# etri/bwa-mem-scale

Hardware: AMD Instinct MI355X
Metric: Mreads/sec through the GPU hot path (seed -> chain -> extend -> dedup, reads and index resident), 150bp SE vs a synthetic genome of GRCh38 size, at 1 MI355X; % HBM roofline in roofline.frac (higher is better)
Workload: dtype int64 intervals / int16 DP (two columns per register; int32 for queries beyond 191 bases or scores beyond 2^14)

## Files before the change

bwa-mem-scale_amd/bwams/capi.py:

```python
from __future__ import annotations

import ctypes as C
import os
import subprocess

import numpy as np

PKG = os.path.dirname(os.path.dirname(os.path.abspath(__file__)))
LIB_PATH = os.environ.get("BWAMS_LIB") or os.path.join(PKG, "_build", "libbwams.so")

SMEM_DTYPE = np.dtype([("rid", "<u4"), ("m", "<u4"), ("n", "<u4"), ("pad_", "<u4"),
                       ("k", "<i8"), ("l", "<i8"), ("s", "<i8")])
SEQPAIR_DTYPE = np.dtype([(n, "<i4") for n in
                          ("idr", "idq", "id", "len1", "len2", "h0", "seqid", "regid",
                           "score", "tle", "gtle", "qle", "gscore", "max_off")])

SYMBOLS = [
    "bwams_strerror", "bwams_last_error", "bwams_device_count", "bwams_debug_reload",
    "bwams_index_open", "bwams_index_from_host", "bwams_index_from_device", "bwams_index_close",
    "bwams_index_bytes", "bwams_index_build", "bwams_index_fetch", "bwams_index_save", "bwams_reg2aln_run", "bwams_reg2aln_run_sam", "bwams_reg2aln_fetch",
    "bwams_index_set_contig_names", "bwams_index_set_contig_annos", "bwams_sam_upload", "bwams_sam_run", "bwams_sam_run_pe", "bwams_sam_run_emf", "bwams_sam_fetch",
    "bwams_process_chunk", "bwams_process_chunk_smart", "bwams_process_chunk2", "bwams_emf_regs_merge", "bwams_fastq_decode", "bwams_fastq_info", "bwams_fastq_has_qual", "bwams_fastq_fetch", "bwams_fastq_to_batch", "bwams_fastq_to_batch_opt", "bwams_fastq_close", "bwams_batch_create", "bwams_batch_destroy", "bwams_seed_fmi",
    "bwams_seed_upload", "bwams_seed_run", "bwams_seed_counts", "bwams_seed_fetch",
    "bwams_ert_from_host", "bwams_ert_open", "bwams_ert_close", "bwams_ert_bytes", "bwams_ert_set_fat", "bwams_seed_run_ert",
# ... 67 lines not shown
class SwOpt(C.Structure):
    _fields_ = [("o_del", C.c_int32), ("e_del", C.c_int32), ("o_ins", C.c_int32),
                ("e_ins", C.c_int32), ("zdrop", C.c_int32), ("end_bonus", C.c_int32),
                ("mat", C.c_int8 * 25), ("pad_", C.c_int8 * 3)]


class MemOpt(C.Structure):
    _fields_ = [("a", C.c_int32), ("o_del", C.c_int32), ("e_del", C.c_int32), ("o_ins", C.c_int32), ("e_ins", C.c_int32),
                ("pen_clip5", C.c_int32), ("pen_clip3", C.c_int32), ("w", C.c_int32), ("zdrop", C.c_int32),
                ("min_seed_len", C.c_int32), ("min_chain_weight", C.c_int32), ("max_chain_extend", C.c_int32),
                ("max_occ", C.c_int32), ("max_chain_gap", C.c_int32), ("mask_level", C.c_float),
                ("drop_ratio", C.c_float), ("mat", C.c_int8 * 25), ("pad_", C.c_int8 * 3), ("extend_all", C.c_int32), ("mask_level_redun", C.c_float), ("max_ins", C.c_int32),
                ("b", C.c_int32), ("pen_unpaired", C.c_int32), ("max_matesw", C.c_int32), ("mapq_coef_len", C.c_int32)]


class FmiDesc(C.Structure):
    _fields_ = [("ref_seq_len", C.c_int64), ("count", C.c_int64 * 5),
                ("cp_occ", C.c_void_p), ("sa_ms_byte", C.c_void_p), ("sa_ls_word", C.c_void_p),
                ("sentinel_index", C.c_int64), ("ref_0123", C.c_void_p)]


class Fastq:

    def __init__(self, text, device: int = 0, n_bytes: int | None = None):
        self.h = C.c_void_p()
        n, nb = C.c_int64(0), C.c_int64(0)
        if isinstance(text, int):
            rc = lib().bwams_fastq_decode(device, C.c_void_p(text), C.c_int64(n_bytes), C.byref(self.h), C.byref(n), C.byref(nb))
        else:
            rc = lib().bwams_fastq_decode(device, text, C.c_int64(len(text)), C.byref(self.h), C.byref(n), C.byref(nb))
        _chk(rc, "bwams_fastq_decode")
        self.n_reads, self.n_bases = n.value, nb.value

    def info(self):
        n, nb, nn, nc, ms = C.c_int64(0), C.c_int64(0), C.c_int64(0), C.c_int64(0), C.c_float(0)
        _chk(lib().bwams_fastq_info(self.h, C.byref(n), C.byref(nb), C.byref(nn), C.byref(nc), C.byref(ms)), "bwams_fastq_info")
        return dict(n_reads=n.value, n_bases=nb.value, name_bytes=nn.value, comment_bytes=nc.value, ms=ms.value)

    def fetch(self):
        i = self.info()
        n1 = i["n_reads"] + 1
        enc = np.zeros(max(i["n_bases"], 1), np.uint8); qual = np.zeros(max(i["n_bases"], 1), np.uint8)
        names = np.zeros(max(i["name_bytes"], 1), np.uint8); comm = np.zeros(max(i["comment_bytes"], 1), np.uint8)
        cum = np.zeros(n1, np.int64); noff = np.zeros(n1, np.int64); coff = np.zeros(n1, np.int64)
        _chk(lib().bwams_fastq_fetch(self.h, _p(enc), _p(cum), _p(names), _p(noff), _p(qual), _p(comm), _p(coff)), "bwams_fastq_fetch")
        nb_, cb_ = bytes(names[:i["name_bytes"]]), bytes(comm[:i["comment_bytes"]])
        return dict(n=i["n_reads"], enc=enc[:i["n_bases"]], cum=cum, quals=qual[:i["n_bases"]] if lib().bwams_fastq_has_qual(self.h) else None,
                    names=[nb_[noff[k]:noff[k + 1]] for k in range(i["n_reads"])],
                    comments=[cb_[coff[k]:coff[k + 1]] or None for k in range(i["n_reads"])])

    def to_batch(self, batch: "Batch"):
        _chk(lib().bwams_fastq_to_batch(self.h, batch.h), "bwams_fastq_to_batch")
        batch._nseq = self.n_reads

    def close(self):
        if self.h:
            lib().bwams_fastq_close(self.h)
            self.h = C.c_void_p()


class SamOpt(C.Structure):
    _fields_ = [("T", C.c_int32), ("flag", C.c_int32), ("XA_drop_ratio", C.c_float), ("max_XA_hits", C.c_int32),
                ("max_XA_hits_alt", C.c_int32), ("rg_id", C.c_char * 256)]


def default_sam_opt(flag: int = 0, rg_id: bytes = b"") -> SamOpt:
    return SamOpt(30, flag, 0.80, 5, 200, rg_id)


class Stats(C.Structure):
    _fields_ = [("n_ext", C.c_int64), ("n_ext_blocks", C.c_int64), ("n_sa_lookups", C.c_int64),
                ("n_lf_steps", C.c_int64), ("n_smem", C.c_int64 * 3), ("bsw_cells", C.c_int64),
                ("n_ext_round", C.c_int64 * 3), ("n_blk_round", C.c_int64 * 3),
                ("ms_smem_r1", C.c_float), ("ms_smem_r2", C.c_float), ("ms_smem_r3", C.c_float),
                ("ms_sort", C.c_float), ("ms_sal", C.c_float), ("ms_seed_total", C.c_float),
                ("ms_bsw", C.c_float), ("ms_ksw", C.c_float), ("ms_tasks", C.c_float), ("ms_emf", C.c_float),
                ("emf_nodes", C.c_int64), ("emf_cmp_bytes", C.c_int64),
                ("n_chains", C.c_int64), ("n_chain_seeds", C.c_int64), ("n_left", C.c_int64), ("n_right", C.c_int64),
                ("n_retry_left", C.c_int64), ("n_retry_right", C.c_int64),
                ("ms_chain", C.c_float), ("ms_ext_plan", C.c_float), ("ms_ext_left", C.c_float),
                ("ms_ext_right", C.c_float), ("ms_ext_purge", C.c_float), ("ms_ext_total", C.c_float),
                ("n_ext_rounds", C.c_int64), ("n_final_regs", C.c_int64), ("ms_dedup", C.c_float), ("ms_pair", C.c_float),
                ("n_pair_tasks", C.c_int64), ("n_pair_redone", C.c_int64), ("n_pair_regs", C.c_int64), ("n_chain_redo", C.c_int64),
                ("ert_kmer_lookups", C.c_int64), ("ert_node_reads", C.c_int64), ("ert_ref_bytes", C.c_int64)]


class BuildStats(C.Structure):
    _fields_ = [("rows", C.c_int64), ("chunks", C.c_int32), ("rounds", C.c_int32), ("unresolved_after_first", C.c_int64),
                ("ms_first_pass", C.c_float), ("ms_outputs", C.c_float)]


class FastaStats(C.Structure):
    _fields_ = [("l_pac", C.c_int64), ("n_seqs", C.c_int32), ("n_holes", C.c_int32), ("n_ambig_bases", C.c_int64),
                ("ms_host_read", C.c_float), ("ms_upload", C.c_float), ("ms_device_pack", C.c_float), ("ms_fm_build", C.c_float),
                ("build", BuildStats)]


class InflateStats(C.Structure):
    _fields_ = [("members", C.c_int64), ("in_bytes", C.c_int64), ("out_bytes", C.c_int64),
                ("ms_upload", C.c_float), ("ms_kernel", C.c_float), ("ms_download", C.c_float)]


class ReaderStats(C.Structure):
    _fields_ = [("device_inflate", C.c_int32), ("in_bytes", C.c_int64), ("out_bytes", C.c_int64),
                ("ms_read", C.c_float), ("ms_inflate", C.c_float)]


class Inflater:

    def __init__(self, device: int = 0, max_in_bytes: int = 32 << 20, max_out_bytes: int = 64 << 20):
        self.h = C.c_void_p()
        self.max_out = max_out_bytes
        _chk(lib().bwams_inflater_create(device, max_in_bytes, max_out_bytes, C.byref(self.h)), "bwams_inflater_create")

    def run_raw(self, gz, out, out_cap: int, on_device: bool):
        used, n_out, st = C.c_int64(0), C.c_int64(0), InflateStats()
        ptr, n = (C.c_void_p(gz[0]), gz[1]) if isinstance(gz, tuple) else (gz, len(gz))
        rc = lib().bwams_inflater_run(self.h, ptr, n, C.c_void_p(out), out_cap, int(on_device), C.byref(used), C.byref(n_out),
                                      C.byref(st))
        return rc, used.value, n_out.value, st

    def run(self, gz: bytes, out_cap: int | None = None):
        cap = out_cap if out_cap is not None else self.max_out
        buf = C.create_string_buffer(max(cap, 1))
        rc, used, n, st = self.run_raw(gz, C.addressof(buf), cap, False)
        _chk(rc, "bwams_inflater_run")
        return buf.raw[:n], used, st

    def close(self):
        if self.h:
            lib().bwams_inflater_destroy(self.h)
            self.h = C.c_void_p()

    def __del__(self):
        try:
            self.close()
        except Exception:
            pass


class DeflateStats(C.Structure):
    _fields_ = [("members", C.c_int64), ("in_bytes", C.c_int64), ("out_bytes", C.c_int64),
                ("ms_upload", C.c_float), ("ms_kernel", C.c_float), ("ms_download", C.c_float)]


DEFLATE_EOF = 0x1


def deflate_bound(n_bytes: int) -> int:
    return lib().bwams_deflate_bound(n_bytes)


class Deflater:

    def __init__(self, device: int = 0, max_in_bytes: int = 32 << 20):
        self.h = C.c_void_p()
        self.device = device
        _chk(lib().bwams_deflater_create(device, max_in_bytes, C.byref(self.h)), "bwams_deflater_create")

    def run_raw(self, data, out, out_cap: int, in_on_device: bool = False, out_on_device: bool = False, flags: int = 0):
        n_out, st = C.c_int64(0), DeflateStats()
        ptr, n = (C.c_void_p(data[0]), data[1]) if isinstance(data, tuple) else (data, len(data))
        rc = lib().bwams_deflater_run(self.h, ptr, n, int(in_on_device), C.c_void_p(out), out_cap, int(out_on_device), flags,
                                      C.byref(n_out), C.byref(st))
        return rc, n_out.value, st

    def run(self, data, eof: bool = False):
# ... 1268 lines not shown
```

bwa-mem-scale_amd/csrc/api.hip:

```cpp
#include <fcntl.h>
#include <sys/mman.h>
#include <sys/stat.h>
#include <unistd.h>

#include <algorithm>
#include <cstring>
#include <mutex>
#include <string>
#include <vector>

#include <rocprim/rocprim.hpp>

#include "fmi_kernels.h"
#include "ert_kernels.h"
#include "stage_state.h"

namespace bwams {

static Knobs g_knobs;
static std::once_flag g_knobs_once;
static int env_int(const char *name, int dflt) { const char *e = getenv(name); return e && *e ? atoi(e) : dflt; }
void knobs_reload() {
    Knobs k;
    { const char *vb = getenv("BWAMS_VERBOSE"); k.verbose = vb && *vb && *vb != '0'; }
    k.debug = env_int("BWAMS_DEBUG", 0);
    k.poison = env_int("BWAMS_POISON", 0);
    k.bwd_min_list = env_int("BWAMS_BWD_MIN_LIST", k.bwd_min_list); k.bwd_cols = env_int("BWAMS_BWD_COLS", k.bwd_cols);
    k.bwd_late_list = env_int("BWAMS_BWD_LATE_LIST", k.bwd_late_list);
    k.bwd_dry_min_list = env_int("BWAMS_BWD_DRY_MIN_LIST", k.bwd_dry_min_list); k.bwd_dry_cols = env_int("BWAMS_BWD_DRY_COLS", k.bwd_dry_cols);
    k.bwd_dry_late_list = env_int("BWAMS_BWD_DRY_LATE_LIST", k.bwd_dry_late_list);
    k.r3_beside = env_int("BWAMS_SEED_R3_BESIDE", 1);
    k.ext_max_rounds = env_int("BWAMS_EXT_MAX_ROUNDS", 0); k.ext_all_rounds = getenv("BWAMS_EXT_ALL_ROUNDS") != nullptr;
    k.ext_inplace = env_int("BWAMS_EXT_INPLACE", 1);
    k.dedup_seq = env_int("BWAMS_DEDUP_SEQ", 0) == 1;
    k.pair_drop_plan = getenv("BWAMS_PAIR_DROP_PLAN") != nullptr;
    k.trace_pair = env_int("BWAMS_TRACE_PAIR", 0);
    k.bsw_pk = env_int("BWAMS_BSW_PK", 1);
    k.chain_batch = env_int("BWAMS_CHAIN_BATCH", 1);
    k.ert_ticket = env_int("BWAMS_ERT_TICKET", 1); k.ert_grid = env_int("BWAMS_ERT_GRID", -1); k.ert_fat = env_int("BWAMS_ERT_FAT", 1);
    g_knobs = k;
}
const Knobs &knobs() {
    std::call_once(g_knobs_once, knobs_reload);
    return g_knobs;
}

static thread_local std::string g_last_error;
void set_last_error(const std::string &s) { g_last_error = s; }

static int check_device(int device) {
    int n = 0;
    hipError_t e = hipGetDeviceCount(&n);
    if (e != hipSuccess || n <= 0) {
        set_last_error(std::string("no HIP device: ") + hipGetErrorString(e));
        return BWAMS_ERR_DEVICE;
    }
    if (device < 0 || device >= n) {
        set_last_error("device ordinal out of range");
        return BWAMS_ERR_ARG;
    }
    hipDeviceProp_t p;
    BWAMS_HIP(hipGetDeviceProperties(&p, device));
    if (std::string(p.gcnArchName).rfind("gfx950", 0) != 0) {
        set_last_error(std::string("device is ") + p.gcnArchName + ", this library is built for gfx950 only");
        return BWAMS_ERR_DEVICE;
    }
    return BWAMS_OK;
}

int tmp_reserve(bwams_batch *b, size_t &tb) {
    if (tb > b->d_tmp.cap) {
        BWAMS_HIP(hipStreamSynchronize(b->stream));
        BWAMS_HIP(b->d_tmp.alloc(tb));
    }
    tb = b->d_tmp.cap;
    return BWAMS_OK;
}
int fmi_build_device(bwams_index *ix, const uint8_t *d_fw, int64_t l_pac, int keep_ref, int64_t chunk_rows, int verbose,
                     bwams_build_stats_t *bs);

}

using namespace bwams;

extern "C" {

const char *bwams_strerror(int code) {
    switch (code) {
        case BWAMS_OK: return "ok";
        case BWAMS_ERR_DEVICE: return "no usable gfx950 device / HIP error";
        case BWAMS_ERR_IO: return "index file missing or malformed";
        case BWAMS_ERR_ARG: return "invalid argument";
        case BWAMS_ERR_CAPACITY: return "output buffer too small";
        case BWAMS_ERR_NOMEM: return "out of memory";
        case BWAMS_ERR_UNSUPPORTED: return "unsupported input";
    }
    return "unknown error";
}

const char *bwams_last_error(void) { return g_last_error.c_str(); }

int bwams_debug_reload(void) { (void)bwams::knobs(); bwams::knobs_reload(); return BWAMS_OK; }

int bwams_device_count(int *n) {
    int c = 0;
    hipError_t e = hipGetDeviceCount(&c);
    if (e != hipSuccess) {
        *n = 0;
        set_last_error(hipGetErrorString(e));
        return BWAMS_ERR_DEVICE;
    }
    *n = c;
    return BWAMS_OK;
}


static int index_finish(bwams_index *ix, const bwams_fmi_desc_t *d, const void *cp, const void *ms, const void *ls, const void *ref) {
    ix->fmi.cp = reinterpret_cast<const uint4 *>(cp);
    ix->fmi.cp2 = nullptr;
    ix->fmi.sa_ms = reinterpret_cast<const int8_t *>(ms);
    ix->fmi.sa_ls = reinterpret_cast<const uint32_t *>(ls);
// ... 1434 lines not shown
```

bwa-mem-scale_amd/csrc/api_chain.hip:

```cpp
#include <cstring>
#include <utility>

#include <rocprim/rocprim.hpp>

#include "stage_state.h"

using namespace bwams;

extern "C" {
int bwams_index_set_contigs(bwams_index_t *ix, const bwams_contig_t *contigs, int32_t n_seqs) {
    if (!ix || !contigs || n_seqs <= 0) return BWAMS_ERR_ARG;
    const int64_t l_pac = (ix->fmi.ref_seq_len - 1) / 2;
    int64_t at = 0;
    for (int32_t i = 0; i < n_seqs; ++i) {
        if (contigs[i].offset != at || contigs[i].len <= 0) {
            set_last_error("bwams_index_set_contigs: sequences must tile [0, l_pac) in order");
            return BWAMS_ERR_ARG;
        }
        at += contigs[i].len;
    }
    if (at != l_pac) {
        set_last_error("bwams_index_set_contigs: sequence lengths do not add up to l_pac");
        return BWAMS_ERR_ARG;
    }
// ... 66 lines not shown
static int chain_common(bwams_batch *b, const bwams_mem_opt_t *opt, const SeedView &sv, int64_t *n_chains, int64_t *n_seeds);

int bwams_chain_run(bwams_batch_t *b, const bwams_mem_opt_t *opt, int64_t *n_chains, int64_t *n_seeds) {
    if (!b || !b->seed_done || !b->with_sa) {
        set_last_error("bwams_chain_run: run bwams_seed_run(with_sa = 1) first");
        return BWAMS_ERR_ARG;
    }
    int rc = check_opt(opt, "bwams_chain_run");
    if (rc) return rc;
    if ((rc = bwams_seed_counts(b, nullptr, nullptr))) return rc;
    SeedView sv;
    sv.smem = b->d_sorted.p; sv.n_smem = b->n_smem; sv.sa_off = b->d_sa_off.p; sv.sa_coord = b->d_sa_coord.p; sv.n_sa = b->n_sa;
    sv.one_smem_quirk = true;
    return chain_common(b, opt, sv, n_chains, n_seeds);
}

int bwams_chain_run_ert(bwams_batch_t *b, const bwams_mem_opt_t *opt, const bwams_ert_mem_t *mems, const int64_t *mem_off,
                        const uint64_t *hits, const int64_t *hit_off, int64_t *n_chains, int64_t *n_seeds) {
    if (!b || b->nseq <= 0 || !mem_off || !hit_off) {
        set_last_error("bwams_chain_run_ert: upload the reads first (bwams_seed_upload) and pass the MEM / hit offsets");
        return BWAMS_ERR_ARG;
    }
    int rc = check_opt(opt, "bwams_chain_run_ert");
    if (rc) return rc;
    const int64_t nseq = b->nseq, n1 = nseq + 1;
    const int64_t n_mems = mem_off[nseq], n_hits = hit_off[nseq];
    if (mem_off[0] != 0 || hit_off[0] != 0 || n_mems < 0 || n_hits < 0 || (n_mems && !mems) || (n_hits && !hits)) return BWAMS_ERR_ARG;
    for (int64_t r = 0; r < nseq; ++r) {
        if (mem_off[r + 1] < mem_off[r] || hit_off[r + 1] < hit_off[r]) { set_last_error("bwams_chain_run_ert: offsets must be non-decreasing"); return BWAMS_ERR_ARG; }
        const int64_t nh = hit_off[r + 1] - hit_off[r];
        for (int64_t i = mem_off[r]; i < mem_off[r + 1]; ++i) {
            const bwams_ert_mem_t &m = mems[i];
            if (m.start < 0 || m.end <= m.start || m.hitcount < 0 || m.hitbeg < 0 || (int64_t)m.hitbeg + m.hitcount > nh) {
                set_last_error("bwams_chain_run_ert: a MEM with an empty span or a hit slice outside its read's hit array");
                return BWAMS_ERR_ARG;
            }
        }
    }
    BWAMS_HIP(hipSetDevice(b->idx->device));
    StageState *s;
    if ((rc = get_state(b, &s))) return rc;
    hipStream_t st = b->stream;
    BWAMS_HIP(s->ch.et_mems.ensure_n((size_t)(n_mems + 1))); BWAMS_HIP(s->ch.et_moff.ensure_n((size_t)n1));
    BWAMS_HIP(s->ch.et_hoff.ensure_n((size_t)n1)); BWAMS_HIP(s->ch.et_hits.ensure_n((size_t)(n_hits + 1)));
    BWAMS_HIP(s->ch.et_smem.ensure_n((size_t)(n_mems + 1))); BWAMS_HIP(s->ch.et_cnt.ensure_n((size_t)(n_mems + 1)));
    BWAMS_HIP(s->ch.et_off.ensure_n((size_t)(n_mems + 1))); BWAMS_HIP(s->ch.et_srt.ensure((size_t)(n_mems + 1) * 24));
    if (n_mems) BWAMS_HIP(hipMemcpyAsync(s->ch.et_mems.p, mems, (size_t)n_mems * sizeof(bwams_ert_mem_t), hipMemcpyHostToDevice, st));
    if (n_hits) BWAMS_HIP(hipMemcpyAsync(s->ch.et_hits.p, hits, (size_t)n_hits * 8, hipMemcpyHostToDevice, st));
    BWAMS_HIP(hipMemcpyAsync(s->ch.et_moff.p, mem_off, (size_t)n1 * 8, hipMemcpyHostToDevice, st));
    BWAMS_HIP(hipMemcpyAsync(s->ch.et_hoff.p, hit_off, (size_t)n1 * 8, hipMemcpyHostToDevice, st));
    ErtArgs E;
    E.mems = s->ch.et_mems.p; E.mem_off = s->ch.et_moff.p; E.hits = s->ch.et_hits.p; E.hit_off = s->ch.et_hoff.p; E.nseq = nseq; E.n_mems = n_mems;
    E.l_pac = (b->idx->fmi.ref_seq_len - 1) / 2; E.max_occ = opt->max_occ; E.pad_ = 0; E.smem_out = s->ch.et_smem.p; E.cnt = s->ch.et_cnt.p;
    E.srt = s->ch.et_srt.p;
    launch_ert_sort(E, st);
    if ((rc = scan_rows(b, s->ch.et_cnt.p, s->ch.et_off.p, 1, n_mems + 1))) return rc;
    int64_t n_sa = 0;
    BWAMS_HIP(hipMemcpyAsync(&n_sa, s->ch.et_off.p + n_mems, 8, hipMemcpyDeviceToHost, st));
    BWAMS_HIP(hipStreamSynchronize(st));
    BWAMS_HIP(s->ch.et_coord.ensure_n((size_t)(n_sa + 1)));
    launch_ert_pick(E, s->ch.et_off.p, s->ch.et_coord.p, st);
    SeedView sv;
    sv.smem = s->ch.et_smem.p; sv.n_smem = n_mems; sv.sa_off = s->ch.et_off.p;
    sv.sa_coord = s->ch.et_coord.p; sv.n_sa = n_sa; sv.one_smem_quirk = false;
    return chain_common(b, opt, sv, n_chains, n_seeds);
}

static int chain_common(bwams_batch *b, const bwams_mem_opt_t *opt, const SeedView &sv, int64_t *n_chains, int64_t *n_seeds) {
    int rc;
    if (b->max_read_len >= 32768) {
        set_last_error("bwams_chain_run: reads of 32768 bases or more are not supported (16-bit query coordinates)");
        return BWAMS_ERR_UNSUPPORTED;
    }
    BWAMS_HIP(hipSetDevice(b->idx->device));
    StageState *s;
    if ((rc = get_state(b, &s))) return rc;
    outdated(s, From::chain);
    hipStream_t st = b->stream;
    const int64_t nseq = b->nseq, n_sa = sv.n_sa, n1 = nseq + 1;
    const size_t ns = (size_t)(n_sa > 0 ? n_sa : 1);
    BWAMS_HIP(s->ch.s_next.ensure_n(ns)); BWAMS_HIP(s->ch.s_ql.ensure_n(ns)); BWAMS_HIP(s->ch.crec.ensure(chain_rec_bytes(n_sa)));
    BWAMS_HIP(s->ch.flt.ensure_n(ns)); BWAMS_HIP(s->ch.f_rec.ensure_n(ns)); BWAMS_HIP(s->ch.f_first.ensure_n(ns));
    BWAMS_HIP(s->ch.f_kept.ensure_n(ns)); BWAMS_HIP(s->ch.f_sel.ensure_n(ns)); BWAMS_HIP(s->ch.n_chn.ensure_n((size_t)n1));
    BWAMS_HIP(s->heavy.ensure_n((size_t)n1)); BWAMS_HIP(s->ch.redo.ensure_n((size_t)n1)); BWAMS_HIP(s->ch.slice.ensure((size_t)n1 * 16));
    BWAMS_HIP(s->ch.okeys.ensure_n((size_t)n1)); BWAMS_HIP(s->ch.okeys2.ensure_n((size_t)n1)); BWAMS_HIP(s->ch.ovals.ensure_n((size_t)n1));
    BWAMS_HIP(s->ch.ovals2.ensure_n((size_t)n1)); BWAMS_HIP(s->ch.nodes.ensure(chain_node_bytes(n_sa, nseq)));
    BWAMS_HIP(s->ch.n_kept.ensure_n((size_t)n1)); BWAMS_HIP(s->ch.n_kept_seeds.ensure_n((size_t)n1)); BWAMS_HIP(s->ch.read_base.ensure_n((size_t)n1));
    BWAMS_HIP(s->ch.frac.ensure_n((size_t)n1)); BWAMS_HIP(s->ch.wide.ensure((size_t)n1 * 16)); BWAMS_HIP(s->ch.chain_off.ensure((size_t)n1 * 16));

    ChainArgs A;
    A.smem = sv.smem; A.n_smem = sv.n_smem; A.sa_off = sv.sa_off; A.sa_coord = sv.sa_coord; A.cum = b->d_cum.p; A.nseq = nseq;
    if ((rc = dev_bns(b->idx, &A.bns))) return rc;
    A.opt = *opt;
    A.s_next = s->ch.s_next.p; A.s_ql = s->ch.s_ql.p; A.crec = s->ch.crec.p; A.flt = s->ch.flt.p; A.f_rec = s->ch.f_rec.p;
    A.f_first = s->ch.f_first.p; A.f_kept = s->ch.f_kept.p; A.f_sel = s->ch.f_sel.p; A.nodes = s->ch.nodes.p; A.n_kept = s->ch.n_kept.p;
    A.n_kept_seeds = s->ch.n_kept_seeds.p; A.n_chn = s->ch.n_chn.p; A.heavy = s->heavy.p; A.redo = s->ch.redo.p; A.slice = s->ch.slice.as<int64_t>();
    A.order = s->ch.ovals2.p; A.read_base = s->ch.read_base.p; A.frac_rep = s->ch.frac.p; A.ctr = b->d_ctr.p; A.seed_batch = knobs().chain_batch;

    BWAMS_HIP(hipEventRecord(s->ev[0], st));
    BWAMS_HIP(hipMemsetAsync(&b->d_ctr.p->chain_redo, 0, 2 * sizeof(unsigned long long), st));
    BWAMS_HIP(hipMemsetAsync(&b->d_ctr.p->chain_overflow, 0, 29 * sizeof(unsigned long long), st));
    if ((sv.one_smem_quirk ? sv.n_smem <= 1 : sv.n_smem <= 0) || n_sa == 0) {
        BWAMS_HIP(hipMemsetAsync(s->ch.n_kept.p, 0, (size_t)n1 * 4, st));
        BWAMS_HIP(hipMemsetAsync(s->ch.n_kept_seeds.p, 0, (size_t)n1 * 4, st));
    } else {
        launch_chain_count(A, s->ch.okeys.p, s->ch.ovals.p, st);
        if ((rc = with_tmp(b, "bwams_chain_run: radix_sort_pairs_desc", [&](void *tmp, size_t &tb) {
                return rocprim::radix_sort_pairs_desc(tmp, tb, s->ch.okeys.p, s->ch.okeys2.p, s->ch.ovals.p, s->ch.ovals2.p, (size_t)nseq, 0, 32, st);
            }))) return rc;
        if (launch_chain(A, s->ch.okeys.p, b->cu_count, st, s->aux, s->fork, s->join)) {
            set_last_error("bwams_chain_run: stream fork/join failed");
            return BWAMS_ERR_DEVICE;
        }
    }
    int64_t tot[2] = {0, 0};
    if (nseq > 0) {
        launch_widen2(A.n_kept, A.n_kept_seeds, nseq, s->ch.wide.as<int64_t>(), st);
        if ((rc = scan_rows(b, s->ch.wide.as<int64_t>(), s->ch.chain_off.as<int64_t>(), 2, n1))) return rc;
        BWAMS_HIP(hipMemcpyAsync(&tot[0], s->ch.chain_off.as<int64_t>() + nseq, 8, hipMemcpyDeviceToHost, st));
        BWAMS_HIP(hipMemcpyAsync(&tot[1], s->ch.chain_off.as<int64_t>() + n1 + nseq, 8, hipMemcpyDeviceToHost, st));
    } else {
        BWAMS_HIP(hipMemsetAsync(s->ch.chain_off.p, 0, (size_t)n1 * 16, st));
    }
    BWAMS_HIP(hipMemcpyAsync(b->h_ctr.p, b->d_ctr.p, sizeof(DevCounters), hipMemcpyDeviceToHost, st));
    BWAMS_HIP(hipStreamSynchronize(st));
    {
        const bool vb = knobs().verbose != 0;
        if (vb) {
            const unsigned long long *d = b->h_ctr.p->dbg;
            fprintf(stderr, "[bwams_chain_run] filter wave tier: reads by chains <=32 %llu <=64 %llu <=128 %llu <=256 %llu <=512 %llu <=960 %llu more %llu; "
                            "Mcycles: sequential(HBM) %.1f sort %.1f filter %.1f; chains %llu selected %llu; longest read: sort %.2f filter %.2f Mcycles, most chains %llu, most selected %llu\n",
                    d[0], d[1], d[2], d[3], d[4], d[5], d[6], d[7] / 1e6, d[8] / 1e6, d[9] / 1e6, d[11], d[10], d[12] / 1e6, d[13] / 1e6, d[14], d[15]);
#ifdef BWAMS_CHAINDBG
            static const char *cn[8] = {"XL", "L", "L2", "L1", "M2", "M", "M1", "S"};
            fprintf(stderr, "[bwams_chain_run] chaining wave tier, per class: reads / mean us / longest us / wave-ms:");
            for (int c = 0; c < 8; ++c) fprintf(stderr, "  %s %llu / %.0f / %.0f / %.1f", cn[c], d[32 + 3 * c], d[32 + 3 * c] ? d[33 + 3 * c] * 1e-2 / d[32 + 3 * c] : 0.0, d[34 + 3 * c] * 1e-2, d[33 + 3 * c] * 1e-5);
            fprintf(stderr, "\n");
            fprintf(stderr, "[bwams_chain_run] wave tier phases, G cycles: preamble %.2f chaining %.2f weights+copy %.2f (sort %.2f filter %.2f: all reads); reads %llu seeds %llu; passes %llu settling %llu seeds (%llu new chains), %llu seeds one by one; pass parts, G cycles: batch prologue %.2f search %.2f record+test %.2f settle %.2f commit %.2f one-by-one %.2f\n",
                    d[56] / 1e9, d[57] / 1e9, d[58] / 1e9, d[8] / 1e9, d[9] / 1e9, d[59], d[60], d[61], d[63], d[64], d[62], d[65] / 1e9, d[66] / 1e9, d[67] / 1e9, d[68] / 1e9, d[69] / 1e9, d[70] / 1e9);
#endif
        }
    }
    if (b->h_ctr.p->chain_overflow) {
        set_last_error("bwams_chain_run: internal B-tree node region exhausted");
        return BWAMS_ERR_CAPACITY;
    }
    const bool has_long = b->h_ctr.p->chain_longread != 0;
    s->ch.n_redo = (int64_t)b->h_ctr.p->chain_redo;
    s->ch.n_chains = tot[0]; s->ch.n_seeds = tot[1]; s->ch.nseq = nseq;
    BWAMS_HIP(s->ch.chains.ensure_n((size_t)(tot[0] + 1))); BWAMS_HIP(s->ch.seeds.ensure_n((size_t)(tot[1] + 1)));
    if (tot[0] > 0) launch_chain_emit(A, s->ch.chain_off.as<int64_t>(), s->ch.chain_off.as<int64_t>() + n1, s->ch.chains.p, s->ch.seeds.p, st);
    if (has_long && tot[0] > 0 && (rc = flt_chained_seeds(b, s, opt, A.bns))) return rc;
    BWAMS_HIP(hipEventRecord(s->ev[1], st));
    BWAMS_HIP(hipGetLastError());
    s->ch.done = true;
    s->opt = *opt;
    if (n_chains) *n_chains = s->ch.n_chains;
    if (n_seeds) *n_seeds = s->ch.n_seeds;
    return BWAMS_OK;
}

int bwams_chain_fetch(bwams_batch_t *b, bwams_chain_t *chains, int64_t chain_cap, bwams_chain_seed_t *seeds,
                      int64_t seed_cap, int64_t *chain_off) {
    if (!b || !b->chain || !b->chain->ch.done) {
        set_last_error("bwams_chain_fetch: no chains on the device");
        return BWAMS_ERR_ARG;
    }
    StageState *s = b->chain;
    if (s->ch.n_chains > chain_cap || s->ch.n_seeds > seed_cap) return BWAMS_ERR_CAPACITY;
    BWAMS_HIP(hipSetDevice(b->idx->device));
    hipStream_t st = b->stream;
    if (s->ch.n_chains) BWAMS_HIP(hipMemcpyAsync(chains, s->ch.chains.p, (size_t)s->ch.n_chains * sizeof(bwams_chain_t), hipMemcpyDeviceToHost, st));
    if (s->ch.n_seeds) BWAMS_HIP(hipMemcpyAsync(seeds, s->ch.seeds.p, (size_t)s->ch.n_seeds * sizeof(bwams_chain_seed_t), hipMemcpyDeviceToHost, st));
    if (chain_off) BWAMS_HIP(hipMemcpyAsync(chain_off, s->ch.chain_off.p, (size_t)(s->ch.nseq + 1) * 8, hipMemcpyDeviceToHost, st));
    BWAMS_HIP(hipStreamSynchronize(st));
    return BWAMS_OK;
}

int bwams_chain_upload(bwams_batch_t *b, const bwams_chain_t *chains, int64_t n_chains, const bwams_chain_seed_t *seeds,
                       int64_t n_seeds, const int64_t *chain_off) {
    if (!b || !chain_off || n_chains < 0 || n_seeds < 0 || (n_chains && (!chains || !seeds))) return BWAMS_ERR_ARG;
    if (b->nseq <= 0) {
        set_last_error("bwams_chain_upload: upload the reads first (bwams_seed_upload)");
        return BWAMS_ERR_ARG;
    }
    const int64_t nseq = b->nseq, n1 = nseq + 1;
    if (chain_off[0] != 0 || chain_off[nseq] != n_chains) return BWAMS_ERR_ARG;
    int64_t at = 0;
    std::string bad;
    int64_t *soff = new int64_t[(size_t)n1];
    for (int64_t r = 0; r < nseq && bad.empty(); ++r) {
        soff[r] = at;
        if (chain_off[r + 1] < chain_off[r]) bad = "chain_off must be non-decreasing";
        for (int64_t j = chain_off[r]; j < chain_off[r + 1] && bad.empty(); ++j) {
            if (chains[j].seqid != r) bad = "chain.seqid does not match chain_off";
            else if (chains[j].seed_off != at || chains[j].n < 0) bad = "chain.seed_off must enumerate the seed array in order";
            at += chains[j].n;
        }
    }
    soff[nseq] = at;
    if (bad.empty() && at != n_seeds) bad = "seed counts do not add up";
    if (!bad.empty()) {
        delete[] soff;
        set_last_error("bwams_chain_upload: " + bad);
        return BWAMS_ERR_ARG;
    }
    BWAMS_HIP(hipSetDevice(b->idx->device));
    StageState *s;
    int rc = get_state(b, &s);
    if (rc) { delete[] soff; return rc; }
    outdated(s, From::chain);
    hipStream_t st = b->stream;
    BWAMS_HIP(s->ch.chain_off.ensure((size_t)n1 * 16)); BWAMS_HIP(s->ch.chains.ensure_n((size_t)(n_chains + 1)));
    BWAMS_HIP(s->ch.seeds.ensure_n((size_t)(n_seeds + 1)));
    BWAMS_HIP(hipMemcpyAsync(s->ch.chain_off.p, chain_off, (size_t)n1 * 8, hipMemcpyHostToDevice, st));
    BWAMS_HIP(hipMemcpyAsync(s->ch.chain_off.as<int64_t>() + n1, soff, (size_t)n1 * 8, hipMemcpyHostToDevice, st));
    if (n_chains) BWAMS_HIP(hipMemcpyAsync(s->ch.chains.p, chains, (size_t)n_chains * sizeof(bwams_chain_t), hipMemcpyHostToDevice, st));
    if (n_seeds) BWAMS_HIP(hipMemcpyAsync(s->ch.seeds.p, seeds, (size_t)n_seeds * sizeof(bwams_chain_seed_t), hipMemcpyHostToDevice, st));
    BWAMS_HIP(hipStreamSynchronize(st));
    delete[] soff;
    s->ch.n_chains = n_chains; s->ch.n_seeds = n_seeds; s->ch.nseq = nseq;
    s->ch.done = true;
    return BWAMS_OK;
}
}
```

bwa-mem-scale_amd/csrc/api_regions.hip:

```cpp
#include <algorithm>
#include <cmath>
#include <cstring>
#include <utility>

#include <rocprim/rocprim.hpp>

#include "stage_state.h"

using namespace bwams;

extern "C" {

int bwams_dedup_run(bwams_batch_t *b, const bwams_mem_opt_t *opt, int64_t *n_regs) {
    if (!b || !b->chain || !b->chain->ext.done) {
        set_last_error("bwams_dedup_run: run bwams_extend_run first");
        return BWAMS_ERR_ARG;
    }
    int rc = check_opt(opt, "bwams_dedup_run");
    if (rc) return rc;
    StageState *s = b->chain;
    BWAMS_HIP(hipSetDevice(b->idx->device));
    hipStream_t st = b->stream;
    outdated(s, From::dedup);
    const int64_t N = s->ch.n_seeds, n1 = s->ch.nseq + 1;
    const int64_t L = b->max_read_len > 1 ? b->max_read_len : 1;
    int64_t n_lanes = ((int64_t)1 << 30) / ((L + 2) * 8);
    n_lanes = n_lanes > 65536 ? 65536 : n_lanes < 64 ? 64 : n_lanes;
    const int64_t n_waves = (int64_t)b->cu_count * 4, n_waves_small = (int64_t)b->cu_count * 16;
    BWAMS_HIP(s->dd.regs.ensure_n((size_t)(N + 1))); BWAMS_HIP(s->dd.out.ensure_n((size_t)(N + 1))); BWAMS_HIP(s->dd.ord.ensure_n((size_t)(N + 1)));
    BWAMS_HIP(s->dd.srt.ensure(dedup_sortrec_bytes(N)));
    BWAMS_HIP(s->dd.eh.ensure((size_t)(n_lanes + 2 * n_waves + n_waves_small) * (size_t)(L + 2) * 8)); BWAMS_HIP(s->dd.nout.ensure_n((size_t)n1));
    BWAMS_HIP(s->dd.wide.ensure((size_t)n1 * 16)); BWAMS_HIP(s->dd.off.ensure_n((size_t)n1));
    DedupArgs D;
    D.regs = s->dd.regs.p; D.seed_off = s->ch.chain_off.as<int64_t>() + n1; D.enc = b->d_enc.p; D.cum = b->d_cum.p; D.nseq = s->ch.nseq;
    D.ref = b->idx->fmi.ref;
    if ((rc = dev_bns(b->idx, &D.bns))) return rc;
    D.opt = *opt; D.ord = s->dd.ord.p; D.srt = s->dd.srt.p; D.eh = s->dd.eh.as<int2>(); D.eh_lanes = n_lanes; D.max_read_len = (int32_t)L;
    D.n_out = s->dd.nout.p;
    BWAMS_HIP(s->heavy.ensure_n((size_t)n1));
    D.force_seq = knobs().dedup_seq;
    BWAMS_HIP(s->dd.light.ensure_n((size_t)n1));
    D.heavy = s->heavy.p; D.light = s->dd.light.p; D.n_heavy_ctr = &b->d_ctr.p->dedup_heavy; D.ticket = &b->d_ctr.p->dedup_ticket;
    D.n_light_ctr = &b->d_ctr.p->dedup_light; D.ticket2 = &b->d_ctr.p->dedup_ticket2; D.ticket3 = &b->d_ctr.p->dedup_ticket3;
    const bool verbose_dd = knobs().verbose != 0;
    D.dbg = verbose_dd ? b->d_ctr.p->dbg : nullptr;
    if (verbose_dd) BWAMS_HIP(hipMemsetAsync(b->d_ctr.p->dbg, 0, sizeof b->d_ctr.p->dbg, st));
    BWAMS_HIP(hipMemsetAsync(&b->d_ctr.p->dedup_heavy, 0, 3 * sizeof(unsigned long long), st));
    BWAMS_HIP(hipMemsetAsync(&b->d_ctr.p->dedup_ticket2, 0, 2 * sizeof(unsigned long long), st));
    BWAMS_HIP(hipEventRecord(s->ev[12], st));
    if (N) BWAMS_HIP(hipMemcpyAsync(D.regs, s->ext.regs.p, (size_t)N * sizeof(bwams_alnreg_t), hipMemcpyDeviceToDevice, st));
    BWAMS_HIP(hipMemsetAsync(D.n_out, 0, (size_t)n1 * 4, st));
    if (launch_dedup(D, n_lanes, n_waves, n_waves_small, st, s->aux[0], s->aux[1], s->aux[2], s->fork, s->join[0], s->join[1], s->join[2])) {
        set_last_error("bwams_dedup_run: stream fork/join failed");
        return BWAMS_ERR_DEVICE;
    }
    int64_t total = 0;
    if (s->ch.nseq > 0) {
        launch_widen2(D.n_out, D.n_out, s->ch.nseq, s->dd.wide.as<int64_t>(), st);
        if ((rc = scan_rows(b, s->dd.wide.as<int64_t>(), s->dd.off.p, 1, n1))) return rc;
        launch_dedup_gather(D, s->dd.off.p, s->dd.out.p, st);
        BWAMS_HIP(hipMemcpyAsync(&total, s->dd.off.p + s->ch.nseq, 8, hipMemcpyDeviceToHost, st));
    } else {
        BWAMS_HIP(hipMemsetAsync(s->dd.off.p, 0, 8, st));
    }
    BWAMS_HIP(hipEventRecord(s->ev[13], st));
    if (verbose_dd) BWAMS_HIP(hipMemcpyAsync(b->h_ctr.p->dbg, b->d_ctr.p->dbg, sizeof b->d_ctr.p->dbg, hipMemcpyDeviceToHost, st));
    BWAMS_HIP(hipStreamSynchronize(st));
    BWAMS_HIP(hipGetLastError());
    if (verbose_dd) {
        const unsigned long long *d = b->h_ctr.p->dbg;
        fprintf(stderr, "[bwams_dedup_run] largest wave instance: %llu reads, %llu slots, %llu alive; Mcycles: load %.1f sort(end) %.1f pairs %.1f reload %.1f sort(score) %.1f store %.1f; "
                        "longest read: sort(end) %.2f pairs %.2f sort(score) %.2f, whole %.2f (read %llu, %llu regions; %llu patch alignments in %.2f, %llu scan trips); all reads: %llu patch alignments in %.1f\n",
                d[0], d[1], d[2], d[3] / 1e6, d[4] / 1e6, d[5] / 1e6, d[6] / 1e6, d[7] / 1e6, d[8] / 1e6, d[9] / 1e6, d[10] / 1e6, d[11] / 1e6, d[12] / 1e6, d[13], d[14],
                d[15], d[16] / 1e6, d[17], d[18], d[19] / 1e6);
    }
    s->dd.n_final = total;
    s->dd.done = true;
    if (n_regs) *n_regs = total;
    return BWAMS_OK;
}

int bwams_dedup_fetch(bwams_batch_t *b, bwams_alnreg_t *regs, int64_t reg_cap, int64_t *reg_off) {
    if (!b || !b->chain || !b->chain->dd.done) {
        set_last_error("bwams_dedup_fetch: run bwams_dedup_run first");
        return BWAMS_ERR_ARG;
    }
    StageState *s = b->chain;
    if (s->dd.n_final > reg_cap) return BWAMS_ERR_CAPACITY;
    BWAMS_HIP(hipSetDevice(b->idx->device));
    hipStream_t st = b->stream;
    if (s->dd.n_final) BWAMS_HIP(hipMemcpyAsync(regs, s->dd.out.p, (size_t)s->dd.n_final * sizeof(bwams_alnreg_t), hipMemcpyDeviceToHost, st));
    if (reg_off) BWAMS_HIP(hipMemcpyAsync(reg_off, s->dd.off.p, (size_t)(s->ch.nseq + 1) * 8, hipMemcpyDeviceToHost, st));
    BWAMS_HIP(hipStreamSynchronize(st));
    return BWAMS_OK;
}


static int pair_run_impl(bwams_batch_t *b, const bwams_mem_opt_t *opt, const bwams_pestat_t pes[4], int64_t id_base, int32_t flags,
                         int primary5_T, int no_pairing, int64_t *n_regs, int64_t *n_tasks);

int bwams_pair_run(bwams_batch_t *b, const bwams_mem_opt_t *opt, const bwams_pestat_t pes[4], int64_t id_base, int32_t flags,
                   int64_t *n_regs, int64_t *n_tasks) {
    return pair_run_impl(b, opt, pes, id_base, flags, -1, 0, n_regs, n_tasks);
}

int bwams_pair_run_sam(bwams_batch_t *b, const bwams_mem_opt_t *opt, const bwams_sam_opt_t *sam_opt, const bwams_pestat_t pes[4],
                       int64_t id_base, int32_t flags, int64_t *n_regs, int64_t *n_tasks) {
    if (!sam_opt) return pair_run_impl(b, opt, pes, id_base, flags, -1, 0, n_regs, n_tasks);
    if (sam_opt->T < 0) {
        set_last_error("bwams_pair_run_sam: T must not be negative");
        return BWAMS_ERR_ARG;
    }
    if (sam_opt->flag & BWAMS_MEM_F_NO_RESCUE) flags |= BWAMS_PAIR_NO_RESCUE;
    return pair_run_impl(b, opt, pes, id_base, flags, (sam_opt->flag & BWAMS_MEM_F_PRIMARY5) ? sam_opt->T : -1,
                         (sam_opt->flag & BWAMS_MEM_F_NOPAIRING) != 0, n_regs, n_tasks);
}

static int pair_run_impl(bwams_batch_t *b, const bwams_mem_opt_t *opt, const bwams_pestat_t pes[4], int64_t id_base, int32_t flags,
                         int primary5_T, int no_pairing, int64_t *n_regs, int64_t *n_tasks) {
    const int single_end = (flags & BWAMS_PAIR_SINGLE_END) != 0;
    const int no_rescue = (flags & BWAMS_PAIR_NO_RESCUE) || single_end, use_ert = (flags & BWAMS_PAIR_USE_ERT) != 0;
    static const bwams_pestat_t no_pes[4] = {{0, 0, 1, 0, 0., 0.}, {0, 0, 1, 0, 0., 0.}, {0, 0, 1, 0, 0., 0.}, {0, 0, 1, 0, 0., 0.}};
    if (single_end && !pes) pes = no_pes;
    if (!b || !b->chain || !b->chain->dd.done) {
        set_last_error("bwams_pair_run: run bwams_dedup_run first");
        return BWAMS_ERR_ARG;
    }
    int rc = check_opt(opt, "bwams_pair_run");
    if (rc) return rc;
    StageState *s = b->chain;
    if (!pes || (!single_end && (s->ch.nseq & 1))) {
        set_last_error("bwams_pair_run: needs the insert-size statistics and an even number of reads (ends of pair p at 2p, 2p + 1)");
        return BWAMS_ERR_ARG;
    }
    int tmax = 1;
// ... 346 lines not shown
```

bwa-mem-scale_amd/csrc/api_state.hip:

```cpp
#include <cstring>
#include <map>

#include <rocprim/rocprim.hpp>

#include "stage_state.h"

namespace bwams {

struct AuxSet { hipStream_t q[7] = {}; int refs = 0; };
static std::mutex g_aux_mu;
static std::map<int, AuxSet> g_aux;
static int aux_acquire(int device, hipStream_t *out) {
    std::lock_guard<std::mutex> g(g_aux_mu);
    AuxSet &a = g_aux[device];
    if (a.refs == 0)
        for (auto &q : a.q) BWAMS_HIP(hipStreamCreateWithFlags(&q, hipStreamNonBlocking));
    ++a.refs;
    for (int i = 0; i < 7; ++i) out[i] = a.q[i];
    return BWAMS_OK;
}
static void aux_release(int device) {
    std::lock_guard<std::mutex> g(g_aux_mu);
    auto it = g_aux.find(device);
    if (it == g_aux.end()) return;
// ... 26 lines not shown
}

void launch_widen2(const int32_t *a, const int32_t *b, int64_t n, int64_t *wide, hipStream_t st) {
    widen2_kernel<<<(unsigned)((2 * (n + 1) + 255) / 256), 256, 0, st>>>(a, b, n, wide);
}

int scan_rows(bwams_batch *b, const int64_t *in, int64_t *out, int rows, int64_t n1) {
    for (int r = 0; r < rows; ++r)
        if (int rc = with_tmp(b, "scan_rows: exclusive_scan", [&](void *tmp, size_t &tb) {
                return rocprim::exclusive_scan(tmp, tb, in + r * n1, out + r * n1, (int64_t)0, (size_t)n1, rocprim::plus<int64_t>(), b->stream);
            })) return rc;
    return BWAMS_OK;
}

void outdated(StageState *s, From first) {
    switch (first) {
    case From::chain: s->ch.done = false; [[fallthrough]];
    case From::built: s->ext.built = s->ext.done = false; [[fallthrough]];
    case From::dedup: s->dd.done = false; [[fallthrough]];
    case From::pair: s->pr.done = false; break;
    case From::al: s->al.done = false; break;
    case From::er: s->er.done = false; break;
    case From::sam_upload: s->sm.up = false; [[fallthrough]];
    case From::sam: s->sm.done = false; [[fallthrough]];
    case From::bam: s->bm.done = s->bs.done = s->md.done = false; break;
    }
}

int get_state(bwams_batch *b, StageState **out) {
    if (!b->chain) {
        b->chain = new StageState();
        for (auto &e : b->chain->ev) BWAMS_HIP(hipEventCreate(&e));
        for (auto &e : b->chain->join) BWAMS_HIP(hipEventCreateWithFlags(&e, hipEventDisableTiming));
        BWAMS_HIP(hipEventCreateWithFlags(&b->chain->fork, hipEventDisableTiming));
        b->chain->ev_ok = true;
        if (int rc = aux_acquire(b->idx->device, b->chain->aux)) return rc;
        b->chain->aux_device = b->idx->device;
    }
    *out = b->chain;
    return BWAMS_OK;
}

int check_opt(const bwams_mem_opt_t *o, const char *who) {
    if (!o || o->e_del <= 0 || o->e_ins <= 0 || o->max_occ <= 0 || o->w < 0) {
        set_last_error(std::string(who) + ": null options, non-positive gap extension penalty or max_occ");
        return BWAMS_ERR_ARG;
    }
    return BWAMS_OK;
}

int dev_bns(bwams_index *ix, DevBns *out) {
    const int64_t l_pac = (ix->fmi.ref_seq_len - 1) / 2;
    if (!ix->d_contigs.p) {
        bwams_contig_t c;
        c.offset = 0; c.len = (int32_t)l_pac; c.is_alt = 0;
        if (l_pac > 0x7fffffffLL) {
            set_last_error("the index holds more than 2^31 bases: call bwams_index_set_contigs with the real sequences");
            return BWAMS_ERR_ARG;
        }
        BWAMS_HIP(ix->d_contigs.alloc(sizeof c));
        BWAMS_HIP(hipMemcpy(ix->d_contigs.p, &c, sizeof c, hipMemcpyHostToDevice));
        ix->n_seqs = 1;
    }
    out->contigs = ix->d_contigs.as<const bwams_contig_t>();
    out->n_seqs = ix->n_seqs;
    out->l_pac = l_pac;
    return BWAMS_OK;
}

void sw_params(const bwams_mem_opt_t &o, int end_bonus, SwParams *prm) {
    prm->o_del = o.o_del; prm->e_del = o.e_del; prm->o_ins = o.o_ins; prm->e_ins = o.e_ins;
    prm->zdrop = o.zdrop; prm->end_bonus = end_bonus;
    int mx = 0;
    for (int i = 0; i < 25; ++i) {
        prm->mat[i] = o.mat[i];
        mx = mx > o.mat[i] ? mx : o.mat[i];
    }
    prm->max_sc = mx;
}

void chain_state_stats(const StageState *s, bwams_stats_t *out) {
    if (!s) return;
    out->n_chains = s->ch.n_chains; out->n_chain_seeds = s->ch.n_seeds; out->n_chain_redo = s->ch.n_redo;
    out->n_left = s->ext.n_left; out->n_right = s->ext.n_right;
    out->n_retry_left = s->ext.n_retry_left; out->n_retry_right = s->ext.n_retry_right;
    auto el = [&](int a, int b, float *dst) {
        float ms = 0;
        if (hipEventElapsedTime(&ms, s->ev[a], s->ev[b]) == hipSuccess) *dst = ms;
    };
    el(0, 1, &out->ms_chain);
    el(2, 3, &out->ms_ext_plan);
    if (s->ext.done) {
        el(4, 5, &out->ms_ext_left);
        el(6, 7, &out->ms_ext_right);
        el(8, 9, &out->ms_ext_purge);
        el(10, 11, &out->ms_ext_total);
        out->n_ext_rounds = s->ext.n_rounds;
    }
    if (s->dd.done) { el(12, 13, &out->ms_dedup); out->n_final_regs = s->dd.n_final; }
    if (s->pr.done) {
        el(14, 15, &out->ms_pair);
        out->n_pair_tasks = s->pr.tasks; out->n_pair_redone = s->pr.redone; out->n_pair_regs = s->pr.total;
    }
    (void)hipGetLastError();
}
}
```

bwa-mem-scale_amd/csrc/chain.hip:

```cpp
#include "common.h"
#include "chain_kernels.h"
#include "wave_ops.h"

namespace bwams {
namespace {

constexpr int KB_T = 5;
constexpr int KB_MAXK = 2 * KB_T - 1;
constexpr int kLaneSeeds = 32;
constexpr int kLightChains = 16;
struct alignas(16) Node {
    int16_t n, internal;
    int32_t ptr[KB_MAXK + 1];
    int64_t pos[KB_MAXK];
    int32_t key[KB_MAXK];
};
static_assert(sizeof(Node) == 160, "node layout");

struct alignas(16) ChainRec {
    int64_t last_rbeg, endr;
    uint16_t first_qbeg, last_qbeg, last_len, endq;
    int32_t rid, n;
    int32_t first_idx, last_idx;
    int32_t wq, wr;
// ... 709 lines not shown
            while (rem) {
                const int i = __builtin_ctzll(rem);
                rem &= rem - 1;
                int fin = act;
                if (displaced) {
                    const int64_t x = qbeg - best_q, y = rbeg - best;
                    if (rid != best_rid) fin = NEW;
                    else if (qbeg >= best_q && qbeg + slen <= best_q + best_l && rbeg + slen <= best + best_l) fin = NOOP;
                    else if (best < l_pac && rbeg >= l_pac) fin = NEW;
                    else fin = (x - y <= w && y - x <= w && x - best_l < max_gap && y - best_l < max_gap) ? UNSETTLED : NEW;
                } else if (touched) fin = UNSETTLED;
                const int a_i = __builtin_amdgcn_readlane(fin, i);
                if (a_i == UNSETTLED) { first_open = i; break; }
                if (lane == i) act = fin;
                if (a_i == NEW) {
                    const int64_t rb_i = readlane64(rbeg, i);
                    const int rid_i = __builtin_amdgcn_readlane(rid, i), q_i = __builtin_amdgcn_readlane(qbeg, i), l_i = __builtin_amdgcn_readlane(slen, i);
                    if (lane > i && rb_i <= rbeg && rb_i > best) { best = rb_i; best_rid = rid_i; best_q = q_i; best_l = l_i; displaced = true; }
                } else if (a_i == MERGE) {
                    const int low_i = __builtin_amdgcn_readlane(lower, i);
                    if (lane > i && lower == low_i) touched = true;
                }
            }
            const bool com = pend && lane < first_open;
            TQ(3)
            const unsigned long long m_new = __ballot(com && act == NEW);
            if (__ballot(com && act == NEW && (eq || (displaced && best == rbeg)))) return false;
            if (com && act == MERGE) {
                S.s_ql[g] = make_int2(qbeg, slen); S.s_next[g] = -1; S.s_next[ch.last_idx] = g;
                if (qbeg >= ch.endq) ch.wq += slen; else if (qbeg + slen > ch.endq) ch.wq += qbeg + slen - ch.endq;
                ch.endq = (uint16_t)((int)ch.endq > qbeg + slen ? (int)ch.endq : qbeg + slen);
                if (rbeg >= ch.endr) ch.wr += slen; else if (rbeg + slen > ch.endr) ch.wr += (int)(rbeg + slen - ch.endr);
                ch.endr = ch.endr > rbeg + slen ? ch.endr : rbeg + slen;
                ch.last_rbeg = rbeg; ch.last_qbeg = (uint16_t)qbeg; ch.last_len = (uint16_t)slen; ch.last_idx = g; ch.n += 1;
                S.crec[lower] = ch;
            }
            if (m_new) {
                const int m = __popcll(m_new);
                const bool mine = com && act == NEW;
                int min_idx = mine ? idx : n;
                for (int d = 32; d >= 1; d >>= 1) { const int o = __shfl_xor(min_idx, d); min_idx = o < min_idx ? o : min_idx; }
                for (int cb = n > 0 ? ((n - 1) >> 6) << 6 : -64; cb >= 0 && cb + 63 > min_idx; cb -= 64) {
                    const int p = cb + lane;
                    const bool mv = p < n;
                    const int64_t kk = mv ? S.s_key[p] : 0;
                    const int32_t cc = mv ? S.s_cid[p] : 0;
                    int sh = __popcll(__ballot(mine && idx < cb));
                    unsigned long long mm = __ballot(mine && idx >= cb && idx < cb + 64);
                    while (mm) { const int i = __builtin_ctzll(mm); mm &= mm - 1; sh += __builtin_amdgcn_readlane(idx, i) < p ? 1 : 0; }
                    if (mv && sh) { S.s_key[p + sh] = kk; S.s_cid[p + sh] = cc; }
                }
                int rank = 0;
                { unsigned long long mm = m_new; while (mm) { const int i = __builtin_ctzll(mm); mm &= mm - 1; rank += __builtin_amdgcn_readlane(idx, i) < idx ? 1 : 0; } }
                { unsigned long long mm = m_new & __ballot(shared); while (mm) { const int i = __builtin_ctzll(mm); mm &= mm - 1; rank += (__builtin_amdgcn_readlane(idx, i) == idx && readlane64(rbeg, i) < rbeg) ? 1 : 0; } }
                if (mine) {
                    const int32_t cid = n + __popcll(m_new & below);
                    S.s_ql[g] = make_int2(qbeg, slen); S.s_next[g] = -1;
                    ChainRec nc;
                    nc.last_rbeg = rbeg; nc.endr = rbeg + slen;
                    nc.first_qbeg = (uint16_t)qbeg; nc.last_qbeg = (uint16_t)qbeg; nc.last_len = (uint16_t)slen; nc.endq = (uint16_t)(qbeg + slen);
                    nc.rid = rid; nc.n = 1; nc.first_idx = g; nc.last_idx = g; nc.wq = slen; nc.wr = slen;
                    S.crec[cid] = nc;
                    S.s_key[idx + 1 + rank] = rbeg; S.s_cid[idx + 1 + rank] = cid;
                }
                n_keys = n + m;
            }
            if (com) pend = false;
#ifdef BWAMS_CHAINDBG
            if (lane == 0) { atomicAdd(&A.ctr->dbg[61], 1ull); atomicAdd(&A.ctr->dbg[63], (unsigned long long)__popcll(__ballot(com))); atomicAdd(&A.ctr->dbg[64], (unsigned long long)__popcll(m_new)); }
#endif
            if (__popcll(__ballot(com)) <= 1) one_by_one = 8;
            if (S.crec_hbm) __threadfence_block();
            TQ(4)
        }
    }
#ifdef BWAMS_CHAINDBG
    if (lane == 0) for (int k = 0; k < 6; ++k) atomicAdd(&A.ctr->dbg[65 + k], tq[k]);
#endif
    return true;
}

__device__ void heavy_read(const ChainArgs &A, int64_t r, int64_t base, int n_chn, unsigned char *lds, int cap, int lane);
__host__ __device__ constexpr size_t heavy_lds_bytes(int cap);
template <bool LDS, int CONT = 0, bool CREC_HBM = false>
__device__ __forceinline__ bool chain_read(const ChainArgs &A, int64_t r, int lane, int nl, Node *nodes, int32_t cap_nodes,
                                           ChainRec *crec_w, int32_t cap_chains) {
    const bool wr = lane == 0;
#ifdef BWAMS_CHAINDBG
    const unsigned long long tp0 = __builtin_amdgcn_s_memtime();
#endif
    if (wr) {
        A.n_kept[r] = 0;
        A.n_kept_seeds[r] = 0;
        A.read_base[r] = 0;
        A.n_chn[r] = 0;
    }
    const bwams_smem_t *sm = A.smem;
    const int64_t beg = A.slice[2 * r], end = A.slice[2 * r + 1];
    const int L = (int)(A.cum[r + 1] - A.cum[r]);
    if (beg == end || L < A.opt.min_seed_len) return true;

    int b = 0, e = 0, l_rep = 0;
    if (nl == 64 && end - beg <= 64) {
        const bool has = beg + lane < end;
        const int my_b = has ? (int)sm[beg + lane].m : 0, my_e = has ? (int)sm[beg + lane].n + 1 : 0;
        unsigned long long rep = __ballot(has && sm[beg + lane].s > (int64_t)A.opt.max_occ);
        while (rep) {
            const int i = __builtin_ctzll(rep);
            rep &= rep - 1;
            const int sb = __builtin_amdgcn_readlane(my_b, i), se = __builtin_amdgcn_readlane(my_e, i);
            if (sb > e) { l_rep += e - b; b = sb; e = se; }
            else e = e > se ? e : se;
        }
    } else
    for (int64_t i = beg; i < end; ++i) {
        const int sb = (int)sm[i].m, se = (int)sm[i].n + 1;
        if (sm[i].s <= (int64_t)A.opt.max_occ) continue;
        if (sb > e) { l_rep += e - b; b = sb; e = se; }
        else e = e > se ? e : se;
    }
    l_rep += e - b;
    if (wr) A.frac_rep[r] = (float)l_rep / (float)L;

    const int64_t base = A.sa_off[beg];
    const int32_t cnt = (int32_t)(A.sa_off[end] - base);
    if (wr) A.read_base[r] = base;
    if (cnt == 0) return true;
    const int64_t *pos = A.sa_coord + base;
    int32_t *s_next = A.s_next + base;
    int2 *s_ql = A.s_ql + base;
    ChainRec *crec_g = reinterpret_cast<ChainRec *>(A.crec) + base;
    ChainRec *crec;
    ReadCtx c;
    if constexpr (LDS) {
        crec = CREC_HBM ? crec_g : crec_w;
        c.nodes = nodes; c.cap_nodes = cap_nodes;
    } else {
        crec = crec_g;
        const int64_t nbase = (base >> 1) + 2 * r;
        c.nodes = reinterpret_cast<Node *>(A.nodes) + nbase;
        c.cap_nodes = (int32_t)((((base + cnt) >> 1) + 2 * (r + 1)) - nbase);
    }
    c.crec = crec;
    c.n_nodes = 0; c.n_keys = 0; c.overflow = false; c.wr = wr;
    int64_t *s_key = nullptr;
    int32_t *s_cid = nullptr;
    if constexpr (CONT == 1) {
        s_key = reinterpret_cast<int64_t *>(nodes);
        s_cid = reinterpret_cast<int32_t *>(s_key + cap_chains);
    } else c.root = new_node(c);
    RidCache rc;
    rc.lo = 0; rc.hi = -1; rc.rid = 0;
    WaveBns wb;
    wb.off = 0;
    if (nl == 64 && A.bns.n_seqs <= 4096) wb = wave_bns_load(A.bns, lane);
    if (LDS && cnt > cap_chains) { if (wr) atomicAdd(&A.ctr->chain_overflow, 1ull); return true; }

    const int64_t l_pac = A.bns.l_pac;
#ifdef BWAMS_CHAINDBG
    const unsigned long long tp1 = __builtin_amdgcn_s_memtime();
#endif
    if constexpr (CONT == 1) {
        if (nl == 64 && A.seed_batch) {
            SeedCtx S;
            S.pos = pos; S.s_next = s_next; S.s_ql = s_ql; S.crec = crec; S.s_key = s_key; S.s_cid = s_cid; S.crec_hbm = CREC_HBM;
            int nk = 0;
// ... 63 lines not shown
                ch.last_rbeg = rbeg; ch.endr = rbeg + slen;
                ch.first_qbeg = (uint16_t)qbeg; ch.last_qbeg = (uint16_t)qbeg; ch.last_len = (uint16_t)slen; ch.endq = (uint16_t)(qbeg + slen);
                ch.rid = rid; ch.n = 1; ch.first_idx = g; ch.last_idx = g; ch.wq = slen; ch.wr = slen;
                const int32_t cid = c.n_keys;
                if (wr) crec[cid] = ch;
                if constexpr (CONT == 1) {
                    if (c.n_keys && !path.ok) return false;
                    sarr_insert(s_key, s_cid, c.n_keys, c.n_keys ? path.leaf + 1 : 0, rbeg, cid, lane);
                    ++c.n_keys;
                } else kbt_put(c, cid, rbeg);
                if (c.overflow) { if (wr) atomicAdd(&A.ctr->chain_overflow, 1ull); return true; }
            }
        }
    }
    if (c.n_keys == 0) return true;
#ifdef BWAMS_CHAINDBG
    const unsigned long long tp2 = __builtin_amdgcn_s_memtime();
#endif

    int32_t *ord = A.f_first + base;
    int32_t n_trav;
    if constexpr (CONT == 1) {
        n_trav = c.n_keys;
        for (int32_t t = lane; t < n_trav; t += nl) ord[t] = s_cid[t];
        __threadfence_block();
    } else n_trav = kbt_traverse(c, ord);
    uint2 *fl = A.flt + base;
    int n_chn = 0;
    if (nl == 64) {
        uint2 first = make_uint2(0u, 0u);
        for (int32_t t0 = 0; t0 < n_trav; t0 += 64) {
            const int32_t t = t0 + lane;
            const bool ok = t < n_trav;
            int32_t id = 0;
            if (ok) { if constexpr (CONT == 1) id = s_cid[t]; else id = ord[t]; }
            const ChainRec *pc = &crec[id];
            int w = pc->wr < pc->wq ? pc->wr : pc->wq;
            w = w < (1 << 30) ? w : (1 << 30) - 1;
            if (t0 == 0) first = make_uint2((unsigned)__builtin_amdgcn_readfirstlane(w), (unsigned)__builtin_amdgcn_readfirstlane(id));
            const bool keep = ok && w >= A.opt.min_chain_weight;
            const unsigned long long m = __ballot(keep);
            if (keep) fl[n_chn + __popcll(m & ((1ull << lane) - 1ull))] = make_uint2((unsigned)w, (unsigned)id);
            n_chn += __popcll(m);
        }
        if (n_chn == 0 && wr) fl[0] = first;
        __threadfence_block();
    } else
    for (int32_t t = 0; t < n_trav; ++t) {
        const int32_t id = ord[t];
        const ChainRec ch = crec[id];
        int w = ch.wr < ch.wq ? ch.wr : ch.wq;
        w = w < (1 << 30) ? w : (1 << 30) - 1;
        if (t == 0 && wr) fl[0] = make_uint2((unsigned)w, (unsigned)id);
        if (w < A.opt.min_chain_weight) continue;
        if (wr) fl[n_chn] = make_uint2((unsigned)w, (unsigned)id);
        ++n_chn;
    }
    if (n_chn == 0) n_chn = 1;
    if constexpr (LDS && !CREC_HBM)
        for (int32_t k = lane; k < c.n_keys; k += nl) crec_g[k] = crec_w[k];
    if constexpr (LDS) {
        if (nl == 64) {
#ifdef BWAMS_CHAINDBG
            if (wr) {
                const unsigned long long tp3 = __builtin_amdgcn_s_memtime();
                atomicAdd(&A.ctr->dbg[56], tp1 - tp0); atomicAdd(&A.ctr->dbg[57], tp2 - tp1); atomicAdd(&A.ctr->dbg[58], tp3 - tp2);
                atomicAdd(&A.ctr->dbg[59], 1ull); atomicAdd(&A.ctr->dbg[60], (unsigned long long)cnt);
            }
#endif
            unsigned char *region = CREC_HBM ? reinterpret_cast<unsigned char *>(nodes) : reinterpret_cast<unsigned char *>(crec_w);
            const size_t bytes = (size_t)cap_chains * (CREC_HBM ? 12 : sizeof(ChainRec) + 12);
            const int cap_f = (int)((bytes - 64) / 41);
            if (cap_f >= 64 && n_chn <= cap_f) {
                if (wr) A.n_chn[r] = n_chn;
                __threadfence_block();
                heavy_read(A, r, base, n_chn, region, cap_f, lane);
                return true;
            }
        }
    }
    if (!wr) return true;
    A.n_chn[r] = n_chn;
    if (n_chn > kLightChains) {
        const unsigned long long slot = atomicAdd(&A.ctr->n_heavy, 1ull);
        A.heavy[slot] = (int32_t)r;
        return true;
    }
    flt_introsort(fl, n_chn);
    uint4 *rec = A.f_rec + base;
    int32_t *kept = A.f_kept + base;
    for (int i = 0; i < n_chn; ++i) {
        rec[i] = make_rec(A, crec[fl[i].y], fl[i].x);
        kept[i] = 0;
    }
    filter_seq(A.opt, n_chn, rec, kept, A.f_sel + base);
    if constexpr (LDS) __threadfence_block();
    finish_read(A, r, base, n_chn, L);
    return true;
}

__global__ __launch_bounds__(64) void chain_kernel(ChainArgs A, const uint32_t *__restrict__ n_seeds) {
    const int64_t r = (int64_t)blockIdx.x * blockDim.x + threadIdx.x;
    if (r >= A.nseq) return;
    if (n_seeds[r] > (uint32_t)kLaneSeeds) return;
    chain_read<false>(A, r, 0, 1, nullptr, 0, nullptr, 0);
}

__global__ __launch_bounds__(64) __attribute__((amdgpu_waves_per_eu(3, 3))) void chain_wave_kernel(ChainArgs A, const unsigned long long *lo_p, const unsigned long long *hi_p,
                                                        unsigned long long *ticket, int K) {
    extern __shared__ __align__(16) unsigned char l_mem[];
    const int lane = threadIdx.x;
    const int64_t lo = lo_p ? (int64_t)*lo_p : 0, hi = (int64_t)*hi_p;
    ChainRec *l_crec = reinterpret_cast<ChainRec *>(l_mem);
    Node *l_nodes = reinterpret_cast<Node *>(l_mem + (size_t)(K > 0 ? K : 0) * sizeof(ChainRec));
    for (;;) {
        const unsigned long long t = wave_ticket(ticket, 1ull);
        if (lo + (int64_t)t >= hi) break;
        const int64_t r = (int64_t)A.order[lo + (int64_t)t];
#ifdef BWAMS_CHAINDBG
        const unsigned long long tk0 = wall_clock64();
#endif
        if (K < 0) {
            if (!chain_read<true, 1, true>(A, r, lane, 64, reinterpret_cast<Node *>(l_mem), 0, nullptr, -K) && lane == 0)
                A.redo[atomicAdd(&A.ctr->chain_redo, 1ull)] = (int32_t)r;
        } else if (K) {
            if (!chain_read<true, 1>(A, r, lane, 64, l_nodes, 0, l_crec, K) && lane == 0)
                A.redo[atomicAdd(&A.ctr->chain_redo, 1ull)] = (int32_t)r;
        } else chain_read<false>(A, r, lane, 64, nullptr, 0, nullptr, 0);
        __syncthreads();
#ifdef BWAMS_CHAINDBG
        if (lane == 0) {
            const int c = K < 0 ? 0 : K == kClassL ? 1 : K == kClassL2 ? 2 : K == kClassL1 ? 3 : K == kClassM2 ? 4 : K == kClassM ? 5 : K == kClassM1 ? 6 : 7;
            const unsigned long long dt = wall_clock64() - tk0;
            atomicAdd(&A.ctr->dbg[32 + 3 * c], 1ull); atomicAdd(&A.ctr->dbg[33 + 3 * c], dt); atomicMax(&A.ctr->dbg[34 + 3 * c], dt);
        }
#endif
    }
}

__global__ __launch_bounds__(64) void chain_redo_kernel(ChainArgs A) {
    const int lane = threadIdx.x;
    const int64_t n = (int64_t)A.ctr->chain_redo;
    for (;;) {
        const int64_t t = (int64_t)wave_ticket(&A.ctr->chain_redo_ticket, 1ull);
        if (t >= n) break;
        chain_read<false>(A, A.redo[t], lane, 64, nullptr, 0, nullptr, 0);
    }
}

constexpr int kHeavyCap[6] = {64, 128, 256, 512, 960, 3840};
__host__ __device__ constexpr size_t heavy_lds_bytes(int cap) { return (size_t)cap * 41 + 64; }
static_assert(heavy_lds_bytes(kHeavyCap[5]) <= 160 * 1024, "the largest class must fit one CU's LDS");

__device__ void heavy_read(const ChainArgs &A, int64_t r, int64_t base, int n_chn, unsigned char *lds, int cap, int lane) {
    uint4 *l_rec = reinterpret_cast<uint4 *>(lds);
    uint4 *l_sel = l_rec + cap;
    uint2 *l_fl = reinterpret_cast<uint2 *>(l_sel + cap);
    uint8_t *l_kept = reinterpret_cast<uint8_t *>(l_fl + cap);
    const int L = (int)(A.cum[r + 1] - A.cum[r]);
    uint2 *fl = A.flt + base;
    const ChainRec *crec = reinterpret_cast<const ChainRec *>(A.crec) + base;
    const unsigned long long t_0 = __builtin_amdgcn_s_memtime();
    if (lane == 0) {
        const int bk = n_chn <= 32 ? 0 : n_chn <= 64 ? 1 : n_chn <= 128 ? 2 : n_chn <= 256 ? 3 : n_chn <= 512 ? 4 : n_chn <= 960 ? 5 : 6;
        atomicAdd(&A.ctr->dbg[bk], 1ull);
    }
    {
        __syncthreads();
        for (int i = lane; i < n_chn; i += 64) l_fl[i] = fl[i];
        __syncthreads();
        wave_flt_introsort(l_fl, n_chn, reinterpret_cast<uint16_t *>(l_sel), reinterpret_cast<int *>(reinterpret_cast<char *>(l_sel) + (size_t)n_chn * 8), lane);
        const unsigned long long t_1 = __builtin_amdgcn_s_memtime();
        for (int i = lane; i < n_chn; i += 64) {
            const uint2 f = l_fl[i];
            l_rec[i] = make_rec(A, crec[f.y], f.x);
            l_kept[i] = 0;
        }
        __syncthreads();
        int n_sel = 1;
        if (lane == 0) { const uint4 r0 = l_rec[0]; l_sel[0] = make_uint4(r0.x, r0.y, r0.z, 0u); l_kept[0] = 3; }
        __syncthreads();
        const float mask_level = A.opt.mask_level, drop_ratio = A.opt.drop_ratio;
        const int max_gap = A.opt.max_chain_gap, min_dw = A.opt.min_seed_len << 1;
        for (int ib = 1; ib < n_chn; ib += 64) {
            const int i = ib + lane;
            const bool valid = i < n_chn;
            const uint4 ri = valid ? l_rec[i] : make_uint4(0, 0, 0, 0);
            const int bi = (int)ri.x, ei = (int)ri.y, wi = (int)(ri.z & 0x7fffffffu), li = ei - bi;
            const bool alt_i = (ri.z >> 31) != 0;
            const float fwi = (float)wi;
            bool alive = valid, large = false;
            const int n_sel0 = n_sel;
            for (int k0 = 0; k0 < n_sel0; k0 += 4) {
                uint4 rj[4];
#pragma unroll
                for (int u = 0; u < 4; ++u) rj[u] = l_sel[k0 + u < n_sel0 ? k0 + u : n_sel0 - 1];
#pragma unroll
                for (int u = 0; u < 4; ++u) {
                    if (k0 + u >= n_sel0) break;
                    const int bj = (int)rj[u].x, ej = (int)rj[u].y;
                    const int b_max = bj > bi ? bj : bi, e_min = ej < ei ? ej : ei;
                    const bool alt_j = (rj[u].z >> 31) != 0;
                    const int lj = ej - bj, min_l = li < lj ? li : lj;
                    const bool lg = alive && e_min > b_max && (!alt_j || alt_i) && (float)(e_min - b_max) >= (float)min_l * mask_level && min_l < max_gap;
                    const unsigned long long m_lg = __ballot(lg);
                    if (m_lg) {
                        if (lane == __builtin_ctzll(m_lg)) atomicMin(&l_rec[rj[u].w].w, (uint32_t)i);
                        if (lg) {
                            large = true;
                            const int wj = (int)(rj[u].z & 0x7fffffffu);
                            if (fwi < (float)wj * drop_ratio && wj - wi >= min_dw) alive = false;
                        }
                    }
                }
                if (!__ballot(alive)) break;
            }
            unsigned long long todo = __ballot(alive);
            while (todo) {
                const int lp = __builtin_ctzll(todo);
                const int bj = __builtin_amdgcn_readlane(bi, lp), ej = __builtin_amdgcn_readlane(ei, lp);
                const uint32_t zj = (uint32_t)__builtin_amdgcn_readlane((int)ri.z, lp);
                if (lane == lp) { l_sel[n_sel] = make_uint4(ri.x, ri.y, ri.z, (uint32_t)i); l_kept[i] = large ? 2 : 3; }
                ++n_sel;
                const int b_max = bj > bi ? bj : bi, e_min = ej < ei ? ej : ei;
                const bool alt_j = (zj >> 31) != 0;
                const int lj = ej - bj, min_l = li < lj ? li : lj;
                const bool lg = alive && lane > lp && e_min > b_max && (!alt_j || alt_i) && (float)(e_min - b_max) >= (float)min_l * mask_level && min_l < max_gap;
                const unsigned long long m_lg = __ballot(lg);
                if (m_lg) {
                    if (lane == __builtin_ctzll(m_lg)) l_rec[ib + lp].w = (uint32_t)i;
                    if (lg) {
                        large = true;
                        const int wj = (int)(zj & 0x7fffffffu);
                        if (fwi < (float)wj * drop_ratio && wj - wi >= min_dw) alive = false;
                    }
                }
                todo = __ballot(alive) & ~((2ull << lp) - 1ull);
            }
            __syncthreads();
        }
        for (int k = lane; k < n_sel; k += 64) {
            const int f = (int)l_rec[l_sel[k].w].w;
            if (f >= 0) l_kept[f] = 1;
        }
        __syncthreads();
        if (lane == 0) {
            const unsigned long long t_2 = __builtin_amdgcn_s_memtime();
            atomicAdd(&A.ctr->dbg[8], t_1 - t_0);
            atomicAdd(&A.ctr->dbg[9], t_2 - t_1);
            atomicMax(&A.ctr->dbg[12], t_1 - t_0);
            atomicMax(&A.ctr->dbg[13], t_2 - t_1);
            atomicMax(&A.ctr->dbg[14], (unsigned long long)n_chn);
            atomicMax(&A.ctr->dbg[15], (unsigned long long)n_sel);
            atomicAdd(&A.ctr->dbg[10], (unsigned long long)n_sel);
            atomicAdd(&A.ctr->dbg[11], (unsigned long long)n_chn);
        }
        if (A.opt.max_chain_extend <= n_chn) {
            if (lane == 0) {
                int i, k;
                for (i = k = 0; i < n_chn; ++i) {
                    if (l_kept[i] == 0 || l_kept[i] == 3) continue;
                    if (++k >= A.opt.max_chain_extend) break;
                }
                for (; i < n_chn; ++i)
                    if (l_kept[i] < 3) l_kept[i] = 0;
            }
            __syncthreads();
        }
        int32_t *first = A.f_first + base;
        int n_out = 0, n_seeds = 0;
        for (int ib = 0; ib < n_chn; ib += 64) {
            const int i = ib + lane;
            const int kp = i < n_chn ? (int)l_kept[i] : 0;
            const unsigned long long m = __ballot(kp != 0);
            if (kp) {
                const int o = n_out + __popcll(m & ((1ull << lane) - 1ull));
                const uint2 f = l_fl[i];
                const uint4 rc4 = l_rec[i];
                fl[o] = make_uint2(f.x | ((unsigned)kp << 29) | (rc4.z & 0x80000000u), f.y);
                first[o] = (int32_t)rc4.w;
                n_seeds += crec[f.y].n;
            }
            n_out += __popcll(m);
        }
        for (int d = 32; d >= 1; d >>= 1) n_seeds += __shfl_xor(n_seeds, d);
        if (lane == 0) {
            A.n_kept[r] = n_out;
            A.n_kept_seeds[r] = n_seeds;
            if (n_out) {
                const double min_l = A.opt.min_chain_weight ? (double)(1.1f * (float)A.opt.min_chain_weight) : (double)5.5f * log((double)L);
                if (!(min_l > (double)(0.05f * (float)L))) atomicAdd(&A.ctr->chain_longread, 1ull);
            }
        }
        __syncthreads();
    }
}

__global__ __launch_bounds__(64) void chain_heavy_kernel(ChainArgs A, const unsigned long long *n_heavy_p, int cap_lo, int cap,
                                                         unsigned long long *ticket) {
    extern __shared__ __align__(16) unsigned char l_heavy[];
    const int kLdsChains = cap;
    const int lane = threadIdx.x;
    const int64_t n_heavy = (int64_t)*n_heavy_p;
    for (;;) {
        const int64_t hi = (int64_t)wave_ticket(ticket, 1ull);
        if (hi >= n_heavy) break;
        const int64_t r = A.heavy[hi];
        const int64_t base = A.read_base[r];
        const int n_chn = A.n_chn[r];
        if (n_chn <= cap_lo || (n_chn > cap && cap != kHeavyCap[5])) continue;
        const int L = (int)(A.cum[r + 1] - A.cum[r]);
        uint2 *fl = A.flt + base;
        uint4 *rec = A.f_rec + base;
        int32_t *kept = A.f_kept + base;
        const ChainRec *crec = reinterpret_cast<const ChainRec *>(A.crec) + base;
        if (n_chn > kLdsChains) {
            const unsigned long long t_0 = __builtin_amdgcn_s_memtime();
            if (lane == 0) {
                atomicAdd(&A.ctr->dbg[6], 1ull);
                flt_introsort(fl, n_chn);
                for (int i = 0; i < n_chn; ++i) { rec[i] = make_rec(A, crec[fl[i].y], fl[i].x); kept[i] = 0; }
                filter_seq(A.opt, n_chn, rec, kept, A.f_sel + base);
                finish_read(A, r, base, n_chn, L);
                atomicAdd(&A.ctr->dbg[7], __builtin_amdgcn_s_memtime() - t_0);
            }
            continue;
        }
        heavy_read(A, r, base, n_chn, l_heavy, cap, lane);
    }
}

__global__ __launch_bounds__(256) void chain_emit_kernel(ChainArgs A, const int64_t *__restrict__ chain_off, const int64_t *__restrict__ seed_off,
                                                         bwams_chain_t *chains, bwams_chain_seed_t *seeds) {
    const int64_t r = ((int64_t)blockIdx.x * blockDim.x + threadIdx.x) >> 4;
    const int sub = threadIdx.x & 15;
    const bool live = r < A.nseq;
    const int nk = live ? A.n_kept[r] : 0;
    if (nk == 0) return;
    const int64_t base = A.read_base[r];
    const uint2 *fl = A.flt + base;
    const int32_t *first = A.f_first + base;
    const int32_t *s_next = A.s_next + base;
    const int2 *s_ql = A.s_ql + base;
    const int64_t *pos = A.sa_coord + base;
    const ChainRec *crec = reinterpret_cast<const ChainRec *>(A.crec) + base;
    int64_t so0 = seed_off[r];
    const int64_t co = chain_off[r];
    const float frac = A.frac_rep[r];
    for (int j0 = 0; j0 < nk; j0 += 16) {
        const int j = j0 + sub;
        const bool has = j < nk;
        uint2 f = make_uint2(0u, 0u);
        ChainRec ch;
        ch.n = 0; ch.first_idx = -1; ch.rid = 0;
        if (has) { f = fl[j]; ch = crec[f.y]; }
        const int n = has ? ch.n : 0;
        int incl = n;
        for (int d = 1; d < 16; d <<= 1) {
            const int o = __shfl_up(incl, d, 16);
            if (sub >= d) incl += o;
        }
        const int total = __shfl(incl, 15, 16);
        if (has) {
            int64_t so = so0 + (incl - n);
            bwams_chain_t c;
            c.seqid = (int32_t)r; c.cseed = 0;
            c.n = n;
            int m = 1;
            while (m < n) m <<= 1;
            c.m = m;
            c.first = first[j];
            c.rid = ch.rid;
            c.w_kept_alt = f.x;
            c.frac_rep = frac;
            c.pos = pos[ch.first_idx];
            c.seed_off = so;
            chains[co + j] = c;
            for (int32_t g = ch.first_idx; g >= 0; g = s_next[g]) {
                bwams_chain_seed_t sd;
                sd.rbeg = pos[g];
                sd.qbeg = s_ql[g].x; sd.len = s_ql[g].y; sd.score = sd.len;
                sd.done = 0; sd.pad0_[0] = sd.pad0_[1] = sd.pad0_[2] = 0;
                sd.aln = 0; sd.pad1_ = 0;
                seeds[so++] = sd;
            }
        }
        so0 += total;
    }
}

}

size_t chain_node_bytes(int64_t n_sa, int64_t nseq) { return (size_t)((n_sa >> 1) + 2 * nseq + 4) * sizeof(Node); }
size_t chain_rec_bytes(int64_t n_sa) { return (size_t)(n_sa > 0 ? n_sa : 1) * sizeof(ChainRec); }

void launch_chain_count(const ChainArgs &A, uint32_t *keys, uint32_t *vals, hipStream_t st) {
    if (A.nseq <= 0) return;
    (void)hipMemsetAsync(A.slice, 0, (size_t)A.nseq * 16, st);
    if (A.n_smem > 0) chain_slice_kernel<<<(unsigned)((A.n_smem + 255) / 256), 256, 0, st>>>(A);
    chain_count_kernel<<<(unsigned)((A.nseq + 255) / 256), 256, 0, st>>>(A, keys, vals);
}
int launch_chain(const ChainArgs &A, const uint32_t *n_seeds, int cu_count, hipStream_t st, hipStream_t *aux,
                 hipEvent_t fork, hipEvent_t *join) {
    if (A.nseq <= 0) return 0;
    unsigned long long *cls = A.ctr->chain_class, *tk = A.ctr->chain_ticket;
    if (hipFuncSetAttribute(reinterpret_cast<const void *>(chain_wave_kernel), hipFuncAttributeMaxDynamicSharedMemorySize,
                            (int)lds_bytes_xl(kClassXL2)) != hipSuccess) return -1;
    if (hipEventRecord(fork, st) != hipSuccess) return -1;
    for (int i = 0; i < 7; ++i)
        if (hipStreamWaitEvent(aux[i], fork, 0) != hipSuccess) return -1;
    chain_wave_kernel<<<(unsigned)cu_count, 64, lds_bytes_xl(kClassXL2), st>>>(A, cls + 9, cls + 6, tk + 9, -kClassXL2);
    chain_wave_kernel<<<(unsigned)(cu_count * 8), 64, 0, aux[0]>>>(A, nullptr, cls + 9, tk + 0, 0);
    chain_wave_kernel<<<(unsigned)cu_count, 64, lds_bytes_xl(kClassXL), aux[0]>>>(A, cls + 6, cls + 0, tk + 6, -kClassXL);
    chain_wave_kernel<<<(unsigned)cu_count, 64, lds_bytes(kClassL), aux[1]>>>(A, cls + 0, cls + 7, tk + 1, kClassL);
    chain_wave_kernel<<<(unsigned)(cu_count * 2), 64, lds_bytes(kClassL2), aux[5]>>>(A, cls + 7, cls + 1, tk + 7, kClassL2);
    chain_wave_kernel<<<(unsigned)(cu_count * 3), 64, lds_bytes(kClassL1), aux[2]>>>(A, cls + 1, cls + 8, tk + 2, kClassL1);
    chain_wave_kernel<<<(unsigned)(cu_count * 4), 64, lds_bytes(kClassM2), aux[6]>>>(A, cls + 8, cls + 2, tk + 8, kClassM2);
    chain_wave_kernel<<<(unsigned)(cu_count * 8), 64, lds_bytes(kClassM1), aux[2]>>>(A, cls + 3, cls + 4, tk + 4, kClassM1);
    chain_wave_kernel<<<(unsigned)(cu_count * 12), 64, lds_bytes(kClassS), aux[3]>>>(A, cls + 4, cls + 5, tk + 5, kClassS);
    chain_kernel<<<(unsigned)((A.nseq + 63) / 64), 64, 0, aux[1]>>>(A, n_seeds);
    chain_wave_kernel<<<(unsigned)(cu_count * 5), 64, lds_bytes(kClassM), aux[5]>>>(A, cls + 2, cls + 3, tk + 3, kClassM);
    for (int i = 0; i < 7; ++i) {
        if (hipEventRecord(join[i], aux[i]) != hipSuccess) return -1;
        if (hipStreamWaitEvent(st, join[i], 0) != hipSuccess) return -1;
    }
    chain_redo_kernel<<<(unsigned)(cu_count * 2), 64, 0, st>>>(A);
    if (hipFuncSetAttribute(reinterpret_cast<const void *>(chain_heavy_kernel), hipFuncAttributeMaxDynamicSharedMemorySize,
                            (int)heavy_lds_bytes(kHeavyCap[5])) != hipSuccess) return -1;
    if (hipEventRecord(fork, st) != hipSuccess) return -1;
    for (int i = 0; i < 5; ++i)
        if (hipStreamWaitEvent(aux[i], fork, 0) != hipSuccess) return -1;
    unsigned long long *htk = A.ctr->heavy_tickets;
    chain_heavy_kernel<<<(unsigned)cu_count, 64, heavy_lds_bytes(kHeavyCap[5]), st>>>(A, &A.ctr->n_heavy, kHeavyCap[4], kHeavyCap[5], htk + 5);
    chain_heavy_kernel<<<(unsigned)(cu_count * 4), 64, heavy_lds_bytes(kHeavyCap[4]), aux[1]>>>(A, &A.ctr->n_heavy, kHeavyCap[3], kHeavyCap[4], htk + 4);
    chain_heavy_kernel<<<(unsigned)(cu_count * 7), 64, heavy_lds_bytes(kHeavyCap[3]), aux[2]>>>(A, &A.ctr->n_heavy, kHeavyCap[2], kHeavyCap[3], htk + 3);
    chain_heavy_kernel<<<(unsigned)(cu_count * 12), 64, heavy_lds_bytes(kHeavyCap[2]), aux[0]>>>(A, &A.ctr->n_heavy, kHeavyCap[1], kHeavyCap[2], htk + 2);
    chain_heavy_kernel<<<(unsigned)(cu_count * 16), 64, heavy_lds_bytes(kHeavyCap[1]), aux[3]>>>(A, &A.ctr->n_heavy, kHeavyCap[0], kHeavyCap[1], htk + 1);
    chain_heavy_kernel<<<(unsigned)(cu_count * 24), 64, heavy_lds_bytes(kHeavyCap[0]), aux[4]>>>(A, &A.ctr->n_heavy, 0, kHeavyCap[0], htk + 0);
    for (int i = 0; i < 5; ++i) {
        if (hipEventRecord(join[i], aux[i]) != hipSuccess) return -1;
        if (hipStreamWaitEvent(st, join[i], 0) != hipSuccess) return -1;
    }
    return 0;
}
void launch_chain_emit(const ChainArgs &A, const int64_t *chain_off, const int64_t *seed_off, bwams_chain_t *chains,
                       bwams_chain_seed_t *seeds, hipStream_t st) {
    if (A.nseq <= 0) return;
    chain_emit_kernel<<<(unsigned)((A.nseq * 16 + 255) / 256), 256, 0, st>>>(A, chain_off, seed_off, chains, seeds);
}

}
```

bwa-mem-scale_amd/csrc/chain_kernels.h:

```cpp
#pragma once

#include "common.h"

namespace bwams {

struct DevBns {
    const bwams_contig_t *contigs;
    int32_t n_seqs;
    int64_t l_pac;
};

struct ChainArgs {
    const bwams_smem_t *smem;
    int64_t n_smem;
    const int64_t *sa_off;
    const int64_t *sa_coord;
    const int64_t *cum;
    int64_t nseq;
    DevBns bns;
    bwams_mem_opt_t opt;
    int32_t *s_next;
    int2 *s_ql;
    void *crec;
    uint2 *flt;
    uint4 *f_rec;
    int32_t *f_first, *f_kept, *f_sel;
    void *nodes;
    int32_t *n_kept, *n_kept_seeds, *n_chn;
    int32_t *heavy;
    int64_t *read_base;
    int64_t *slice;
    const uint32_t *order;
    float *frac_rep;
    int32_t *redo;
    int32_t seed_batch;
    DevCounters *ctr;
};

size_t chain_node_bytes(int64_t n_sa, int64_t nseq);
size_t chain_rec_bytes(int64_t n_sa);
void launch_chain_count(const ChainArgs &A, uint32_t *keys, uint32_t *vals, hipStream_t st);
int launch_chain(const ChainArgs &A, const uint32_t *n_seeds, int cu_count, hipStream_t st, hipStream_t *aux,
                 hipEvent_t fork, hipEvent_t *join);
void launch_chain_emit(const ChainArgs &A, const int64_t *chain_off, const int64_t *seed_off, bwams_chain_t *chains,
                       bwams_chain_seed_t *seeds, hipStream_t st);

struct ExtArgs {
    const bwams_chain_t *chains;
    int64_t n_chains;
    bwams_chain_seed_t *seeds;
    int64_t n_seeds;
    const int64_t *chain_off;
    const int64_t *seed_off;
    const uint8_t *enc;
    const int64_t *cum;
    int64_t nseq;
    const uint8_t *ref;
    DevBns bns;
    bwams_mem_opt_t opt;
    bwams_alnreg_t *regs;
    uint32_t *srt;
    int64_t *rmax;
    int32_t *cnt;
    int32_t *state;
    void *kreg;
    int32_t *cur, *lim;
    int32_t *sel_heavy;
    unsigned long long *n_sel_heavy, *sel_ticket;
    int32_t *req_list;
    int32_t *rtask;
    DevCounters *ctr;
};
void launch_ext_plan(const ExtArgs &A, int extend_all, hipStream_t st);
void launch_ext_widen(const ExtArgs &A, const int32_t *list, int64_t n, int64_t *wide, hipStream_t st);
void launch_ext_build(const ExtArgs &A, const int32_t *list, int64_t n, const int64_t *offs, bwams_seqpair_t *left, uint8_t *lref, uint8_t *lqer,
                      bwams_seqpair_t *right, uint8_t *rref, uint8_t *rqer, int64_t *lsrc, int64_t *rsrc, hipStream_t st);
void launch_ext_post(const ExtArgs &A, int right, const bwams_seqpair_t *pairs, int64_t n, int w, int last_try,
                     bwams_seqpair_t *retry, unsigned long long *n_retry, bwams_seqpair_t *rpairs, hipStream_t st);
void launch_ext_heavy_list(const ExtArgs &A, hipStream_t st);
int launch_ext_select(const ExtArgs &A, int cu_count, hipStream_t st, hipStream_t *aux, hipEvent_t fork, hipEvent_t *join);
void launch_ext_request_rest(const ExtArgs &A, hipStream_t st);

struct SeedSwArgs {
    bwams_chain_t *chains;
    int64_t n_chains;
    bwams_chain_seed_t *seeds;
    int64_t n_seeds;
    const uint8_t *enc;
    const int64_t *cum;
    int64_t nseq;
    const uint8_t *ref;
    DevBns bns;
    bwams_mem_opt_t opt;
    int32_t *cnt;
    int32_t *win_qb;
    int64_t *win_rb;
    int32_t *seed_read;
};
void launch_seedsw_plan(const SeedSwArgs &A, int64_t *wide, hipStream_t st);
void launch_seedsw_build(const SeedSwArgs &A, const int64_t *offs, bwams_seqpair_t *pairs, uint8_t *ref, uint8_t *qer,
                         int cu_count, hipStream_t st);
void launch_seedsw_apply(const SeedSwArgs &A, const int64_t *offs, const bwams_kswr_t *res, int32_t *new_n, int64_t *wide,
                         hipStream_t st);
void launch_seedsw_repack(const SeedSwArgs &A, const int32_t *new_n, const int64_t *new_off, bwams_chain_seed_t *out,
                          const int64_t *chain_off, int64_t *seed_off, hipStream_t st);

struct DedupArgs {
    bwams_alnreg_t *regs;
    const int64_t *seed_off;
    const uint8_t *enc;
    const int64_t *cum;
    int64_t nseq;
    const uint8_t *ref;
    DevBns bns;
    bwams_mem_opt_t opt;
    int32_t *ord;
    void *srt;
    int2 *eh;
    int64_t eh_lanes;
    int32_t max_read_len;
    int32_t *n_out;
    int32_t *heavy, *light;
    unsigned long long *n_heavy_ctr, *n_light_ctr, *ticket;
    int32_t force_seq;
    unsigned long long *ticket2, *ticket3;
    unsigned long long *dbg;
};
size_t dedup_sortrec_bytes(int64_t n);
int launch_dedup(const DedupArgs &A, int64_t n_lanes, int64_t n_waves, int64_t n_waves_small, hipStream_t st, hipStream_t aux,
                 hipStream_t aux2, hipStream_t aux3, hipEvent_t fork, hipEvent_t join, hipEvent_t join2, hipEvent_t join3);
void launch_pestat(const bwams_alnreg_t *regs, const int64_t *reg_off, int64_t n_pairs, int64_t l_pac, const bwams_mem_opt_t &opt,
                   unsigned long long *keys, hipStream_t st);
void launch_dedup_gather(const DedupArgs &A, const int64_t *out_off, bwams_alnreg_t *out, hipStream_t st);
int launch_sort_test(const int64_t *k, const int32_t *s, const int32_t *q, int n, int by_score, int mode, int32_t *order);

struct EmfRegArgs {
    DevEmf t;
    const uint32_t *perfect;
    const uint8_t *code;
    const uint8_t *enc;
    const int64_t *cum;
    int64_t nseq;
    DevBns bns;
    bwams_mem_opt_t opt;
    void *scratch;
};
size_t emfregs_scratch_bytes(int64_t n);
void launch_emfregs_count(const EmfRegArgs &A, int64_t *wide, hipStream_t st);
void launch_emfregs_merge_count(const int64_t *off_a, const int64_t *off_b, int64_t nseq, int64_t *wide, hipStream_t st);
void launch_emfregs_merge(const bwams_alnreg_t *a, const int64_t *off_a, const bwams_alnreg_t *b, const int64_t *off_b, int64_t nseq,
                          const int64_t *off_o, bwams_alnreg_t *out, hipStream_t st);
void launch_emfregs_fill(const EmfRegArgs &A, const int64_t *scr_off, int32_t *n_final, uint8_t *first_is_rev, int64_t *wide,
                         hipStream_t st);
void launch_emfregs_emit(const EmfRegArgs &A, const int64_t *scr_off, const int32_t *n_final, const int64_t *out_off,
                         bwams_alnreg_t *out, hipStream_t st);

struct PairArgs {
    const bwams_alnreg_t *regs;
    const int64_t *reg_off;
    const uint8_t *enc;
    const int64_t *cum;
    int64_t nseq;
    const uint8_t *ref;
    DevBns bns;
    bwams_mem_opt_t opt;
    bwams_pestat_t pes[4];
    int64_t id_base;
    int32_t no_rescue, pass;
    int32_t drop_plan;
    int32_t use_ert;
    int32_t single_end;
    int32_t no_pairing;
    int32_t primary5_T;
    int32_t *na;
    const int64_t *aoff, *ooff;
    int32_t *anchor, *slot_read;
    int64_t n_slots;
    int32_t *task;
    int64_t *trb;
    int32_t *tl1;
    const int32_t *aln;
    bwams_alnreg_t *pool;
    int32_t *ord, *zbuf;
    void *srt;
    int32_t *n_fin, *n_pri, *n_sw;
    uint8_t *full;
    int32_t *heavy;
    DevCounters *ctr;
};
void launch_pair_count(const PairArgs &A, int64_t *wide, hipStream_t st);
void launch_pair_cap(const PairArgs &A, int64_t *wide, hipStream_t st);
void launch_pair_slots(const PairArgs &A, hipStream_t st);
void launch_pair_plan(const PairArgs &A, int64_t *wide, hipStream_t st);
void launch_pair_build(const PairArgs &A, const int64_t *offs, bwams_seqpair_t *pairs, uint8_t *tref, uint8_t *tqer, int cu_count,
                       hipStream_t st);
void launch_pair_post(const PairArgs &A, int cu_count, hipStream_t st);
void launch_pair_mark(const PairArgs &A, int cu_count, hipStream_t st);
void launch_pair_widen(const PairArgs &A, int64_t *wide, hipStream_t st);
void launch_pair_gather(const PairArgs &A, const int64_t *out_off, bwams_alnreg_t *out, hipStream_t st);
void launch_pair_reorder5(const PairArgs &A, const int64_t *out_off, bwams_alnreg_t *out, hipStream_t st);
void launch_pair_pair(const PairArgs &A, const int64_t *out_off, const bwams_alnreg_t *out, bwams_pair_t *res, hipStream_t st);

struct ErtArgs {
    const bwams_ert_mem_t *mems;
    const int64_t *mem_off;
    const uint64_t *hits;
    const int64_t *hit_off;
    int64_t nseq, n_mems, l_pac;
    int32_t max_occ, pad_;
    bwams_smem_t *smem_out;
    int64_t *cnt;
    void *srt;
// ... 69 lines not shown
```

bwa-mem-scale_amd/csrc/common.h:

```cpp
#pragma once

#include <cstdlib>
#include <hip/hip_runtime.h>
#include <mutex>
#include <stdint.h>
#include <stdio.h>
#include <string>
#include <vector>

#include "../../include/bwams.h"

namespace bwams {

void set_last_error(const std::string &s);

struct Knobs {
    int verbose = 0;
    int debug = 0;
    int poison = 0;
    int bwd_min_list = 40, bwd_cols = 24, bwd_late_list = 8;
    int bwd_dry_min_list = 24, bwd_dry_cols = 8, bwd_dry_late_list = 12;
    int r3_beside = 1;
    int ext_max_rounds = 0;
    int ext_all_rounds = 0;
    int ext_inplace = 1;
    int dedup_seq = 0;
    int pair_drop_plan = 0;
    int trace_pair = 0;
    int bsw_pk = 1;
    int chain_batch = 1;
    int ert_fat = 1;
    int ert_grid = -1, ert_ticket = 1;
};
const Knobs &knobs();
void knobs_reload();

template <class T> static inline hipError_t dev_malloc(T **p, size_t bytes) {
    const bool poison = knobs().poison != 0;
    hipError_t e = hipMalloc(reinterpret_cast<void **>(p), bytes);
    if (e == hipSuccess && poison && bytes) {
        e = hipMemset(*p, 0xAB, bytes);
        if (e == hipSuccess) e = hipDeviceSynchronize();
    }
    return e;
}

template <class T = void, bool Host = false> struct Buf {
    T *p = nullptr;
    size_t cap = 0;
    Buf() = default;
    Buf(Buf &&o) noexcept : p(o.p), cap(o.cap) { o.p = nullptr; o.cap = 0; }
    Buf &operator=(Buf &&o) noexcept {
        if (this != &o) { release(); p = o.p; cap = o.cap; o.p = nullptr; o.cap = 0; }
        return *this;
    }
    ~Buf() { release(); }
    template <class U> U *as() const { return reinterpret_cast<U *>(p); }
    void release() {
        if (p) (void)(Host ? hipHostFree(p) : hipFree(p));
        p = nullptr;
        cap = 0;
    }
    hipError_t alloc(size_t bytes) {
        release();
        hipError_t e = Host ? hipHostMalloc(&p, bytes, hipHostMallocDefault) : dev_malloc(&p, bytes);
        cap = p ? bytes : 0;
        return e;
    }
    hipError_t ensure(size_t bytes, size_t new_cap) { return bytes <= cap ? hipSuccess : alloc(new_cap); }
    hipError_t ensure(size_t bytes) { return ensure(bytes, bytes + bytes / 8 + 4096); }
    hipError_t ensure_n(size_t n) { return ensure(n * sizeof(T)); }
};
template <class T = void> using DevBuf = Buf<T, false>;
template <class T = void> using HostBuf = Buf<T, true>;

#define BWAMS_HIP(call)                                                                  \
    do {                                                                                 \
        hipError_t e_ = (call);                                                          \
        if (e_ != hipSuccess) {                                                          \
            char buf_[512];                                                              \
            snprintf(buf_, sizeof buf_, "%s:%d: %s -> %s", __FILE__, __LINE__, #call,    \
                     hipGetErrorString(e_));                                             \
            bwams::set_last_error(buf_);                                                 \
            return (e_ == hipErrorOutOfMemory) ? BWAMS_ERR_NOMEM : BWAMS_ERR_DEVICE;     \
        }                                                                                \
    } while (0)

struct DevFmi {
    const uint4 *cp;
    const uint4 *cp2;
    const int8_t *sa_ms;
    const uint32_t *sa_ls;
    const uint8_t *ref;
    const uint32_t *all_smem;
    const uint4 *last_smem;
    int32_t all_bp, last_bp;
    int64_t count[5];
    int64_t sentinel;
    int64_t ref_seq_len;
};

struct DevEmf {
    const uint4 *seed_table;
    const uint32_t *loc_table;
    const uint8_t *ref;
    uint32_t num_seed_entry, num_loc_entry, seq_len;
    int32_t seed_len;
};

struct DevErt {
    const uint64_t *kmer;
    const uint8_t *mlt;
    const uint8_t *ref;
    int64_t ref_len;
    int32_t K, X, read_len;
    uint64_t *cnt_tab;
    int32_t cnt_bits;
    const uint8_t *fat;
};

struct DevCounters {
    unsigned long long n_ext, n_ext_blocks, n_sa_lookups, n_lf_steps;
    unsigned long long n_smem_total;
    unsigned long long n_smem_valid;
    unsigned long long valid_after[3];
    unsigned long long n_after_r1, n_after_r2;
    unsigned long long work_head;
    unsigned long long n_work2;
    unsigned long long overflow;
    unsigned long long bsw_cells;
    unsigned long long bsw_head[4];
    unsigned long long bsw_cls_cnt[6], bsw_cls_head[6];
    unsigned long long ext_after[3], blk_after[3];
    unsigned long long emf_nodes, emf_cmp_bytes;
    unsigned long long chain_overflow;
    unsigned long long chain_longread;
    unsigned long long n_heavy;
    unsigned long long chain_class[10];
    unsigned long long chain_ticket[10];
    unsigned long long heavy_tickets[6];
    unsigned long long sel_heavy;
    unsigned long long ext_n_req;
    unsigned long long ext_n_rest;
    unsigned long long ext_n_tasks;
    unsigned long long ext_head[2];
    unsigned long long ext_sel_ticket[3];
    unsigned long long ext_n_retry[2];
    unsigned long long dedup_heavy, dedup_ticket, dedup_light;
    unsigned long long chain_redo, chain_redo_ticket;
    unsigned long long pair_heavy, pair_ticket;
    unsigned long long dbg[80];
    unsigned long long pair_ticket2;
    unsigned long long dedup_ticket2, dedup_ticket3;
    unsigned long long ert_kmer, ert_nodes, ert_ref;
    unsigned long long work_head3, n_ext3, n_blk3, n_smem3;
    unsigned long long ert_ticket;
    unsigned long long bwd_items, bwd_entries, bwd_ticket;
    unsigned long long bwd_items_s, bwd_ticket_s;
    unsigned long long pair_full, pair_fail;
};

struct StageState;
void chain_state_free(StageState *s);

struct BamArgs {
    const char *text;
    const int64_t *line_end, *read_off;
    int64_t n_rec, nseq;
    const char *ctg_names;
    const int32_t *ctg_off, *ctg_sorted;
    int32_t n_ctg;
    int64_t *size;
    const int64_t *rec_off;
    uint8_t *out;
    unsigned long long *bad;
};
void launch_bam_count(const BamArgs &A, int cu_count, hipStream_t st);
void launch_bam_write(const BamArgs &A, int64_t *bam_off, int cu_count, hipStream_t st);

int bam_sort_bits(uint32_t n_ref);
void launch_bam_sort_keys(const uint8_t *bam, const int64_t *rec_off, int64_t n_rec, uint32_t n_ref, bwams_bam_coord_t *coord,
                          uint64_t *dkey, uint32_t *idx, int cu_count, hipStream_t st);
void launch_bam_sort_permute(const bwams_bam_coord_t *coord, const uint32_t *idx, int64_t n_rec, bwams_bam_coord_t *coord_out,
                             int64_t *size, int cu_count, hipStream_t st);
void launch_bam_sort_gather(const uint8_t *src, const int64_t *rec_off, const uint32_t *idx, const int64_t *new_off, int64_t n_rec,
                            uint8_t *dst, int cu_count, hipStream_t st);

struct MdRec {
    int64_t c;
    int32_t rid;
    uint16_t flag, score;
};
struct MdTemplates {
    DevBuf<> head, tid, rtmpl, tstart, rec, tend, has, ends, info, tmp;
    int64_t n_t = 0, n_e = 0;
};
struct MdDecide {
    DevBuf<> k1, k2, ka, kb, i1, i2, info, tmp;
};
int md_templates(MdTemplates &m, const uint8_t *bam, const int64_t *rec_off, int64_t n_rec, int cu_count, hipStream_t st);
int md_decide(MdDecide &w, const bwams_dup_end_t *ends, int64_t n_e, int64_t n_t, uint8_t *dup, int64_t counts[3], int cu_count,
              hipStream_t st);
void launch_md_apply(uint8_t *bam, const int64_t *rec_off, const uint32_t *perm, const uint32_t *rtmpl, const uint8_t *dup, int64_t n_rec,
                     unsigned long long *n_marked, int cu_count, hipStream_t st);
void launch_md_gather32(const uint32_t *src, const uint32_t *idx, int64_t n, uint32_t *dst, int cu_count, hipStream_t st);

int deflater_device(const bwams_deflater *d);
int deflater_run_after(bwams_deflater *d, hipStream_t after, const void *in, int64_t n_bytes, int in_on_device, void *out, int64_t out_cap,
                       int out_on_device, int32_t flags, int64_t *n_out, bwams_deflate_stats_t *stats);

struct SwParams {
    int o_del, e_del, o_ins, e_ins, zdrop, end_bonus, max_sc;
    int8_t mat[25];
};

struct Round2Work {
    uint32_t rid;
    int32_t x;
    int32_t min_intv;
};

struct BwdItem {
    uint32_t rid;
    int32_t x;
    int32_t min_intv;
    int32_t num_prev;
    int64_t off;
};

int launch_bsw(bwams_seqpair_t *pairs, int64_t n, const uint8_t *ref, const uint8_t *qer, int w, const SwParams &prm, int qmax,
               DevCounters *ctr, int cu_count, hipStream_t st, int32_t *list, hipStream_t *aux = nullptr, hipEvent_t fork = nullptr,
               hipEvent_t *join = nullptr, const int64_t *src = nullptr, int dir = 1);
size_t bsw_list_bytes(int64_t n_tasks);
int bsw_lds_waves(int qmax);
void launch_emf_probe(const DevEmf &t, const uint8_t *enc, const int64_t *cum, int64_t nseq, uint32_t *out,
                      uint8_t *code, uint8_t *skip, DevCounters *ctr, hipStream_t st);
// ... 150 lines not shown
```

bwa-mem-scale_amd/csrc/dedup.hip:

```cpp
#include "common.h"
#include "chain_kernels.h"
#include "wave_ops.h"
#include "region_sort.h"

namespace bwams {
namespace {

constexpr int kLightN = 16;
constexpr int kSmallN = 128, kMidN = 512;
constexpr int kLdsN = 2048;
constexpr int MINUS_INF = -0x40000000;
constexpr int kEhLdsLen = 1000;
__host__ __device__ constexpr size_t dd_lds_bytes(int cap, int max_read_len) {
    return (size_t)60 * cap + (max_read_len <= kEhLdsLen ? (size_t)(max_read_len + 2) * 8 + (((size_t)max_read_len + 2 + 15) & ~(size_t)15) : 0);
}

__device__ int global_score(const bwams_mem_opt_t &o, int qlen, const uint8_t *qseq, int qs, int tlen, const uint8_t *tseq, int ts,
                            int w, int2 *eh) {
    const int oe_del = o.o_del + o.e_del, oe_ins = o.o_ins + o.e_ins;
    eh[0] = make_int2(0, MINUS_INF);
    int j;
    for (j = 1; j <= qlen && j <= w; ++j) eh[j] = make_int2(-(o.o_ins + o.e_ins * j), MINUS_INF);
    for (; j <= qlen; ++j) eh[j] = make_int2(MINUS_INF, MINUS_INF);
    for (int i = 0; i < tlen; ++i) {
// ... 272 lines not shown
    bwams_alnreg_t *a = A.regs + reg0;
    int32_t *ord = A.ord + reg0;
    const uint8_t *query = A.enc + A.cum[r];
    int n = 0;
    for (int i = 0; i < av_n; ++i)
        if (a[i].qe > a[i].qb) ord[n++] = i;
    if (n > 1) {
        for (int i = 0; i < n; ++i) { SortRec x; x.k = a[ord[i]].re; x.s = 0; x.q = 0; x.idx = ord[i]; x.pad_ = 0; srt[i] = x; }
        sort_records(srt, n, 0);
        for (int i = 0; i < n; ++i) { ord[i] = srt[i].idx; a[ord[i]].n_comp_is_alt = 1; }
        for (int i = 1; i < n; ++i) {
            bwams_alnreg_t *p = &a[ord[i]];
            const bwams_alnreg_t *pr = &a[ord[i - 1]];
            if (p->rid != pr->rid || p->rb >= pr->re + A.opt.max_chain_gap) continue;
            for (int j = i - 1; j >= 0; --j) {
                bwams_alnreg_t *q = &a[ord[j]];
                if (!(p->rid == q->rid && p->rb < q->re + A.opt.max_chain_gap)) break;
                if (q->qe == q->qb) continue;
                const int64_t or_ = q->re - p->rb;
                const int64_t oq = q->qb < p->qb ? q->qe - p->qb : p->qe - q->qb;
                const int64_t mr = q->re - q->rb < p->re - p->rb ? q->re - q->rb : p->re - p->rb;
                const int64_t mq = q->qe - q->qb < p->qe - p->qb ? q->qe - q->qb : p->qe - p->qb;
                int score, w;
                if ((float)or_ > A.opt.mask_level_redun * (float)mr && (float)oq > A.opt.mask_level_redun * (float)mq) {
                    if (p->score < q->score) { p->qe = p->qb; break; }
                    else q->qe = q->qb;
                } else if (q->rb < p->rb && (score = patch_reg<false>(A, query, *q, *p, &w, eh)) > 0) {
                    p->n_comp_is_alt = (p->n_comp_is_alt + q->n_comp_is_alt + 1) & 0x3fffffff;
                    p->seedcov = p->seedcov > q->seedcov ? p->seedcov : q->seedcov;
                    p->sub = p->sub > q->sub ? p->sub : q->sub;
                    p->csub = p->csub > q->csub ? p->csub : q->csub;
                    p->qb = q->qb; p->rb = q->rb;
                    p->truesc = p->score = score;
                    p->w = w;
                    q->qb = q->qe;
                }
            }
        }
        int m = 0;
        for (int i = 0; i < n; ++i)
            if (a[ord[i]].qe > a[ord[i]].qb) ord[m++] = ord[i];
        n = m;
        for (int i = 0; i < n; ++i) {
            const bwams_alnreg_t *p = &a[ord[i]];
            SortRec x; x.k = p->rb; x.s = p->score; x.q = p->qb; x.idx = ord[i]; x.pad_ = 0;
            srt[i] = x;
        }
        sort_records(srt, n, 1);
        for (int i = 0; i < n; ++i) ord[i] = srt[i].idx;
        for (int i = 1; i < n; ++i) {
            bwams_alnreg_t *p = &a[ord[i]];
            const bwams_alnreg_t *pr = &a[ord[i - 1]];
            if (p->score == pr->score && p->rb == pr->rb && p->qb == pr->qb) p->qe = p->qb;
        }
        m = n ? 1 : 0;
        for (int i = 1; i < n; ++i)
            if (a[ord[i]].qe > a[ord[i]].qb) ord[m++] = ord[i];
        n = m;
    }
    for (int i = 0; i < n; ++i) {
        bwams_alnreg_t *p = &a[ord[i]];
        if (p->rid >= 0 && A.bns.contigs[p->rid].is_alt) p->n_comp_is_alt = (p->n_comp_is_alt & 0x3fffffff) | (1 << 30);
    }
    return n;
}

__global__ void dedup_triage_kernel(DedupArgs A) {
    const int64_t r = (int64_t)blockIdx.x * blockDim.x + threadIdx.x;
    if (r >= A.nseq) return;
    const int64_t reg0 = A.seed_off[r];
    const int av_n = (int)(A.seed_off[r + 1] - reg0);
    bwams_alnreg_t *a = A.regs + reg0;
    int n = 0, last = 0;
    for (int i = 0; i < av_n; ++i)
        if (a[i].qe > a[i].qb) { last = i; ++n; }
    if (n <= 1) {
        if (n == 1) {
            A.ord[reg0] = last;
            if (a[last].rid >= 0 && A.bns.contigs[a[last].rid].is_alt) a[last].n_comp_is_alt = (a[last].n_comp_is_alt & 0x3fffffff) | (1 << 30);
        }
        A.n_out[r] = n;
        return;
    }
    if (av_n > kLightN) A.heavy[atomicAdd(A.n_heavy_ctr, 1ull)] = (int32_t)r;
    else A.light[atomicAdd(A.n_light_ctr, 1ull)] = (int32_t)r;
}

__global__ __launch_bounds__(64) void dedup_kernel(DedupArgs A, int64_t n_lanes) {
    const int64_t g = (int64_t)blockIdx.x * blockDim.x + threadIdx.x;
    if (g >= n_lanes) return;
    int2 *eh = A.eh + g * (int64_t)(A.max_read_len + 2);
    const int64_t n_light = (int64_t)*A.n_light_ctr;
    for (int64_t t = g; t < n_light; t += n_lanes) {
        const int64_t r = A.light[t];
        A.n_out[r] = dedup_read(A, r, reinterpret_cast<SortRec *>(A.srt) + A.seed_off[r], eh);
    }
}

__device__ __forceinline__ void load_qbqe(const bwams_alnreg_t *p, int &qb, int &qe) {
    const unsigned long long v = __hip_atomic_load(reinterpret_cast<const unsigned long long *>(&p->qb), __ATOMIC_RELAXED,
                                                   __HIP_MEMORY_SCOPE_AGENT);
    qb = (int)(uint32_t)v; qe = (int)(uint32_t)(v >> 32);
}
__device__ __forceinline__ int wave_compact_alive(const bwams_alnreg_t *a, int32_t *ord, int n_in, bool first, int lane) {
    int n = 0;
    for (int ib = 0; ib < n_in; ib += 64) {
        const int i = ib + lane;
        int slot = 0;
        bool alive = false;
        if (i < n_in) {
            slot = first ? i : ord[i];
            int qb, qe;
            load_qbqe(&a[slot], qb, qe);
            alive = qe > qb;
        }
        const unsigned long long m = __ballot(alive);
        if (alive) ord[n + __popcll(m & ((1ull << lane) - 1ull))] = slot;
        n += __popcll(m);
    }
    return n;
}

template <int CAP, int LO>
__global__ __launch_bounds__(64) void dedup_wave_kernel(DedupArgs A, int64_t n_waves, int64_t eh_base, unsigned long long *ticket) {
    extern __shared__ __align__(16) unsigned char lds_dd[];
    SortRec *l_srt = reinterpret_cast<SortRec *>(lds_dd), *l_srt2 = l_srt + CAP;
    int2 *lds_eh = A.max_read_len <= kEhLdsLen ? reinterpret_cast<int2 *>(lds_dd + (size_t)60 * CAP) : nullptr;
    uint8_t *lds_q = reinterpret_cast<uint8_t *>(lds_eh + (A.max_read_len + 2));
    int4 *l_x = reinterpret_cast<int4 *>(l_srt2);
    int64_t *l_rb = reinterpret_cast<int64_t *>(l_srt2 + CAP);
    int32_t *l_ord = reinterpret_cast<int32_t *>(l_rb + CAP);
    const int lane = threadIdx.x;
    int2 *eh = A.eh + (eh_base + blockIdx.x) * (int64_t)(A.max_read_len + 2);
    const int64_t n_heavy = (int64_t)*A.n_heavy_ctr;
    for (;;) {
        const int64_t t = (int64_t)wave_ticket(ticket, 1ull);
        if (t >= n_heavy) break;
        const int64_t r = A.heavy[t];
        const int64_t reg0 = A.seed_off[r];
        const int av_n = (int)(A.seed_off[r + 1] - reg0);
        if (av_n <= LO || (av_n > CAP && CAP != kLdsN)) continue;
        bwams_alnreg_t *a = A.regs + reg0;
        int32_t *ord = A.ord + reg0;
        const uint8_t *query = A.enc + A.cum[r];
        __syncthreads();
        if (av_n > kLdsN || A.force_seq == 1) {
            if (lane == 0) A.n_out[r] = dedup_read(A, r, reinterpret_cast<SortRec *>(A.srt) + reg0, eh);
            continue;
        }
        const bool prof = CAP == kLdsN && A.dbg != nullptr;
        unsigned long long n_al = 0, t_al = 0, n_it = 0;
        unsigned long long tk0 = prof ? wall_clock64() : 0ull, tk1 = tk0, tk2 = tk0, tk3 = tk0, tk4 = tk0, tk5 = tk0;
        int n = wave_compact_alive(a, l_ord, av_n, true, lane);
        const int n_alive0 = n;
        __syncthreads();
        if (n > 1) {
            for (int i = lane; i < n; i += 64) {
                const bwams_alnreg_t *p = &a[l_ord[i]];
                SortRec x; x.k = p->re; x.s = p->rid; x.q = 0; x.idx = l_ord[i]; x.pad_ = 0;
                l_srt[i] = x;
            }
            __syncthreads();
            if (prof) tk1 = wall_clock64();
            wave_sort_records(l_srt, l_srt2, n, 0, lane, false, 0, CAP);
            if (prof) tk2 = wall_clock64();
            for (int i = lane; i < n; i += 64) {
                const int slot = l_srt[i].idx;
                l_ord[i] = slot;
                l_rb[i] = a[slot].rb;
                a[slot].n_comp_is_alt = 1;
            }
            __threadfence_block();
            __syncthreads();
            for (int i = lane; i < n; i += 64) {
                const bwams_alnreg_t *p = &a[l_ord[i]];
                l_x[i] = make_int4(p->qb, p->qe, p->score, 0);
            }
            __syncthreads();
            const int64_t gap = A.opt.max_chain_gap, l_pac = A.bns.l_pac;
            const float mlr = A.opt.mask_level_redun;
            for (int i = 1; i < n; ++i) {
                const int rid_i = l_srt[i].s;
                if (rid_i != l_srt[i - 1].s || l_rb[i] >= l_srt[i - 1].k + gap) continue;
                int64_t p_rb = l_rb[i];
                const int64_t p_re = l_srt[i].k;
                int4 px = l_x[i];
                bool done = false;
                int jtop = i - 1;
                while (jtop >= 0 && !done) {
                    ++n_it;
                    const int j = jtop - lane;
                    bool end = j < 0, red = false, pat = false;
                    if (!end) {
                        const int64_t q_re = l_srt[j].k;
                        end = !(rid_i == l_srt[j].s && p_rb < q_re + gap);
                        if (!end) {
                            const int4 qx = l_x[j];
                            const int64_t q_rb = l_rb[j];
                            if (qx.y != qx.x) {
                                const int64_t or_ = q_re - p_rb;
                                const int64_t oq = qx.x < px.x ? qx.y - px.x : px.y - qx.x;
                                const int64_t mr = q_re - q_rb < p_re - p_rb ? q_re - q_rb : p_re - p_rb;
                                const int64_t mq = qx.y - qx.x < px.y - px.x ? qx.y - qx.x : px.y - px.x;
                                red = (float)or_ > mlr * (float)mr && (float)oq > mlr * (float)mq;
                                pat = !red && q_rb < p_rb && patch_geom(A.opt, l_pac, q_rb, q_re, qx.x, qx.y, p_rb, p_re, px.x, px.y);
                            }
                        }
                    }
                    const unsigned long long m_end = __ballot(end), m_red = __ballot(red);
                    unsigned long long ev = m_end | m_red | __ballot(pat);
                    int consumed = 64;
                    while (ev) {
                        const int l = __builtin_ctzll(ev);
                        ev &= ev - 1;
                        if ((m_end >> l) & 1) { done = true; break; }
                        const int jj = jtop - l;
                        bwams_alnreg_t *pp = &a[l_ord[i]], *qq = &a[l_ord[jj]];
                        if ((m_red >> l) & 1) {
                            if (px.z < l_x[jj].z) {
                                px.y = px.x;
                                if (lane == 0) { pp->qe = px.x; l_x[i] = px; }
                                done = true;
                                break;
                            }
                            if (lane == 0) { const int qb = l_x[jj].x; qq->qe = qb; l_x[jj].y = qb; }
                            continue;
                        }
                        int score = 0, w = 0;
                        const unsigned long long ta0 = prof ? wall_clock64() : 0ull;
                        if (lds_eh) {
                            const bwams_alnreg_t qa = *qq, pa = *pp;
                            score = patch_reg<true>(A, query, qa, pa, &w, lds_eh, lds_q, lane);
                        } else if (lane == 0) score = patch_reg<false>(A, query, *qq, *pp, &w, eh);
                        if (prof) { t_al += wall_clock64() - ta0; ++n_al; }
                        score = __builtin_amdgcn_readfirstlane(score);
                        w = __builtin_amdgcn_readfirstlane(w);
                        if (score > 0) {
                            __syncthreads();
                            const int4 qx = l_x[jj];
                            p_rb = l_rb[jj];
                            px.x = qx.x; px.z = score;
                            __syncthreads();
                            if (lane == 0) {
                                pp->n_comp_is_alt = (pp->n_comp_is_alt + qq->n_comp_is_alt + 1) & 0x3fffffff;
                                pp->seedcov = pp->seedcov > qq->seedcov ? pp->seedcov : qq->seedcov;
                                pp->sub = pp->sub > qq->sub ? pp->sub : qq->sub;
                                pp->csub = pp->csub > qq->csub ? pp->csub : qq->csub;
                                pp->qb = qq->qb; pp->rb = qq->rb;
                                pp->truesc = pp->score = score;
                                pp->w = w;
                                qq->qb = qq->qe;
                                l_rb[i] = p_rb; l_x[i] = px; l_x[jj].x = qx.y;
                            }
                            consumed = l + 1;
                            break;
                        }
                    }
                    __syncthreads();
                    jtop -= consumed;
                }
            }
            __threadfence_block();
            __syncthreads();
            if (prof) tk3 = wall_clock64();
            n = wave_compact_alive(a, l_ord, n, false, lane);
            __syncthreads();
            for (int i = lane; i < n; i += 64) {
                const bwams_alnreg_t *p = &a[l_ord[i]];
                SortRec x;
                x.k = (int64_t)__hip_atomic_load(reinterpret_cast<const unsigned long long *>(&p->rb), __ATOMIC_RELAXED, __HIP_MEMORY_SCOPE_AGENT);
                x.s = __hip_atomic_load(&p->score, __ATOMIC_RELAXED, __HIP_MEMORY_SCOPE_AGENT);
                int qb, qe;
                load_qbqe(p, qb, qe);
                x.q = qb; x.idx = l_ord[i]; x.pad_ = 0;
                l_srt[i] = x;
            }
            __syncthreads();
            if (prof) tk4 = wall_clock64();
            wave_sort_records(l_srt, l_srt2, n, 1, lane, false, 0, CAP);
            if (prof) tk5 = wall_clock64();
            int m = 0;
            for (int ib = 0; ib < n; ib += 64) {
                const int i = ib + lane;
                bool keep = false;
                int slot = 0;
                if (i < n) {
                    const SortRec x = l_srt[i];
                    slot = x.idx;
                    keep = i == 0 || !(x.s == l_srt[i - 1].s && x.k == l_srt[i - 1].k && x.q == l_srt[i - 1].q);
                    if (!keep) a[slot].qe = a[slot].qb;
                }
                const unsigned long long mk = __ballot(keep);
                if (keep) l_ord[m + __popcll(mk & ((1ull << lane) - 1ull))] = slot;
                m += __popcll(mk);
            }
            n = m;
            __threadfence_block();
            __syncthreads();
        }
        for (int i = lane; i < n; i += 64) {
            bwams_alnreg_t *p = &a[l_ord[i]];
            ord[i] = l_ord[i];
            const int nc = __hip_atomic_load(&p->n_comp_is_alt, __ATOMIC_RELAXED, __HIP_MEMORY_SCOPE_AGENT);
            if (p->rid >= 0 && A.bns.contigs[p->rid].is_alt) p->n_comp_is_alt = (nc & 0x3fffffff) | (1 << 30);
        }
        if (lane == 0) A.n_out[r] = n;
        if (prof && lane == 0) {
            const unsigned long long tk6 = wall_clock64();
            atomicAdd(&A.dbg[0], 1ull); atomicAdd(&A.dbg[1], (unsigned long long)av_n); atomicAdd(&A.dbg[2], (unsigned long long)n_alive0);
            atomicAdd(&A.dbg[3], tk1 - tk0); atomicAdd(&A.dbg[4], tk2 - tk1); atomicAdd(&A.dbg[5], tk3 - tk2);
            atomicAdd(&A.dbg[6], tk4 - tk3); atomicAdd(&A.dbg[7], tk5 - tk4); atomicAdd(&A.dbg[8], tk6 - tk5);
            atomicMax(&A.dbg[9], tk2 - tk1); atomicMax(&A.dbg[10], tk3 - tk2); atomicMax(&A.dbg[11], tk5 - tk4);
            if (atomicMax(&A.dbg[12], tk6 - tk0) < tk6 - tk0) { A.dbg[13] = (unsigned long long)r; A.dbg[14] = (unsigned long long)n_alive0; A.dbg[15] = n_al; A.dbg[16] = t_al; A.dbg[17] = n_it; }
            atomicAdd(&A.dbg[18], n_al); atomicAdd(&A.dbg[19], t_al);
        }
    }
}

static_assert(sizeof(bwams_alnreg_t) == 112, "a region is seven 16-byte pieces");
__global__ __launch_bounds__(256) void dedup_gather_kernel(DedupArgs A, const int64_t *__restrict__ out_off, bwams_alnreg_t *out) {
    const int64_t r = ((int64_t)blockIdx.x * blockDim.x + threadIdx.x) >> 4;
    const int sub = threadIdx.x & 15;
    if (r >= A.nseq) return;
    const int64_t reg0 = A.seed_off[r];
    const int n = A.n_out[r];
    if (n <= 0) return;
    const int64_t o0 = out_off[r];
    const uint4 *src = reinterpret_cast<const uint4 *>(A.regs + reg0);
    uint4 *dst = reinterpret_cast<uint4 *>(out + o0);
    for (int u = sub; u < n * 7; u += 16) {
        const int i = u / 7, piece = u - 7 * i;
        dst[u] = src[(int64_t)A.ord[reg0 + i] * 7 + piece];
    }
}

__device__ __forceinline__ int cal_sub(const bwams_mem_opt_t &opt, int n, const bwams_alnreg_t *a) {
    int j;
    for (j = 1; j < n; ++j) {
        const int b_max = a[j].qb > a[0].qb ? a[j].qb : a[0].qb;
        const int e_min = a[j].qe < a[0].qe ? a[j].qe : a[0].qe;
        if (e_min > b_max) {
            const int lj = a[j].qe - a[j].qb, l0 = a[0].qe - a[0].qb;
            const int min_l = lj < l0 ? lj : l0;
            if ((float)(e_min - b_max) >= (float)min_l * opt.mask_level) break;
        }
    }
    return j < n ? a[j].score : opt.min_seed_len * opt.a;
}
__global__ void pestat_kernel(const bwams_alnreg_t *__restrict__ regs, const int64_t *__restrict__ reg_off, int64_t n_pairs,
                              int64_t l_pac, bwams_mem_opt_t opt, unsigned long long *keys) {
    const int64_t i = (int64_t)blockIdx.x * blockDim.x + threadIdx.x;
    if (i >= n_pairs) return;
    unsigned long long key = ~0ull;
    const int64_t o0 = reg_off[2 * i], o1 = reg_off[2 * i + 1], o2 = reg_off[2 * i + 2];
    const int n0 = (int)(o1 - o0), n1 = (int)(o2 - o1);
    if (n0 && n1) {
        const bwams_alnreg_t *r0 = regs + o0, *r1 = regs + o1;
        if (!((double)cal_sub(opt, n0, r0) > 0.8 * (double)r0[0].score) && !((double)cal_sub(opt, n1, r1) > 0.8 * (double)r1[0].score) &&
            r0[0].rid == r1[0].rid) {
            const int64_t b1 = r0[0].rb, b2 = r1[0].rb;
            const int s1 = b1 >= l_pac, s2 = b2 >= l_pac;
            const int64_t p2 = s1 == s2 ? b2 : (l_pac << 1) - 1 - b2;
            const int64_t is = p2 > b1 ? p2 - b1 : b1 - p2;
            const int dir = (s1 == s2 ? 0 : 1) ^ (p2 > b1 ? 0 : 3);
            if (is && is <= opt.max_ins) key = ((unsigned long long)dir << 60) | (unsigned long long)is;
        }
    }
    keys[i] = key;
}

constexpr int kTestN = 1024;
__global__ __launch_bounds__(64) void sort_test_kernel(const SortRec *__restrict__ in, int n, int by_score, int mode, int32_t *__restrict__ order,
                                                       SortRec *__restrict__ scratch) {
    __shared__ SortRec l_a[kTestN], l_t[kTestN];
    const int lane = threadIdx.x;
    if (mode == 2 || mode == 4) {
        for (int i = lane; i < n; i += 64) scratch[i] = in[i];
        __syncthreads();
        if (lane == 0) sort_records(scratch, n, by_score, mode == 4 ? 2 : 0);
        __syncthreads();
        for (int i = lane; i < n; i += 64) order[i] = scratch[i].idx;
        return;
    }
    for (int i = lane; i < n; i += 64) l_a[i] = in[i];
    __syncthreads();
    wave_sort_records(l_a, l_t, n, by_score, lane, mode == 1 || mode == 3, mode == 3 ? 2 : 0, kTestN);
    for (int i = lane; i < n; i += 64) order[i] = l_a[i].idx;
}

}

int launch_sort_test(const int64_t *k, const int32_t *s_, const int32_t *q, int n, int by_score, int mode, int32_t *order) {
    if (n < 0 || n > kTestN) return -1;
    SortRec *h = (SortRec *)malloc(sizeof(SortRec) * (size_t)(n + 1));
    for (int i = 0; i < n; ++i) { h[i].k = k[i]; h[i].s = s_[i]; h[i].q = q[i]; h[i].idx = i; h[i].pad_ = 0; }
    int rc = -1;
    {
        DevBuf<SortRec> d_in, d_scr;
        DevBuf<int32_t> d_ord;
        if (d_in.alloc(sizeof(SortRec) * (size_t)(n + 1)) == hipSuccess && d_ord.alloc(4 * (size_t)(n + 1)) == hipSuccess &&
            d_scr.alloc(sizeof(SortRec) * (size_t)(n + 1)) == hipSuccess &&
            hipMemcpy(d_in.p, h, sizeof(SortRec) * (size_t)n, hipMemcpyHostToDevice) == hipSuccess) {
            sort_test_kernel<<<1, 64>>>(d_in.p, n, by_score, mode, d_ord.p, d_scr.p);
            if (hipDeviceSynchronize() == hipSuccess && hipMemcpy(order, d_ord.p, 4 * (size_t)n, hipMemcpyDeviceToHost) == hipSuccess) rc = 0;
        }
    }
    free(h);
    return rc;
}

void launch_pestat(const bwams_alnreg_t *regs, const int64_t *reg_off, int64_t n_pairs, int64_t l_pac, const bwams_mem_opt_t &opt,
                   unsigned long long *keys, hipStream_t st) {
    if (n_pairs <= 0) return;
    pestat_kernel<<<(unsigned)((n_pairs + 255) / 256), 256, 0, st>>>(regs, reg_off, n_pairs, l_pac, opt, keys);
}

size_t dedup_sortrec_bytes(int64_t n) { return (size_t)(n + 1) * sizeof(SortRec); }

int launch_dedup(const DedupArgs &A, int64_t n_lanes, int64_t n_waves, int64_t n_waves_small, hipStream_t st, hipStream_t aux,
                 hipStream_t aux2, hipStream_t aux3, hipEvent_t fork, hipEvent_t join, hipEvent_t join2, hipEvent_t join3) {
    if (A.nseq <= 0) return 0;
    dedup_triage_kernel<<<(unsigned)((A.nseq + 255) / 256), 256, 0, st>>>(A);
    if (hipEventRecord(fork, st) != hipSuccess || hipStreamWaitEvent(aux, fork, 0) != hipSuccess) return -1;
    if (hipFuncSetAttribute(reinterpret_cast<const void *>(dedup_wave_kernel<kLdsN, kMidN>), hipFuncAttributeMaxDynamicSharedMemorySize, (int)dd_lds_bytes(kLdsN, A.max_read_len)) != hipSuccess) return -1;
    dedup_wave_kernel<kLdsN, kMidN><<<(unsigned)n_waves, 64, dd_lds_bytes(kLdsN, A.max_read_len), st>>>(A, n_waves, A.eh_lanes, A.ticket);
    dedup_kernel<<<(unsigned)((n_lanes + 63) / 64), 64, 0, aux>>>(A, n_lanes);
    if (hipEventRecord(join, aux) != hipSuccess || hipStreamWaitEvent(st, join, 0) != hipSuccess) return -1;
    if (hipStreamWaitEvent(aux3, fork, 0) != hipSuccess) return -1;
    dedup_wave_kernel<kMidN, kSmallN><<<(unsigned)n_waves, 64, dd_lds_bytes(kMidN, A.max_read_len), aux3>>>(A, n_waves, A.eh_lanes + n_waves, A.ticket3);
    if (hipEventRecord(join3, aux3) != hipSuccess || hipStreamWaitEvent(st, join3, 0) != hipSuccess) return -1;
    if (hipStreamWaitEvent(aux2, fork, 0) != hipSuccess) return -1;
    dedup_wave_kernel<kSmallN, kLightN><<<(unsigned)n_waves_small, 64, dd_lds_bytes(kSmallN, A.max_read_len), aux2>>>(A, n_waves_small, A.eh_lanes + 2 * n_waves, A.ticket2);
    if (hipEventRecord(join2, aux2) != hipSuccess || hipStreamWaitEvent(st, join2, 0) != hipSuccess) return -1;
    return 0;
}
void launch_dedup_gather(const DedupArgs &A, const int64_t *out_off, bwams_alnreg_t *out, hipStream_t st) {
    if (A.nseq <= 0) return;
    dedup_gather_kernel<<<(unsigned)((A.nseq * 16 + 255) / 256), 256, 0, st>>>(A, out_off, out);
}

}
```

bwa-mem-scale_amd/csrc/stage_state.h:

```cpp
#pragma once

#include "chain_kernels.h"

namespace bwams {

struct StageState {
    struct ChainStage {
        DevBuf<int32_t> s_next, f_first, f_kept, f_sel; DevBuf<int2> s_ql; DevBuf<uint2> flt; DevBuf<uint4> f_rec;
        DevBuf<> crec, nodes;
        DevBuf<int32_t> n_kept, n_kept_seeds, n_chn, redo; DevBuf<int64_t> read_base; DevBuf<float> frac;
        DevBuf<uint32_t> okeys, okeys2, ovals, ovals2;
        DevBuf<> wide, chain_off;
        DevBuf<> slice;
        DevBuf<bwams_chain_t> chains; DevBuf<bwams_chain_seed_t> seeds, seeds2;
        DevBuf<int32_t> sw_qb, sw_read, sw_newn; DevBuf<int64_t> sw_rb; DevBuf<bwams_kswr_t> sw_res;
        DevBuf<bwams_ert_mem_t> et_mems; DevBuf<int64_t> et_moff, et_hoff, et_cnt, et_off, et_coord; DevBuf<uint64_t> et_hits;
        DevBuf<bwams_smem_t> et_smem;
        DevBuf<> et_srt;
        int64_t n_chains = 0, n_seeds = 0, nseq = 0, n_redo = 0; bool done = false;
    } ch;
    struct ExtStage {
        DevBuf<bwams_alnreg_t> regs; DevBuf<uint32_t> srt; DevBuf<int32_t> state, cur, lim;
        DevBuf<> rmax;
        DevBuf<> cnt;
        DevBuf<> ewide, eoffs;
        DevBuf<> kreg;
        DevBuf<bwams_seqpair_t> lpairs, rpairs, retry; DevBuf<uint8_t> lref, lqer, rref, rqer;
        DevBuf<> lsrc, rsrc;
        DevBuf<int32_t> req_list, rtask;
        int64_t n_left = 0, n_right = 0, lref_b = 0, lqer_b = 0, rref_b = 0, rqer_b = 0, n_retry_left = 0, n_retry_right = 0, n_rounds = 0;
        bool tasks_inplace = false, built = false, done = false;
    } ext;
    struct DedupStage {
        DevBuf<bwams_alnreg_t> regs, out; DevBuf<int32_t> ord, nout, light;
        DevBuf<> srt;
        DevBuf<> eh;
        DevBuf<> wide;
        DevBuf<int64_t> off; DevBuf<unsigned long long> pe_keys, pe_keys2;
        int64_t n_final = 0; bool done = false;
    } dd;
    struct PairStage {
        DevBuf<int32_t> na, anchor, slot, task, tl1, ord, z, nfin, npri, nsw; DevBuf<int64_t> wide, trb, owide, ooff;
        DevBuf<> offs;
        DevBuf<> twide, toffs;
        DevBuf<bwams_seqpair_t> pairs; DevBuf<uint8_t> tref, tqer, full;
        DevBuf<> aln;
        DevBuf<bwams_alnreg_t> pool, out;
        DevBuf<> srt;
        DevBuf<bwams_pair_t> res;
        int64_t total = 0, tasks = 0, redone = 0; bool done = false, single = false;
    } pr;
    struct EmfRegStage {
        DevBuf<int64_t> wide, off, ooff, mg_wide, mg_off;
        DevBuf<> scr;
        DevBuf<int32_t> n; DevBuf<uint8_t> rev; DevBuf<bwams_alnreg_t> out, mg_out;
        int64_t total = 0, nseq = 0; bool done = false;
    } er;
    struct AlnStage {
        DevBuf<int64_t> need, off; DevBuf<int32_t> cls; DevBuf<uint8_t> scr, only;
        DevBuf<> list;
        DevBuf<bwams_aln_t> rec;
        DevBuf<> wide, offs;
        DevBuf<uint32_t> cig; DevBuf<char> md; DevBuf<unsigned long long> cnt;
        int64_t n = 0, ncig = 0, nmd = 0; int source = 0; bool done = false;
    } al;
    struct SamStage {
        DevBuf<char> names, qual, comm, out; DevBuf<int64_t> noff, coff, len, off; DevBuf<int32_t> mapq; DevBuf<double> logtab;
        DevBuf<> bad;
        int64_t bytes = 0, nseq = 0, nregs = 0;
        int64_t merged_n = -1;
        bool up = false, has_qual = false, has_comm = false, done = false, log_ok = false;
    } sm;
    struct BamStage {
        DevBuf<int64_t> size, roff, off; DevBuf<uint8_t> out; DevBuf<unsigned long long> bad;
        int64_t bytes = 0, nrec = 0, nseq = 0;
        uint32_t nref = 0;
        bool done = false;
    } bm;
    struct BamSortStage {
        DevBuf<uint8_t> out; DevBuf<bwams_bam_coord_t> coord, coord0; DevBuf<uint64_t> keys, keys2; DevBuf<uint32_t> idx, idx2;
        DevBuf<int64_t> size, off;
        int64_t bytes = 0, nrec = 0; bool done = false;
    } bs;
    struct MarkdupStage {
        MdTemplates t;
        MdDecide decide;
        DevBuf<uint8_t> dup; DevBuf<unsigned long long> cnt; DevBuf<uint32_t> sorted;
        bool done = false;
    } md;
    DevBuf<int32_t> heavy;
    bwams_mem_opt_t opt{};
    hipEvent_t ev[16] = {};
    bool ev_ok = false;
    hipStream_t aux[7] = {};
    int aux_device = -1;
    hipEvent_t fork = nullptr, join[7] = {};
};

enum class From { chain, built, dedup, pair, al, er, sam_upload, sam, bam };
void outdated(StageState *s, From first);

int get_state(bwams_batch *b, StageState **out);
// ... 9 lines not shown
```

include/bwams.h:

```cpp
#ifndef BWAMS_H
#define BWAMS_H

#include <stddef.h>
#include <stdint.h>
#include "bwams_types.h"

#ifdef __cplusplus
extern "C" {
#endif

#define BWAMS_OK               0
#define BWAMS_ERR_DEVICE      -1
#define BWAMS_ERR_IO          -2
#define BWAMS_ERR_ARG         -3
#define BWAMS_ERR_CAPACITY    -4
#define BWAMS_ERR_NOMEM       -5
#define BWAMS_ERR_UNSUPPORTED -6

typedef struct bwams_index bwams_index_t;
typedef struct bwams_batch bwams_batch_t;
typedef struct bwams_emf bwams_emf_t;

const char *bwams_strerror(int code);
const char *bwams_last_error(void);
// ... 126 lines not shown


int bwams_reg2aln_run(bwams_batch_t *b, const bwams_mem_opt_t *opt, int32_t source, int64_t *n_aln, int64_t *n_cigar_ops,
                      int64_t *md_bytes);
int bwams_reg2aln_run_sam(bwams_batch_t *b, const bwams_mem_opt_t *opt, const bwams_sam_opt_t *sopt, const bwams_pestat_t *pes,
                          int64_t *n_aln, int64_t *n_needed, int64_t *n_cigar_ops, int64_t *md_bytes);
int bwams_reg2aln_fetch(bwams_batch_t *b, bwams_aln_t *aln, int64_t aln_cap, uint32_t *cigar, int64_t cigar_cap, char *md,
                        int64_t md_cap);

int bwams_index_set_contig_names(bwams_index_t *ix, const char *names, const int32_t *name_off);
int bwams_index_set_contig_annos(bwams_index_t *ix, const char *annos, const int32_t *anno_off);
int bwams_sam_upload(bwams_batch_t *b, const char *names, const int64_t *name_off, const char *quals, const char *comments,
                     const int64_t *comment_off);
int bwams_sam_run(bwams_batch_t *b, const bwams_mem_opt_t *opt, const bwams_sam_opt_t *sopt, int64_t *sam_bytes);
int bwams_sam_run_emf(bwams_batch_t *b, const bwams_mem_opt_t *opt, const bwams_sam_opt_t *sopt, bwams_emf_t *emf, int64_t *sam_bytes);
int bwams_sam_run_pe(bwams_batch_t *b, const bwams_mem_opt_t *opt, const bwams_sam_opt_t *sopt, const bwams_pestat_t pes[4],
                     int64_t *sam_bytes);
int bwams_sam_fetch(bwams_batch_t *b, char *sam, int64_t cap, int64_t *read_off, int32_t *mapq, int64_t mapq_cap);
int bwams_sam_fetch_bgzf(bwams_batch_t *b, bwams_deflater_t *d, void *out, int64_t cap, int32_t flags, int64_t *n_out);

int bwams_bam_run(bwams_batch_t *b, int64_t *bam_bytes, int64_t *n_records);
int bwams_bam_fetch(bwams_batch_t *b, void *bam, int64_t cap, int64_t *read_off);
int bwams_bam_fetch_bgzf(bwams_batch_t *b, bwams_deflater_t *d, void *out, int64_t cap, int32_t flags, int64_t *n_out);
int bwams_bam_upload(bwams_batch_t *b, const void *bam, int64_t n_bytes, int64_t *n_records);
int bwams_bam_sort(bwams_batch_t *b, int64_t *n_records);
int bwams_bam_sorted_fetch(bwams_batch_t *b, void *bam, int64_t cap, bwams_bam_coord_t *coords);
int bwams_bam_templates(bwams_batch_t *b, int64_t *n_templates, int64_t *n_ends);
int bwams_bam_templates_fetch(bwams_batch_t *b, bwams_dup_end_t *ends, int64_t cap, uint32_t *rec_tmpl, int32_t sorted);
int bwams_dup_decide(int device, const bwams_dup_end_t *ends, int64_t n_ends, int64_t n_templates, uint8_t *dup, bwams_dup_stats_t *st);
int bwams_bam_markdup(bwams_batch_t *b, bwams_dup_stats_t *st);
int bwams_sam_header(const bwams_index_t *idx, const char *hdr_line, const char *pg_line, char *out, int64_t cap, int64_t *n_out);
int bwams_bam_header(const bwams_index_t *idx, const char *text, int64_t n_text, void *out, int64_t cap, int64_t *n_out);

typedef struct bwams_fastq bwams_fastq_t;
int bwams_fastq_decode(int device, const char *text, int64_t n_bytes, bwams_fastq_t **out, int64_t *n_reads, int64_t *n_bases);
int bwams_fastq_info(const bwams_fastq_t *f, int64_t *n_reads, int64_t *n_bases, int64_t *name_bytes, int64_t *comment_bytes, float *ms);
int bwams_fastq_has_qual(const bwams_fastq_t *f);
int bwams_fastq_fetch(bwams_fastq_t *f, uint8_t *enc, int64_t *cum, char *names, int64_t *name_off, char *quals, char *comments,
                      int64_t *comment_off);
int bwams_fastq_to_batch(bwams_fastq_t *f, bwams_batch_t *b);
int bwams_fastq_to_batch_opt(bwams_fastq_t *f, bwams_batch_t *b, int32_t copy_comment);
int bwams_fastq_close(bwams_fastq_t *f);


int bwams_ksw_align(bwams_batch_t *b, const bwams_seqpair_t *pairs, int64_t n,
                    const uint8_t *ref, int64_t ref_bytes, const uint8_t *qer, int64_t qer_bytes,
                    const bwams_sw_opt_t *opt, bwams_kswr_t *out);

int bwams_debug_sort(bwams_index_t *idx, const int64_t *k, const int32_t *s, const int32_t *q, int32_t n, int32_t which,
                     int32_t mode, int32_t *order_out);


typedef struct bwams_stats {
    int64_t n_ext;
    int64_t n_ext_blocks;
    int64_t n_sa_lookups;
    int64_t n_lf_steps;
    int64_t n_smem[3];
    int64_t bsw_cells;
    int64_t n_ext_round[3];
    int64_t n_blk_round[3];
    float   ms_smem_r1, ms_smem_r2, ms_smem_r3, ms_sort, ms_sal, ms_seed_total;
    float   ms_bsw;
    float   ms_ksw;
    float   ms_tasks;
    float   ms_emf;
    int64_t emf_nodes;
    int64_t emf_cmp_bytes;
    int64_t n_chains, n_chain_seeds;
    int64_t n_left, n_right;
    int64_t n_retry_left, n_retry_right;
    float   ms_chain, ms_ext_plan, ms_ext_left, ms_ext_right, ms_ext_purge, ms_ext_total;
    int64_t n_ext_rounds;
    int64_t n_final_regs;
    float   ms_dedup;
    float   ms_pair;
    int64_t n_pair_tasks;
    int64_t n_pair_redone;
    int64_t n_pair_regs;
    int64_t n_chain_redo;
    int64_t ert_kmer_lookups;
    int64_t ert_node_reads;
    int64_t ert_ref_bytes;
} bwams_stats_t;
int bwams_batch_stats(bwams_batch_t *b, bwams_stats_t *out);

typedef struct bwams_ert bwams_ert_t;

int bwams_ert_from_host(bwams_index_t *idx, const uint64_t *kmer_table, int32_t kmer_size, int32_t xmer_size,
                        int32_t read_len, const uint8_t *mlt_table, int64_t mlt_bytes, bwams_ert_t **out);
int bwams_ert_open(bwams_index_t *idx, const char *prefix, int32_t read_len, bwams_ert_t **out);
int bwams_ert_build(bwams_index_t *idx, int32_t kmer_size, int32_t xmer_size, int32_t read_len, int32_t hit_threshold,
                    bwams_ert_t **out);
int bwams_ert_info(const bwams_ert_t *ert, int32_t *kmer_size, int32_t *xmer_size, int32_t *read_len, int64_t *mlt_bytes,
                   float build_ms[3]);
int bwams_ert_fetch(bwams_ert_t *ert, uint64_t *kmer_table, uint8_t *mlt_table);
int bwams_ert_save(bwams_ert_t *ert, const char *prefix);
int bwams_ert_close(bwams_ert_t *ert);
int64_t bwams_ert_bytes(const bwams_ert_t *ert);
int bwams_ert_set_fat(bwams_ert_t *ert, int32_t on);

int bwams_seed_run_ert(bwams_batch_t *b, bwams_ert_t *ert, const bwams_seed_opt_t *opt, int with_sa);


int bwams_index_set_contigs(bwams_index_t *idx, const bwams_contig_t *contigs, int32_t n_seqs);

int bwams_chain_run(bwams_batch_t *b, const bwams_mem_opt_t *opt, int64_t *n_chains, int64_t *n_seeds);
int bwams_chain_run_ert(bwams_batch_t *b, const bwams_mem_opt_t *opt, const bwams_ert_mem_t *mems, const int64_t *mem_off,
                        const uint64_t *hits, const int64_t *hit_off, int64_t *n_chains, int64_t *n_seeds);
int bwams_chain_fetch(bwams_batch_t *b, bwams_chain_t *chains, int64_t chain_cap, bwams_chain_seed_t *seeds,
                      int64_t seed_cap, int64_t *chain_off);
int bwams_chain_upload(bwams_batch_t *b, const bwams_chain_t *chains, int64_t n_chains, const bwams_chain_seed_t *seeds,
                       int64_t n_seeds, const int64_t *chain_off);

int bwams_extend_build(bwams_batch_t *b, const bwams_mem_opt_t *opt, int64_t *n_left, int64_t *n_right);
int bwams_extend_run(bwams_batch_t *b, const bwams_mem_opt_t *opt, int64_t *n_regs);
int bwams_extend_fetch(bwams_batch_t *b, bwams_alnreg_t *regs, int64_t reg_cap, int64_t *reg_off, int32_t *seed_aln);
int bwams_dedup_run(bwams_batch_t *b, const bwams_mem_opt_t *opt, int64_t *n_regs);
int bwams_dedup_fetch(bwams_batch_t *b, bwams_alnreg_t *regs, int64_t reg_cap, int64_t *reg_off);
int bwams_emf_regs_run(bwams_batch_t *b, bwams_emf_t *emf, const bwams_mem_opt_t *opt, int64_t *n_regs);
int bwams_emf_regs_merge(bwams_batch_t *b, int64_t *n_regs);
int bwams_emf_regs_fetch(bwams_batch_t *b, bwams_alnreg_t *regs, int64_t reg_cap, int64_t *reg_off, uint8_t *first_is_rev);

int bwams_pestat(bwams_batch_t *b, const bwams_mem_opt_t *opt, bwams_pestat_t pes[4]);
int bwams_pestat_keys(bwams_batch_t *b, const bwams_mem_opt_t *opt, uint64_t *keys, int64_t cap, int64_t *n_keys);
int bwams_pestat_from_keys(const uint64_t *keys, int64_t n, bwams_pestat_t pes[4]);
#define BWAMS_PAIR_NO_RESCUE 1
#define BWAMS_PAIR_SINGLE_END 4
#define BWAMS_PAIR_USE_ERT   2
int bwams_pair_run(bwams_batch_t *b, const bwams_mem_opt_t *opt, const bwams_pestat_t pes[4], int64_t id_base, int32_t flags,
                   int64_t *n_regs, int64_t *n_tasks);
int bwams_pair_run_sam(bwams_batch_t *b, const bwams_mem_opt_t *opt, const bwams_sam_opt_t *sam_opt, const bwams_pestat_t pes[4],
                       int64_t id_base, int32_t flags, int64_t *n_regs, int64_t *n_tasks);
int bwams_pair_fetch(bwams_batch_t *b, bwams_alnreg_t *regs, int64_t reg_cap, int64_t *reg_off, bwams_pair_t *pairs);
int bwams_extend_tasks_fetch(bwams_batch_t *b, int32_t side, bwams_seqpair_t *pairs, int64_t pair_cap, uint8_t *ref,
                             int64_t ref_cap, uint8_t *qer, int64_t qer_cap, int64_t *n_pairs, int64_t *ref_bytes,
                             int64_t *qer_bytes);

int bwams_batch_sync(bwams_batch_t *b);

int bwams_process_chunk(bwams_batch_t *b, bwams_emf_t *emf, bwams_ert_t *ert, const bwams_seed_opt_t *so, const bwams_mem_opt_t *mo,
                        const bwams_sam_opt_t *sam_opt, const char *fastq, int64_t n_bytes, int32_t paired, const bwams_pestat_t *pes0,
                        int64_t n_processed, int32_t flags, int64_t *n_reads, int64_t *sam_bytes);
int bwams_process_chunk2(bwams_batch_t *b, bwams_emf_t *emf, bwams_ert_t *ert, const bwams_seed_opt_t *so, const bwams_mem_opt_t *mo,
                         const bwams_sam_opt_t *sam_opt, const char *fastq1, int64_t n_bytes1, const char *fastq2, int64_t n_bytes2,
                         const bwams_pestat_t *pes0, int64_t n_processed, int32_t flags, int64_t *n_reads, int64_t *sam_bytes);
int bwams_process_chunk_smart(bwams_batch_t *b, bwams_emf_t *emf, bwams_ert_t *ert, const bwams_seed_opt_t *so, const bwams_mem_opt_t *mo,
                              const bwams_sam_opt_t *sam_opt, const char *fastq, int64_t n_bytes, const bwams_pestat_t *pes0,
                              int64_t n_processed, int32_t flags, int64_t *n_reads, int64_t *n_single, int64_t *sam_bytes);
#define BWAMS_CHUNK_COPY_COMMENT 0x100

int bwams_process_reads(bwams_batch_t *b, bwams_emf_t *emf, bwams_ert_t *ert, const bwams_seed_opt_t *so, const bwams_mem_opt_t *mo,
                        const bwams_sam_opt_t *sam_opt, const uint8_t *enc_qdb, const int64_t *cum_len, int64_t n_reads, const char *names,
                        const int64_t *name_off, const char *quals, const char *comments, const int64_t *comment_off, int32_t paired,
                        const bwams_pestat_t *pes0, int64_t n_processed, int32_t flags, int64_t *sam_bytes);
int bwams_process_reads_stage1(bwams_batch_t *b, bwams_emf_t *emf, bwams_ert_t *ert, const bwams_seed_opt_t *so, const bwams_mem_opt_t *mo,
                               const uint8_t *enc_qdb, const int64_t *cum_len, int64_t n_reads, const char *names, const int64_t *name_off,
                               const char *quals, const char *comments, const int64_t *comment_off);
int bwams_process_reads_stage2(bwams_batch_t *b, bwams_emf_t *emf, bwams_ert_t *ert, const bwams_mem_opt_t *mo, const bwams_sam_opt_t *sam_opt,
                               int32_t paired, const bwams_pestat_t *pes, int64_t id_base, int32_t flags, int64_t *sam_bytes);
int bwams_process_reads_upload(bwams_batch_t *b, const uint8_t *enc_qdb, const int64_t *cum_len, int64_t n_reads, const char *names,
                               const int64_t *name_off, const char *quals, const char *comments, const int64_t *comment_off);
int bwams_process_reads_stage1_run(bwams_batch_t *b, bwams_emf_t *emf, bwams_ert_t *ert, const bwams_seed_opt_t *so, const bwams_mem_opt_t *mo);
int bwams_batch_device(const bwams_batch_t *b, int32_t *device);
typedef struct bwams_multi bwams_multi_t;
int bwams_shard_bounds(int64_t n_reads, int32_t n_shards, int32_t paired, int64_t *bounds );
// ... 51 lines not shown
```

Baseline: 9.906.

## Bucket heavy chain and dedup reads into per-class lists instead of filtering

Heavy reads in chain and dedup are now appended to separate per-size-class lists, with one counter and ticket per class, instead of a single shared list that each class kernel scanned while skipping reads outside its range. The wave and heavy kernels take a list of classes and drain them in order, so waves no longer fetch and discard work meant for other classes. A new plan knob (off by default) also allows a single-stream dedup launch and an alternative chain schedule. The cost is more counters and a larger heavy buffer (six or three strides), plus per-class stats exposed through the API.

New measurement: 10.42, median of 6. 1.05x the previous value.

```diff
diff --git a/bwa-mem-scale_amd/bwams/capi.py b/bwa-mem-scale_amd/bwams/capi.py
--- a/bwa-mem-scale_amd/bwams/capi.py
+++ b/bwa-mem-scale_amd/bwams/capi.py
@@ -173,7 +173,8 @@
                 ("ms_ext_right", C.c_float), ("ms_ext_purge", C.c_float), ("ms_ext_total", C.c_float),
                 ("n_ext_rounds", C.c_int64), ("n_final_regs", C.c_int64), ("ms_dedup", C.c_float), ("ms_pair", C.c_float),
                 ("n_pair_tasks", C.c_int64), ("n_pair_redone", C.c_int64), ("n_pair_regs", C.c_int64), ("n_chain_redo", C.c_int64),
-                ("ert_kmer_lookups", C.c_int64), ("ert_node_reads", C.c_int64), ("ert_ref_bytes", C.c_int64)]
+                ("ert_kmer_lookups", C.c_int64), ("ert_node_reads", C.c_int64), ("ert_ref_bytes", C.c_int64),
+                ("n_chain_heavy", C.c_int64 * 6)]
 
 
 class BuildStats(C.Structure):
diff --git a/bwa-mem-scale_amd/csrc/api.hip b/bwa-mem-scale_amd/csrc/api.hip
--- a/bwa-mem-scale_amd/csrc/api.hip
+++ b/bwa-mem-scale_amd/csrc/api.hip
@@ -37,6 +37,7 @@
     k.trace_pair = env_int("BWAMS_TRACE_PAIR", 0);
     k.bsw_pk = env_int("BWAMS_BSW_PK", 1);
     k.chain_batch = env_int("BWAMS_CHAIN_BATCH", 1);
+    k.chain_plan = env_int("BWAMS_CHAIN_PLAN", 0) == 1;
     k.ert_ticket = env_int("BWAMS_ERT_TICKET", 1); k.ert_grid = env_int("BWAMS_ERT_GRID", -1); k.ert_fat = env_int("BWAMS_ERT_FAT", 1);
     g_knobs = k;
 }
diff --git a/bwa-mem-scale_amd/csrc/api_chain.hip b/bwa-mem-scale_amd/csrc/api_chain.hip
--- a/bwa-mem-scale_amd/csrc/api_chain.hip
+++ b/bwa-mem-scale_amd/csrc/api_chain.hip
@@ -172,7 +172,7 @@
     BWAMS_HIP(s->ch.s_next.ensure_n(ns)); BWAMS_HIP(s->ch.s_ql.ensure_n(ns)); BWAMS_HIP(s->ch.crec.ensure(chain_rec_bytes(n_sa)));
     BWAMS_HIP(s->ch.flt.ensure_n(ns)); BWAMS_HIP(s->ch.f_rec.ensure_n(ns)); BWAMS_HIP(s->ch.f_first.ensure_n(ns));
     BWAMS_HIP(s->ch.f_kept.ensure_n(ns)); BWAMS_HIP(s->ch.f_sel.ensure_n(ns)); BWAMS_HIP(s->ch.n_chn.ensure_n((size_t)n1));
-    BWAMS_HIP(s->heavy.ensure_n((size_t)n1)); BWAMS_HIP(s->ch.redo.ensure_n((size_t)n1)); BWAMS_HIP(s->ch.slice.ensure((size_t)n1 * 16));
+    BWAMS_HIP(s->heavy.ensure_n((size_t)n1 * 6)); BWAMS_HIP(s->ch.redo.ensure_n((size_t)n1)); BWAMS_HIP(s->ch.slice.ensure((size_t)n1 * 16));
     BWAMS_HIP(s->ch.okeys.ensure_n((size_t)n1)); BWAMS_HIP(s->ch.okeys2.ensure_n((size_t)n1)); BWAMS_HIP(s->ch.ovals.ensure_n((size_t)n1));
     BWAMS_HIP(s->ch.ovals2.ensure_n((size_t)n1)); BWAMS_HIP(s->ch.nodes.ensure(chain_node_bytes(n_sa, nseq)));
     BWAMS_HIP(s->ch.n_kept.ensure_n((size_t)n1)); BWAMS_HIP(s->ch.n_kept_seeds.ensure_n((size_t)n1)); BWAMS_HIP(s->ch.read_base.ensure_n((size_t)n1));
@@ -184,12 +184,12 @@
     A.opt = *opt;
     A.s_next = s->ch.s_next.p; A.s_ql = s->ch.s_ql.p; A.crec = s->ch.crec.p; A.flt = s->ch.flt.p; A.f_rec = s->ch.f_rec.p;
     A.f_first = s->ch.f_first.p; A.f_kept = s->ch.f_kept.p; A.f_sel = s->ch.f_sel.p; A.nodes = s->ch.nodes.p; A.n_kept = s->ch.n_kept.p;
-    A.n_kept_seeds = s->ch.n_kept_seeds.p; A.n_chn = s->ch.n_chn.p; A.heavy = s->heavy.p; A.redo = s->ch.redo.p; A.slice = s->ch.slice.as<int64_t>();
+    A.n_kept_seeds = s->ch.n_kept_seeds.p; A.n_chn = s->ch.n_chn.p; A.heavy = s->heavy.p; A.heavy_stride = n1; A.redo = s->ch.redo.p; A.slice = s->ch.slice.as<int64_t>();
     A.order = s->ch.ovals2.p; A.read_base = s->ch.read_base.p; A.frac_rep = s->ch.frac.p; A.ctr = b->d_ctr.p; A.seed_batch = knobs().chain_batch;
 
     BWAMS_HIP(hipEventRecord(s->ev[0], st));
     BWAMS_HIP(hipMemsetAsync(&b->d_ctr.p->chain_redo, 0, 2 * sizeof(unsigned long long), st));
-    BWAMS_HIP(hipMemsetAsync(&b->d_ctr.p->chain_overflow, 0, 29 * sizeof(unsigned long long), st));
+    BWAMS_HIP(hipMemsetAsync(&b->d_ctr.p->chain_overflow, 0, 34 * sizeof(unsigned long long), st));
     if ((sv.one_smem_quirk ? sv.n_smem <= 1 : sv.n_smem <= 0) || n_sa == 0) {
         BWAMS_HIP(hipMemsetAsync(s->ch.n_kept.p, 0, (size_t)n1 * 4, st));
         BWAMS_HIP(hipMemsetAsync(s->ch.n_kept_seeds.p, 0, (size_t)n1 * 4, st));
@@ -198,7 +198,7 @@
         if ((rc = with_tmp(b, "bwams_chain_run: radix_sort_pairs_desc", [&](void *tmp, size_t &tb) {
                 return rocprim::radix_sort_pairs_desc(tmp, tb, s->ch.okeys.p, s->ch.okeys2.p, s->ch.ovals.p, s->ch.ovals2.p, (size_t)nseq, 0, 32, st);
             }))) return rc;
-        if (launch_chain(A, s->ch.okeys.p, b->cu_count, st, s->aux, s->fork, s->join)) {
+        if (launch_chain(A, s->ch.okeys.p, b->cu_count, knobs().chain_plan, st, s->aux, s->fork, s->join)) {
             set_last_error("bwams_chain_run: stream fork/join failed");
             return BWAMS_ERR_DEVICE;
         }
@@ -237,6 +237,7 @@
     }
     const bool has_long = b->h_ctr.p->chain_longread != 0;
     s->ch.n_redo = (int64_t)b->h_ctr.p->chain_redo;
+    for (int c = 0; c < 6; ++c) s->ch.n_heavy[c] = (int64_t)b->h_ctr.p->n_heavy[c];
     s->ch.n_chains = tot[0]; s->ch.n_seeds = tot[1]; s->ch.nseq = nseq;
     BWAMS_HIP(s->ch.chains.ensure_n((size_t)(tot[0] + 1))); BWAMS_HIP(s->ch.seeds.ensure_n((size_t)(tot[1] + 1)));
     if (tot[0] > 0) launch_chain_emit(A, s->ch.chain_off.as<int64_t>(), s->ch.chain_off.as<int64_t>() + n1, s->ch.chains.p, s->ch.seeds.p, st);
diff --git a/bwa-mem-scale_amd/csrc/api_regions.hip b/bwa-mem-scale_amd/csrc/api_regions.hip
--- a/bwa-mem-scale_amd/csrc/api_regions.hip
+++ b/bwa-mem-scale_amd/csrc/api_regions.hip
@@ -37,20 +37,21 @@
     if ((rc = dev_bns(b->idx, &D.bns))) return rc;
     D.opt = *opt; D.ord = s->dd.ord.p; D.srt = s->dd.srt.p; D.eh = s->dd.eh.as<int2>(); D.eh_lanes = n_lanes; D.max_read_len = (int32_t)L;
     D.n_out = s->dd.nout.p;
-    BWAMS_HIP(s->heavy.ensure_n((size_t)n1));
+    BWAMS_HIP(s->heavy.ensure_n((size_t)n1 * 3));
     D.force_seq = knobs().dedup_seq;
     BWAMS_HIP(s->dd.light.ensure_n((size_t)n1));
-    D.heavy = s->heavy.p; D.light = s->dd.light.p; D.n_heavy_ctr = &b->d_ctr.p->dedup_heavy; D.ticket = &b->d_ctr.p->dedup_ticket;
-    D.n_light_ctr = &b->d_ctr.p->dedup_light; D.ticket2 = &b->d_ctr.p->dedup_ticket2; D.ticket3 = &b->d_ctr.p->dedup_ticket3;
+    D.heavy = s->heavy.p; D.heavy_stride = n1; D.light = s->dd.light.p; D.n_light_ctr = &b->d_ctr.p->dedup_light;
+    D.n_heavy_ctr[0] = &b->d_ctr.p->dedup_heavy; D.n_heavy_ctr[1] = &b->d_ctr.p->dedup_heavy3; D.n_heavy_ctr[2] = &b->d_ctr.p->dedup_heavy2;
+    D.ticket[0] = &b->d_ctr.p->dedup_ticket; D.ticket[1] = &b->d_ctr.p->dedup_ticket3; D.ticket[2] = &b->d_ctr.p->dedup_ticket2;
     const bool verbose_dd = knobs().verbose != 0;
     D.dbg = verbose_dd ? b->d_ctr.p->dbg : nullptr;
     if (verbose_dd) BWAMS_HIP(hipMemsetAsync(b->d_ctr.p->dbg, 0, sizeof b->d_ctr.p->dbg, st));
     BWAMS_HIP(hipMemsetAsync(&b->d_ctr.p->dedup_heavy, 0, 3 * sizeof(unsigned long long), st));
-    BWAMS_HIP(hipMemsetAsync(&b->d_ctr.p->dedup_ticket2, 0, 2 * sizeof(unsigned long long), st));
+    BWAMS_HIP(hipMemsetAsync(&b->d_ctr.p->dedup_ticket2, 0, 4 * sizeof(unsigned long long), st));
     BWAMS_HIP(hipEventRecord(s->ev[12], st));
     if (N) BWAMS_HIP(hipMemcpyAsync(D.regs, s->ext.regs.p, (size_t)N * sizeof(bwams_alnreg_t), hipMemcpyDeviceToDevice, st));
     BWAMS_HIP(hipMemsetAsync(D.n_out, 0, (size_t)n1 * 4, st));
-    if (launch_dedup(D, n_lanes, n_waves, n_waves_small, st, s->aux[0], s->aux[1], s->aux[2], s->fork, s->join[0], s->join[1], s->join[2])) {
+    if (launch_dedup(D, n_lanes, n_waves, n_waves_small, knobs().chain_plan, st, s->aux[0], s->aux[1], s->aux[2], s->fork, s->join[0], s->join[1], s->join[2])) {
         set_last_error("bwams_dedup_run: stream fork/join failed");
         return BWAMS_ERR_DEVICE;
     }
diff --git a/bwa-mem-scale_amd/csrc/api_state.hip b/bwa-mem-scale_amd/csrc/api_state.hip
--- a/bwa-mem-scale_amd/csrc/api_state.hip
+++ b/bwa-mem-scale_amd/csrc/api_state.hip
@@ -132,6 +132,7 @@
 void chain_state_stats(const StageState *s, bwams_stats_t *out) {
     if (!s) return;
     out->n_chains = s->ch.n_chains; out->n_chain_seeds = s->ch.n_seeds; out->n_chain_redo = s->ch.n_redo;
+    for (int c = 0; c < 6; ++c) out->n_chain_heavy[c] = s->ch.n_heavy[c];
     out->n_left = s->ext.n_left; out->n_right = s->ext.n_right;
     out->n_retry_left = s->ext.n_retry_left; out->n_retry_right = s->ext.n_retry_right;
     auto el = [&](int a, int b, float *dst) {
diff --git a/bwa-mem-scale_amd/csrc/chain.hip b/bwa-mem-scale_amd/csrc/chain.hip
--- a/bwa-mem-scale_amd/csrc/chain.hip
+++ b/bwa-mem-scale_amd/csrc/chain.hip
@@ -815,6 +815,7 @@
 
 __device__ void heavy_read(const ChainArgs &A, int64_t r, int64_t base, int n_chn, unsigned char *lds, int cap, int lane);
 __host__ __device__ constexpr size_t heavy_lds_bytes(int cap);
+__device__ __forceinline__ int heavy_class(int n_chn);
 template <bool LDS, int CONT = 0, bool CREC_HBM = false>
 __device__ __forceinline__ bool chain_read(const ChainArgs &A, int64_t r, int lane, int nl, Node *nodes, int32_t cap_nodes,
                                            ChainRec *crec_w, int32_t cap_chains) {
@@ -1044,8 +1045,9 @@
     if (!wr) return true;
     A.n_chn[r] = n_chn;
     if (n_chn > kLightChains) {
-        const unsigned long long slot = atomicAdd(&A.ctr->n_heavy, 1ull);
-        A.heavy[slot] = (int32_t)r;
+        const int hc = heavy_class(n_chn);
+        const unsigned long long slot = atomicAdd(&A.ctr->n_heavy[hc], 1ull);
+        A.heavy[hc * A.heavy_stride + (int64_t)slot] = (int32_t)r;
         return true;
     }
     flt_introsort(fl, n_chn);
@@ -1068,35 +1070,40 @@
     chain_read<false>(A, r, 0, 1, nullptr, 0, nullptr, 0);
 }
 
-__global__ __launch_bounds__(64) __attribute__((amdgpu_waves_per_eu(3, 3))) void chain_wave_kernel(ChainArgs A, const unsigned long long *lo_p, const unsigned long long *hi_p,
-                                                        unsigned long long *ticket, int K) {
+constexpr int kMaxList = 7;
+struct ClassList { int n; int lo[kMaxList], hi[kMaxList], tk[kMaxList]; };
+
+__global__ __launch_bounds__(64) __attribute__((amdgpu_waves_per_eu(3, 3))) void chain_wave_kernel(ChainArgs A, ClassList C, int K) {
     extern __shared__ __align__(16) unsigned char l_mem[];
     const int lane = threadIdx.x;
-    const int64_t lo = lo_p ? (int64_t)*lo_p : 0, hi = (int64_t)*hi_p;
     ChainRec *l_crec = reinterpret_cast<ChainRec *>(l_mem);
     Node *l_nodes = reinterpret_cast<Node *>(l_mem + (size_t)(K > 0 ? K : 0) * sizeof(ChainRec));
-    for (;;) {
-        const unsigned long long t = wave_ticket(ticket, 1ull);
-        if (lo + (int64_t)t >= hi) break;
-        const int64_t r = (int64_t)A.order[lo + (int64_t)t];
+    for (int e = 0; e < C.n; ++e) {
+        const int64_t lo = C.lo[e] < 0 ? 0 : (int64_t)A.ctr->chain_class[C.lo[e]], hi = (int64_t)A.ctr->chain_class[C.hi[e]];
+        unsigned long long *ticket = &A.ctr->chain_ticket[C.tk[e]];
+        for (;;) {
+            const unsigned long long t = wave_ticket(ticket, 1ull);
+            if (lo + (int64_t)t >= hi) break;
+            const int64_t r = (int64_t)A.order[lo + (int64_t)t];
 #ifdef BWAMS_CHAINDBG
-        const unsigned long long tk0 = wall_clock64();
+            const unsigned long long tk0 = wall_clock64();
 #endif
-        if (K < 0) {
-            if (!chain_read<true, 1, true>(A, r, lane, 64, reinterpret_cast<Node *>(l_mem), 0, nullptr, -K) && lane == 0)
-                A.redo[atomicAdd(&A.ctr->chain_redo, 1ull)] = (int32_t)r;
-        } else if (K) {
-            if (!chain_read<true, 1>(A, r, lane, 64, l_nodes, 0, l_crec, K) && lane == 0)
-                A.redo[atomicAdd(&A.ctr->chain_redo, 1ull)] = (int32_t)r;
-        } else chain_read<false>(A, r, lane, 64, nullptr, 0, nullptr, 0);
-        __syncthreads();
+            if (K < 0) {
+                if (!chain_read<true, 1, true>(A, r, lane, 64, reinterpret_cast<Node *>(l_mem), 0, nullptr, -K) && lane == 0)
+                    A.redo[atomicAdd(&A.ctr->chain_redo, 1ull)] = (int32_t)r;
+            } else if (K) {
+                if (!chain_read<true, 1>(A, r, lane, 64, l_nodes, 0, l_crec, K) && lane == 0)
+                    A.redo[atomicAdd(&A.ctr->chain_redo, 1ull)] = (int32_t)r;
+            } else chain_read<false>(A, r, lane, 64, nullptr, 0, nullptr, 0);
+            __syncthreads();
 #ifdef BWAMS_CHAINDBG
-        if (lane == 0) {
-            const int c = K < 0 ? 0 : K == kClassL ? 1 : K == kClassL2 ? 2 : K == kClassL1 ? 3 : K == kClassM2 ? 4 : K == kClassM ? 5 : K == kClassM1 ? 6 : 7;
-            const unsigned long long dt = wall_clock64() - tk0;
-            atomicAdd(&A.ctr->dbg[32 + 3 * c], 1ull); atomicAdd(&A.ctr->dbg[33 + 3 * c], dt); atomicMax(&A.ctr->dbg[34 + 3 * c], dt);
-        }
+            if (lane == 0) {
+                const int c = K < 0 ? 0 : K == kClassL ? 1 : K == kClassL2 ? 2 : K == kClassL1 ? 3 : K == kClassM2 ? 4 : K == kClassM ? 5 : K == kClassM1 ? 6 : 7;
+                const unsigned long long dt = wall_clock64() - tk0;
+                atomicAdd(&A.ctr->dbg[32 + 3 * c], 1ull); atomicAdd(&A.ctr->dbg[33 + 3 * c], dt); atomicMax(&A.ctr->dbg[34 + 3 * c], dt);
+            }
 #endif
+        }
     }
 }
 
@@ -1111,6 +1118,9 @@
 }
 
 constexpr int kHeavyCap[6] = {64, 128, 256, 512, 960, 3840};
+__device__ __forceinline__ int heavy_class(int n_chn) {
+    return n_chn <= kHeavyCap[0] ? 0 : n_chn <= kHeavyCap[1] ? 1 : n_chn <= kHeavyCap[2] ? 2 : n_chn <= kHeavyCap[3] ? 3 : n_chn <= kHeavyCap[4] ? 4 : 5;
+}
 __host__ __device__ constexpr size_t heavy_lds_bytes(int cap) { return (size_t)cap * 41 + 64; }
 static_assert(heavy_lds_bytes(kHeavyCap[5]) <= 160 * 1024, "the largest class must fit one CU's LDS");
 
@@ -1258,37 +1268,39 @@
     }
 }
 
-__global__ __launch_bounds__(64) void chain_heavy_kernel(ChainArgs A, const unsigned long long *n_heavy_p, int cap_lo, int cap,
-                                                         unsigned long long *ticket) {
+struct HeavyList { int n; int cls[6]; };
+__global__ __launch_bounds__(64) void chain_heavy_kernel(ChainArgs A, HeavyList C, int cap) {
     extern __shared__ __align__(16) unsigned char l_heavy[];
-    const int kLdsChains = cap;
     const int lane = threadIdx.x;
-    const int64_t n_heavy = (int64_t)*n_heavy_p;
-    for (;;) {
-        const int64_t hi = (int64_t)wave_ticket(ticket, 1ull);
-        if (hi >= n_heavy) break;
-        const int64_t r = A.heavy[hi];
-        const int64_t base = A.read_base[r];
-        const int n_chn = A.n_chn[r];
-        if (n_chn <= cap_lo || (n_chn > cap && cap != kHeavyCap[5])) continue;
-        const int L = (int)(A.cum[r + 1] - A.cum[r]);
-        uint2 *fl = A.flt + base;
-        uint4 *rec = A.f_rec + base;
-        int32_t *kept = A.f_kept + base;
-        const ChainRec *crec = reinterpret_cast<const ChainRec *>(A.crec) + base;
-        if (n_chn > kLdsChains) {
-            const unsigned long long t_0 = __builtin_amdgcn_s_memtime();
-            if (lane == 0) {
-                atomicAdd(&A.ctr->dbg[6], 1ull);
-                flt_introsort(fl, n_chn);
-                for (int i = 0; i < n_chn; ++i) { rec[i] = make_rec(A, crec[fl[i].y], fl[i].x); kept[i] = 0; }
-                filter_seq(A.opt, n_chn, rec, kept, A.f_sel + base);
-                finish_read(A, r, base, n_chn, L);
-                atomicAdd(&A.ctr->dbg[7], __builtin_amdgcn_s_memtime() - t_0);
-            }
-            continue;
-        }
-        heavy_read(A, r, base, n_chn, l_heavy, cap, lane);
+    for (int e = 0; e < C.n; ++e) {
+        const int c = C.cls[e];
+        const int64_t n_heavy = (int64_t)A.ctr->n_heavy[c];
+        const int32_t *list = A.heavy + c * A.heavy_stride;
+        for (;;) {
+            const int64_t hi = (int64_t)wave_ticket(&A.ctr->heavy_tickets[c], 1ull);
+            if (hi >= n_heavy) break;
+            const int64_t r = list[hi];
+            const int64_t base = A.read_base[r];
+            const int n_chn = A.n_chn[r];
+            if (n_chn > cap) {
+                const int L = (int)(A.cum[r + 1] - A.cum[r]);
+                uint2 *fl = A.flt + base;
+                uint4 *rec = A.f_rec + base;
+                int32_t *kept = A.f_kept + base;
+                const ChainRec *crec = reinterpret_cast<const ChainRec *>(A.crec) + base;
+                const unsigned long long t_0 = __builtin_amdgcn_s_memtime();
+                if (lane == 0) {
+                    atomicAdd(&A.ctr->dbg[6], 1ull);
+                    flt_introsort(fl, n_chn);
+                    for (int i = 0; i < n_chn; ++i) { rec[i] = make_rec(A, crec[fl[i].y], fl[i].x); kept[i] = 0; }
+                    filter_seq(A.opt, n_chn, rec, kept, A.f_sel + base);
+                    finish_read(A, r, base, n_chn, L);
+                    atomicAdd(&A.ctr->dbg[7], __builtin_amdgcn_s_memtime() - t_0);
+                }
+                continue;
+            }
+            heavy_read(A, r, base, n_chn, l_heavy, cap, lane);
+        }
     }
 }
 
@@ -1362,47 +1374,106 @@
     if (A.n_smem > 0) chain_slice_kernel<<<(unsigned)((A.n_smem + 255) / 256), 256, 0, st>>>(A);
     chain_count_kernel<<<(unsigned)((A.nseq + 255) / 256), 256, 0, st>>>(A, keys, vals);
 }
-int launch_chain(const ChainArgs &A, const uint32_t *n_seeds, int cu_count, hipStream_t st, hipStream_t *aux,
+namespace {
+
+struct WaveClass { int lo, hi, tk, K; size_t lds; };
+enum { cHBM, cXL2, cXL, cL, cL2, cL1, cM2, cM, cM1, cS, cLane };
+constexpr WaveClass kWave[10] = {
+    {-1, 9, 0, 0, 0},
+    {9, 6, 9, -kClassXL2, lds_bytes_xl(kClassXL2)}, {6, 0, 6, -kClassXL, lds_bytes_xl(kClassXL)},
+    {0, 7, 1, kClassL, lds_bytes(kClassL)}, {7, 1, 7, kClassL2, lds_bytes(kClassL2)}, {1, 8, 2, kClassL1, lds_bytes(kClassL1)},
+    {8, 2, 8, kClassM2, lds_bytes(kClassM2)}, {2, 3, 3, kClassM, lds_bytes(kClassM)}, {3, 4, 4, kClassM1, lds_bytes(kClassM1)},
+    {4, 5, 5, kClassS, lds_bytes(kClassS)}};
+
+struct PlanRow { int first, last, per_cu, lane; };
+constexpr int wave_mode(int c) { return c == cHBM ? 0 : c <= cXL ? 1 : 2; }
+template <size_t N> constexpr bool wave_rows_ok(const PlanRow (&r)[N]) {
+    for (size_t i = 0; i < N; ++i) {
+        if (r[i].per_cu <= 0 || r[i].lane < 0 || r[i].lane > 3) return false;
+        if (r[i].first == cLane) continue;
+        if (r[i].first < 0 || r[i].first > r[i].last || r[i].last > cS || r[i].last - r[i].first + 1 > kMaxList) return false;
+        if (wave_mode(r[i].first) != wave_mode(r[i].last)) return false;
+    }
+    for (int c = cHBM; c <= cLane; ++c) {
+        bool covered = false;
+        for (size_t i = 0; i < N; ++i) covered = covered || (c == cLane ? r[i].first == cLane : r[i].first != cLane && r[i].first <= c && c <= r[i].last);
+        if (!covered) return false;
+    }
+    return true;
+}
+template <size_t N> constexpr bool heavy_rows_ok(const PlanRow (&r)[N]) {
+    for (size_t i = 0; i < N; ++i)
+        if (r[i].per_cu <= 0 || r[i].lane < 0 || r[i].lane > 3 || r[i].first > 5 || r[i].last < 0 || r[i].first < r[i].last) return false;
+    for (int c = 0; c <= 5; ++c) {
+        bool covered = false;
+        for (size_t i = 0; i < N; ++i) covered = covered || (r[i].last <= c && c <= r[i].first);
+        if (!covered) return false;
+    }
+    return true;
+}
+
+constexpr PlanRow kWavePlan[] = {
+    {cXL2, cXL, 1, 0}, {cHBM, cHBM, 8, 0}, {cL1, cM2, 3, 0}, {cM1, cS, 8, 0},
+    {cL, cL2, 1, 1}, {cLane, cLane, 1, 1},
+    {cL2, cL1, 2, 2}, {cM, cM1, 5, 2},
+    {cS, cS, 12, 3}, {cM2, cM, 4, 3}};
+constexpr PlanRow kHeavyPlan[] = {{5, 4, 1, 0}, {4, 3, 4, 1}, {3, 2, 7, 2}, {2, 1, 12, 3}, {1, 0, 16, 1}, {0, 0, 24, 2}};
+constexpr PlanRow kWaveSerial[] = {{cXL2, cXL, 1, 0}, {cHBM, cHBM, 8, 0}, {cL, cS, 1, 0}, {cLane, cLane, 1, 0}};
+constexpr PlanRow kHeavySerial[] = {{5, 0, 1, 0}};
+static_assert(wave_rows_ok(kWavePlan) && wave_rows_ok(kWaveSerial) && heavy_rows_ok(kHeavyPlan) && heavy_rows_ok(kHeavySerial), "a plan row its list cannot hold, or a class no row covers");
+
+void launch_wave_row(const ChainArgs &A, const PlanRow &w, const uint32_t *n_seeds, int cu_count, hipStream_t s) {
+    if (w.first == cLane) {
+        chain_kernel<<<(unsigned)((A.nseq + 63) / 64), 64, 0, s>>>(A, n_seeds);
+        return;
+    }
+    ClassList C = {};
+    for (int c = w.first; c <= w.last; ++c, ++C.n) { C.lo[C.n] = kWave[c].lo; C.hi[C.n] = kWave[c].hi; C.tk[C.n] = kWave[c].tk; }
+    chain_wave_kernel<<<(unsigned)(cu_count * w.per_cu), 64, kWave[w.first].lds, s>>>(A, C, kWave[w.first].K);
+}
+void launch_heavy_row(const ChainArgs &A, const PlanRow &w, int cu_count, hipStream_t s) {
+    HeavyList C = {};
+    for (int c = w.first; c >= w.last; --c) C.cls[C.n++] = c;
+    chain_heavy_kernel<<<(unsigned)(cu_count * w.per_cu), 64, heavy_lds_bytes(kHeavyCap[w.first]), s>>>(A, C, kHeavyCap[w.first]);
+}
+template <size_t N> void launch_wave_rows(const ChainArgs &A, const PlanRow (&rows)[N], const uint32_t *n_seeds, int cu_count, const hipStream_t *lane) {
+    for (const PlanRow &w : rows) launch_wave_row(A, w, n_seeds, cu_count, lane[w.lane]);
+}
+template <size_t N> void launch_heavy_rows(const ChainArgs &A, const PlanRow (&rows)[N], int cu_count, const hipStream_t *lane) {
+    for (const PlanRow &w : rows) launch_heavy_row(A, w, cu_count, lane[w.lane]);
+}
+int fork_lanes(hipStream_t st, hipStream_t *aux, hipEvent_t fork) {
+    if (hipEventRecord(fork, st) != hipSuccess) return -1;
+    for (int i = 0; i < 3; ++i)
+        if (hipStreamWaitEvent(aux[i], fork, 0) != hipSuccess) return -1;
+    return 0;
+}
+int join_lanes(hipStream_t st, hipStream_t *aux, hipEvent_t *join) {
+    for (int i = 0; i < 3; ++i) {
+        if (hipEventRecord(join[i], aux[i]) != hipSuccess) return -1;
+        if (hipStreamWaitEvent(st, join[i], 0) != hipSuccess) return -1;
+    }
+    return 0;
+}
+
+}
+
+int launch_chain(const ChainArgs &A, const uint32_t *n_seeds, int cu_count, int plan, hipStream_t st, hipStream_t *aux,
                  hipEvent_t fork, hipEvent_t *join) {
     if (A.nseq <= 0) return 0;
-    unsigned long long *cls = A.ctr->chain_class, *tk = A.ctr->chain_ticket;
     if (hipFuncSetAttribute(reinterpret_cast<const void *>(chain_wave_kernel), hipFuncAttributeMaxDynamicSharedMemorySize,
                             (int)lds_bytes_xl(kClassXL2)) != hipSuccess) return -1;
-    if (hipEventRecord(fork, st) != hipSuccess) return -1;
-    for (int i = 0; i < 7; ++i)
-        if (hipStreamWaitEvent(aux[i], fork, 0) != hipSuccess) return -1;
-    chain_wave_kernel<<<(unsigned)cu_count, 64, lds_bytes_xl(kClassXL2), st>>>(A, cls + 9, cls + 6, tk + 9, -kClassXL2);
-    chain_wave_kernel<<<(unsigned)(cu_count * 8), 64, 0, aux[0]>>>(A, nullptr, cls + 9, tk + 0, 0);
-    chain_wave_kernel<<<(unsigned)cu_count, 64, lds_bytes_xl(kClassXL), aux[0]>>>(A, cls + 6, cls + 0, tk + 6, -kClassXL);
-    chain_wave_kernel<<<(unsigned)cu_count, 64, lds_bytes(kClassL), aux[1]>>>(A, cls + 0, cls + 7, tk + 1, kClassL);
-    chain_wave_kernel<<<(unsigned)(cu_count * 2), 64, lds_bytes(kClassL2), aux[5]>>>(A, cls + 7, cls + 1, tk + 7, kClassL2);
-    chain_wave_kernel<<<(unsigned)(cu_count * 3), 64, lds_bytes(kClassL1), aux[2]>>>(A, cls + 1, cls + 8, tk + 2, kClassL1);
-    chain_wave_kernel<<<(unsigned)(cu_count * 4), 64, lds_bytes(kClassM2), aux[6]>>>(A, cls + 8, cls + 2, tk + 8, kClassM2);
-    chain_wave_kernel<<<(unsigned)(cu_count * 8), 64, lds_bytes(kClassM1), aux[2]>>>(A, cls + 3, cls + 4, tk + 4, kClassM1);
-    chain_wave_kernel<<<(unsigned)(cu_count * 12), 64, lds_bytes(kClassS), aux[3]>>>(A, cls + 4, cls + 5, tk + 5, kClassS);
-    chain_kernel<<<(unsigned)((A.nseq + 63) / 64), 64, 0, aux[1]>>>(A, n_seeds);
-    chain_wave_kernel<<<(unsigned)(cu_count * 5), 64, lds_bytes(kClassM), aux[5]>>>(A, cls + 2, cls + 3, tk + 3, kClassM);
-    for (int i = 0; i < 7; ++i) {
-        if (hipEventRecord(join[i], aux[i]) != hipSuccess) return -1;
-        if (hipStreamWaitEvent(st, join[i], 0) != hipSuccess) return -1;
-    }
-    chain_redo_kernel<<<(unsigned)(cu_count * 2), 64, 0, st>>>(A);
     if (hipFuncSetAttribute(reinterpret_cast<const void *>(chain_heavy_kernel), hipFuncAttributeMaxDynamicSharedMemorySize,
                             (int)heavy_lds_bytes(kHeavyCap[5])) != hipSuccess) return -1;
-    if (hipEventRecord(fork, st) != hipSuccess) return -1;
-    for (int i = 0; i < 5; ++i)
-        if (hipStreamWaitEvent(aux[i], fork, 0) != hipSuccess) return -1;
-    unsigned long long *htk = A.ctr->heavy_tickets;
-    chain_heavy_kernel<<<(unsigned)cu_count, 64, heavy_lds_bytes(kHeavyCap[5]), st>>>(A, &A.ctr->n_heavy, kHeavyCap[4], kHeavyCap[5], htk + 5);
-    chain_heavy_kernel<<<(unsigned)(cu_count * 4), 64, heavy_lds_bytes(kHeavyCap[4]), aux[1]>>>(A, &A.ctr->n_heavy, kHeavyCap[3], kHeavyCap[4], htk + 4);
-    chain_heavy_kernel<<<(unsigned)(cu_count * 7), 64, heavy_lds_bytes(kHeavyCap[3]), aux[2]>>>(A, &A.ctr->n_heavy, kHeavyCap[2], kHeavyCap[3], htk + 3);
-    chain_heavy_kernel<<<(unsigned)(cu_count * 12), 64, heavy_lds_bytes(kHeavyCap[2]), aux[0]>>>(A, &A.ctr->n_heavy, kHeavyCap[1], kHeavyCap[2], htk + 2);
-    chain_heavy_kernel<<<(unsigned)(cu_count * 16), 64, heavy_lds_bytes(kHeavyCap[1]), aux[3]>>>(A, &A.ctr->n_heavy, kHeavyCap[0], kHeavyCap[1], htk + 1);
-    chain_heavy_kernel<<<(unsigned)(cu_count * 24), 64, heavy_lds_bytes(kHeavyCap[0]), aux[4]>>>(A, &A.ctr->n_heavy, 0, kHeavyCap[0], htk + 0);
-    for (int i = 0; i < 5; ++i) {
-        if (hipEventRecord(join[i], aux[i]) != hipSuccess) return -1;
-        if (hipStreamWaitEvent(st, join[i], 0) != hipSuccess) return -1;
-    }
+    const bool serial = plan == 1;
+    hipStream_t lane[4] = {st, serial ? st : aux[0], serial ? st : aux[1], serial ? st : aux[2]};
+    if (!serial && fork_lanes(st, aux, fork)) return -1;
+    if (serial) launch_wave_rows(A, kWaveSerial, n_seeds, cu_count, lane); else launch_wave_rows(A, kWavePlan, n_seeds, cu_count, lane);
+    if (!serial && join_lanes(st, aux, join)) return -1;
+    chain_redo_kernel<<<(unsigned)(cu_count * 2), 64, 0, st>>>(A);
+    if (!serial && fork_lanes(st, aux, fork)) return -1;
+    if (serial) launch_heavy_rows(A, kHeavySerial, cu_count, lane); else launch_heavy_rows(A, kHeavyPlan, cu_count, lane);
+    if (!serial && join_lanes(st, aux, join)) return -1;
     return 0;
 }
 void launch_chain_emit(const ChainArgs &A, const int64_t *chain_off, const int64_t *seed_off, bwams_chain_t *chains,
diff --git a/bwa-mem-scale_amd/csrc/chain_kernels.h b/bwa-mem-scale_amd/csrc/chain_kernels.h
--- a/bwa-mem-scale_amd/csrc/chain_kernels.h
+++ b/bwa-mem-scale_amd/csrc/chain_kernels.h
@@ -28,6 +28,7 @@
     void *nodes;
     int32_t *n_kept, *n_kept_seeds, *n_chn;
     int32_t *heavy;
+    int64_t heavy_stride;
     int64_t *read_base;
     int64_t *slice;
     const uint32_t *order;
@@ -40,7 +41,7 @@
 size_t chain_node_bytes(int64_t n_sa, int64_t nseq);
 size_t chain_rec_bytes(int64_t n_sa);
 void launch_chain_count(const ChainArgs &A, uint32_t *keys, uint32_t *vals, hipStream_t st);
-int launch_chain(const ChainArgs &A, const uint32_t *n_seeds, int cu_count, hipStream_t st, hipStream_t *aux,
+int launch_chain(const ChainArgs &A, const uint32_t *n_seeds, int cu_count, int plan, hipStream_t st, hipStream_t *aux,
                  hipEvent_t fork, hipEvent_t *join);
 void launch_chain_emit(const ChainArgs &A, const int64_t *chain_off, const int64_t *seed_off, bwams_chain_t *chains,
                        bwams_chain_seed_t *seeds, hipStream_t st);
@@ -121,13 +122,14 @@
     int32_t max_read_len;
     int32_t *n_out;
     int32_t *heavy, *light;
-    unsigned long long *n_heavy_ctr, *n_light_ctr, *ticket;
+    int64_t heavy_stride;
+    unsigned long long *n_heavy_ctr[3], *ticket[3];
+    unsigned long long *n_light_ctr;
     int32_t force_seq;
-    unsigned long long *ticket2, *ticket3;
     unsigned long long *dbg;
 };
 size_t dedup_sortrec_bytes(int64_t n);
-int launch_dedup(const DedupArgs &A, int64_t n_lanes, int64_t n_waves, int64_t n_waves_small, hipStream_t st, hipStream_t aux,
+int launch_dedup(const DedupArgs &A, int64_t n_lanes, int64_t n_waves, int64_t n_waves_small, int plan, hipStream_t st, hipStream_t aux,
                  hipStream_t aux2, hipStream_t aux3, hipEvent_t fork, hipEvent_t join, hipEvent_t join2, hipEvent_t join3);
 void launch_pestat(const bwams_alnreg_t *regs, const int64_t *reg_off, int64_t n_pairs, int64_t l_pac, const bwams_mem_opt_t &opt,
                    unsigned long long *keys, hipStream_t st);
diff --git a/bwa-mem-scale_amd/csrc/common.h b/bwa-mem-scale_amd/csrc/common.h
--- a/bwa-mem-scale_amd/csrc/common.h
+++ b/bwa-mem-scale_amd/csrc/common.h
@@ -29,6 +29,7 @@
     int trace_pair = 0;
     int bsw_pk = 1;
     int chain_batch = 1;
+    int chain_plan = 0;
     int ert_fat = 1;
     int ert_grid = -1, ert_ticket = 1;
 };
@@ -135,7 +136,7 @@
     unsigned long long emf_nodes, emf_cmp_bytes;
     unsigned long long chain_overflow;
     unsigned long long chain_longread;
-    unsigned long long n_heavy;
+    unsigned long long n_heavy[6];
     unsigned long long chain_class[10];
     unsigned long long chain_ticket[10];
     unsigned long long heavy_tickets[6];
@@ -152,6 +153,7 @@
     unsigned long long dbg[80];
     unsigned long long pair_ticket2;
     unsigned long long dedup_ticket2, dedup_ticket3;
+    unsigned long long dedup_heavy2, dedup_heavy3;
     unsigned long long ert_kmer, ert_nodes, ert_ref;
     unsigned long long work_head3, n_ext3, n_blk3, n_smem3;
     unsigned long long ert_ticket;
diff --git a/bwa-mem-scale_amd/csrc/dedup.hip b/bwa-mem-scale_amd/csrc/dedup.hip
--- a/bwa-mem-scale_amd/csrc/dedup.hip
+++ b/bwa-mem-scale_amd/csrc/dedup.hip
@@ -378,8 +378,10 @@
         A.n_out[r] = n;
         return;
     }
-    if (av_n > kLightN) A.heavy[atomicAdd(A.n_heavy_ctr, 1ull)] = (int32_t)r;
-    else A.light[atomicAdd(A.n_light_ctr, 1ull)] = (int32_t)r;
+    if (av_n > kLightN) {
+        const int c = av_n > kMidN ? 0 : av_n > kSmallN ? 1 : 2;
+        A.heavy[c * A.heavy_stride + (int64_t)atomicAdd(A.n_heavy_ctr[c], 1ull)] = (int32_t)r;
+    } else A.light[atomicAdd(A.n_light_ctr, 1ull)] = (int32_t)r;
 }
 
 __global__ __launch_bounds__(64) void dedup_kernel(DedupArgs A, int64_t n_lanes) {
@@ -417,8 +419,8 @@
     return n;
 }
 
-template <int CAP, int LO>
-__global__ __launch_bounds__(64) void dedup_wave_kernel(DedupArgs A, int64_t n_waves, int64_t eh_base, unsigned long long *ticket) {
+template <int CAP, int FIRST>
+__global__ __launch_bounds__(64) void dedup_wave_kernel(DedupArgs A, int64_t eh_base) {
     extern __shared__ __align__(16) unsigned char lds_dd[];
     SortRec *l_srt = reinterpret_cast<SortRec *>(lds_dd), *l_srt2 = l_srt + CAP;
     int2 *lds_eh = A.max_read_len <= kEhLdsLen ? reinterpret_cast<int2 *>(lds_dd + (size_t)60 * CAP) : nullptr;
@@ -428,14 +430,15 @@
     int32_t *l_ord = reinterpret_cast<int32_t *>(l_rb + CAP);
     const int lane = threadIdx.x;
     int2 *eh = A.eh + (eh_base + blockIdx.x) * (int64_t)(A.max_read_len + 2);
-    const int64_t n_heavy = (int64_t)*A.n_heavy_ctr;
+    for (int c = FIRST; c < 3; ++c) {
+    const int64_t n_heavy = (int64_t)*A.n_heavy_ctr[c];
+    const int32_t *heavy = A.heavy + c * A.heavy_stride;
     for (;;) {
-        const int64_t t = (int64_t)wave_ticket(ticket, 1ull);
+        const int64_t t = (int64_t)wave_ticket(A.ticket[c], 1ull);
         if (t >= n_heavy) break;
-        const int64_t r = A.heavy[t];
+        const int64_t r = heavy[t];
         const int64_t reg0 = A.seed_off[r];
         const int av_n = (int)(A.seed_off[r + 1] - reg0);
-        if (av_n <= LO || (av_n > CAP && CAP != kLdsN)) continue;
         bwams_alnreg_t *a = A.regs + reg0;
         int32_t *ord = A.ord + reg0;
         const uint8_t *query = A.enc + A.cum[r];
@@ -444,7 +447,7 @@
             if (lane == 0) A.n_out[r] = dedup_read(A, r, reinterpret_cast<SortRec *>(A.srt) + reg0, eh);
             continue;
         }
-        const bool prof = CAP == kLdsN && A.dbg != nullptr;
+        const bool prof = c == 0 && A.dbg != nullptr;
         unsigned long long n_al = 0, t_al = 0, n_it = 0;
         unsigned long long tk0 = prof ? wall_clock64() : 0ull, tk1 = tk0, tk2 = tk0, tk3 = tk0, tk4 = tk0, tk5 = tk0;
         int n = wave_compact_alive(a, l_ord, av_n, true, lane);
@@ -611,6 +614,7 @@
             atomicAdd(&A.dbg[18], n_al); atomicAdd(&A.dbg[19], t_al);
         }
     }
+    }
 }
 
 static_assert(sizeof(bwams_alnreg_t) == 112, "a region is seven 16-byte pieces");
@@ -713,20 +717,25 @@
 
 size_t dedup_sortrec_bytes(int64_t n) { return (size_t)(n + 1) * sizeof(SortRec); }
 
-int launch_dedup(const DedupArgs &A, int64_t n_lanes, int64_t n_waves, int64_t n_waves_small, hipStream_t st, hipStream_t aux,
+int launch_dedup(const DedupArgs &A, int64_t n_lanes, int64_t n_waves, int64_t n_waves_small, int plan, hipStream_t st, hipStream_t aux,
                  hipStream_t aux2, hipStream_t aux3, hipEvent_t fork, hipEvent_t join, hipEvent_t join2, hipEvent_t join3) {
     if (A.nseq <= 0) return 0;
     dedup_triage_kernel<<<(unsigned)((A.nseq + 255) / 256), 256, 0, st>>>(A);
+    if (hipFuncSetAttribute(reinterpret_cast<const void *>(dedup_wave_kernel<kLdsN, 0>), hipFuncAttributeMaxDynamicSharedMemorySize, (int)dd_lds_bytes(kLdsN, A.max_read_len)) != hipSuccess) return -1;
+    if (plan == 1) {
+        dedup_wave_kernel<kLdsN, 0><<<(unsigned)n_waves, 64, dd_lds_bytes(kLdsN, A.max_read_len), st>>>(A, A.eh_lanes);
+        dedup_kernel<<<(unsigned)((n_lanes + 63) / 64), 64, 0, st>>>(A, n_lanes);
+        return 0;
+    }
     if (hipEventRecord(fork, st) != hipSuccess || hipStreamWaitEvent(aux, fork, 0) != hipSuccess) return -1;
-    if (hipFuncSetAttribute(reinterpret_cast<const void *>(dedup_wave_kernel<kLdsN, kMidN>), hipFuncAttributeMaxDynamicSharedMemorySize, (int)dd_lds_bytes(kLdsN, A.max_read_len)) != hipSuccess) return -1;
-    dedup_wave_kernel<kLdsN, kMidN><<<(unsigned)n_waves, 64, dd_lds_bytes(kLdsN, A.max_read_len), st>>>(A, n_waves, A.eh_lanes, A.ticket);
+    dedup_wave_kernel<kLdsN, 0><<<(unsigned)n_waves, 64, dd_lds_bytes(kLdsN, A.max_read_len), st>>>(A, A.eh_lanes);
     dedup_kernel<<<(unsigned)((n_lanes + 63) / 64), 64, 0, aux>>>(A, n_lanes);
     if (hipEventRecord(join, aux) != hipSuccess || hipStreamWaitEvent(st, join, 0) != hipSuccess) return -1;
     if (hipStreamWaitEvent(aux3, fork, 0) != hipSuccess) return -1;
-    dedup_wave_kernel<kMidN, kSmallN><<<(unsigned)n_waves, 64, dd_lds_bytes(kMidN, A.max_read_len), aux3>>>(A, n_waves, A.eh_lanes + n_waves, A.ticket3);
+    dedup_wave_kernel<kMidN, 1><<<(unsigned)n_waves, 64, dd_lds_bytes(kMidN, A.max_read_len), aux3>>>(A, A.eh_lanes + n_waves);
     if (hipEventRecord(join3, aux3) != hipSuccess || hipStreamWaitEvent(st, join3, 0) != hipSuccess) return -1;
     if (hipStreamWaitEvent(aux2, fork, 0) != hipSuccess) return -1;
-    dedup_wave_kernel<kSmallN, kLightN><<<(unsigned)n_waves_small, 64, dd_lds_bytes(kSmallN, A.max_read_len), aux2>>>(A, n_waves_small, A.eh_lanes + 2 * n_waves, A.ticket2);
+    dedup_wave_kernel<kSmallN, 2><<<(unsigned)n_waves_small, 64, dd_lds_bytes(kSmallN, A.max_read_len), aux2>>>(A, A.eh_lanes + 2 * n_waves);
     if (hipEventRecord(join2, aux2) != hipSuccess || hipStreamWaitEvent(st, join2, 0) != hipSuccess) return -1;
     return 0;
 }
diff --git a/bwa-mem-scale_amd/csrc/stage_state.h b/bwa-mem-scale_amd/csrc/stage_state.h
--- a/bwa-mem-scale_amd/csrc/stage_state.h
+++ b/bwa-mem-scale_amd/csrc/stage_state.h
@@ -17,7 +17,7 @@
         DevBuf<bwams_ert_mem_t> et_mems; DevBuf<int64_t> et_moff, et_hoff, et_cnt, et_off, et_coord; DevBuf<uint64_t> et_hits;
         DevBuf<bwams_smem_t> et_smem;
         DevBuf<> et_srt;
-        int64_t n_chains = 0, n_seeds = 0, nseq = 0, n_redo = 0; bool done = false;
+        int64_t n_chains = 0, n_seeds = 0, nseq = 0, n_redo = 0, n_heavy[6] = {}; bool done = false;
     } ch;
     struct ExtStage {
         DevBuf<bwams_alnreg_t> regs; DevBuf<uint32_t> srt; DevBuf<int32_t> state, cur, lim;
diff --git a/include/bwams.h b/include/bwams.h
--- a/include/bwams.h
+++ b/include/bwams.h
@@ -232,6 +232,7 @@
     int64_t ert_kmer_lookups;
     int64_t ert_node_reads;
     int64_t ert_ref_bytes;
+    int64_t n_chain_heavy[6];
 } bwams_stats_t;
 int bwams_batch_stats(bwams_batch_t *b, bwams_stats_t *out);
 
```
